# yzang2019/tendermint-fork

Measured on AMD Instinct MI355X. Metric: ed25519 verifies/sec at 1/8 MI355X, higher is better.
Workload: dtype u32 (GF(2^255-19) radix 2^25.5 limbs, int64 accumulate); 1 GPU; C2: raw batch of 1048576 ed25519 signatures per GPU; signatures_per_gpu=1048576, key_cache=False, parallelism=shard-per-gpu x1

## Files before the change

### __graft_entry__.py

```python
from __future__ import annotations

import os
import subprocess
import sys

ROOT = os.path.dirname(os.path.abspath(__file__))
PKG = os.path.join(ROOT, "tendermint-fork_amd")


def _paths():
    for p in (ROOT, PKG):
        if p not in sys.path:
            sys.path.insert(0, p)


def build() -> None:
    env = dict(os.environ, PYTORCH_ROCM_ARCH="gfx950")
    jobs = str(min(8, os.cpu_count() or 1))
    subprocess.check_call(["make", "-j", jobs, "-C", PKG], env=env)
    subprocess.check_call(["make", "-s", "-C", os.path.join(ROOT, "oracle")])
    subprocess.check_call(["make", "-s", "-C", os.path.join(ROOT, "tests", "native")])
    _paths()
    import tmed
    tmed.lib()


def smoke() -> None:
    _paths()
    import numpy as np
    from oracle import port
    from tmed import Engine
    eng = Engine(0)
    rng = np.random.default_rng(0)
    for n in (256, 32768):
        seeds = rng.integers(0, 256, (n, 32), dtype=np.uint8)
        offs = (np.arange(n + 1) * 115).astype(np.uint32)
        msgs = rng.integers(0, 256, int(offs[-1]) + 16, dtype=np.uint8)
        sigs, pubs = eng.sign_arrays(seeds, msgs, offs)
        sigs[1::7, 9] ^= 1
        out = eng.verify_arrays(pubs, sigs, msgs, offs)
        exp = port.verify_batch(pubs, sigs, msgs, offs.astype(np.uint64), 8)
        esig, epub = port.sign_batch(seeds[:8], msgs, offs[:9].astype(np.uint64), 1)
        assert (out == exp).all(), "GPU/oracle decision mismatch (n=%d)" % n
        assert (pubs[:8] == epub).all() and (sigs[:1] == esig[:1]).all(), "GPU signer != oracle signer"
        assert out.sum() == n - len(range(1, n, 7))
    eng.close()
    print("smoke ok: 256 + 32768 signatures verified on cuda:0, decisions == oracle")


if __name__ == "__main__":
    build()
    if len(sys.argv) > 1 and sys.argv[1] == "smoke":
        smoke()
```

### tendermint-fork_amd/csrc/fe25519.h

```cpp
#pragma once
#include <stdint.h>

#if defined(__HIPCC__)
#include <hip/hip_runtime.h>
#define TMED_HD __host__ __device__ __forceinline__
#define TMED_HDM __host__ __device__ __forceinline__
#else
#define TMED_HD static inline
#define TMED_HDM inline
#endif

namespace tmed {

struct fe { int32_t v[10]; };

TMED_HD int32_t mul19(int32_t x) { return (int32_t)(19u * (uint32_t)x); }
TMED_HD int32_t mul38(int32_t x) { return (int32_t)(38u * (uint32_t)x); }
TMED_HD int32_t dbl32(int32_t x) {
#if defined(__HIP_DEVICE_COMPILE__)
  int32_t r;
  asm("v_add_u32 %0, %1, %1" : "=v"(r) : "v"(x));
  return r;
#else
  return (int32_t)(2u * (uint32_t)x);
// ... 163 lines not shown
  int64_t H0[10], H1[10];
  fe_sq2_sq1_fused(H0, H1, a.x, a.x2, a.x4, a.x19, a.x38, b.x, b.x2, b.x4, b.x19, b.x38);
  fe_fused_fin(h0, H0);
  fe_fused_fin(h1, H1);
}

TMED_HD void fe_sqn(fe &h, const fe &f, int n) {
  fe_sqc(h, f);
#pragma unroll 1
  for (int i = 1; i < n; i++) fe_sqc(h, h);
}

TMED_HD void fe_pow250(fe &z250, fe &z11, const fe &z) {
  fe z2, z9, t, a, b, c;
  fe_sqc(z2, z);
  fe_sqn(t, z2, 2); fe_mul(z9, t, z);
  fe_mul(z11, z9, z2);
  fe_sqc(t, z11); fe_mul(a, t, z9);
  fe_sqn(t, a, 5); fe_mul(b, t, a);
  fe_sqn(t, b, 10); fe_mul(c, t, b);
  fe_sqn(t, c, 20); fe_mul(t, t, c);
  fe_sqn(t, t, 10); fe_mul(a, t, b);
  fe_sqn(t, a, 50); fe_mul(b, t, a);
  fe_sqn(t, b, 100); fe_mul(t, t, b);
  fe_sqn(t, t, 50); fe_mul(z250, t, a);
}

TMED_HD void fe_invert(fe &out, const fe &z) {
  fe z250, z11, t;
  fe_pow250(z250, z11, z);
  fe_sqn(t, z250, 5); fe_mul(out, t, z11);
}

TMED_HD void fe_pow22523(fe &out, const fe &z) {
  fe z250, z11, t;
  fe_pow250(z250, z11, z);
  fe_sqn(t, z250, 2); fe_mul(out, t, z);
}

TMED_HD void fe_from_words(fe &h, const uint32_t w[8]) {
  const int off[10] = {0, 26, 51, 77, 102, 128, 153, 179, 204, 230};
  int64_t t[10];
#pragma unroll
  for (int i = 0; i < 10; i++) {
    const int o = off[i], q = o >> 5, r = o & 31;
    const uint64_t lo = w[q];
    const uint64_t hi = (q + 1 < 8) ? (uint64_t)w[q + 1] : 0;
    const uint64_t x = ((hi << 32) | lo) >> r;
    const uint32_t mask = (i & 1) ? 0x1ffffffu : 0x3ffffffu;
    t[i] = (int64_t)(uint32_t)(x & mask) + fe_bias(i);
  }
  fe_carry64(h, t);
}

TMED_HD void fe_to_words(uint32_t w[8], const fe &f) {
  int32_t h[10];
#pragma unroll
  for (int i = 0; i < 10; i++) h[i] = f.v[i];
  int32_t q = (19 * h[9] + (1 << 24)) >> 25;
#pragma unroll
  for (int i = 0; i < 10; i++) q = (h[i] + q) >> ((i & 1) ? 25 : 26);
  h[0] += 19 * q;
#pragma unroll
  for (int i = 0; i < 9; i++) {
    const int s = (i & 1) ? 25 : 26;
    const int32_t c = h[i] >> s;
    h[i + 1] += c;
// ... 211 lines not shown
```

### tendermint-fork_amd/csrc/fe_cols.h

```cpp
#pragma once

TMED_HD void fe_mul_fused(int64_t H[10], const int32_t f[10], const int32_t f2[10], const int32_t g[10], const int32_t g19[10]) {
  const int64_t b0 = (int64_t)1 << 25, b50 = (int64_t)1 << 50;
  int64_t t0, t1;
#if defined(__HIP_DEVICE_COMPILE__)
  asm(
      "v_mad_i64_i32 %0, vcc, %12, %27, %46\n"
      "v_mad_i64_i32 %1, vcc, %12, %28, %47\n"
      "v_mad_i64_i32 %0, vcc, %22, %45, %0\n"
      "v_mad_i64_i32 %1, vcc, %13, %27, %1\n"
      "v_mad_i64_i32 %0, vcc, %14, %44, %0\n"
      "v_mad_i64_i32 %1, vcc, %14, %45, %1\n"
      "v_mad_i64_i32 %0, vcc, %23, %43, %0\n"
      "v_mad_i64_i32 %1, vcc, %15, %44, %1\n"
      "v_mad_i64_i32 %0, vcc, %16, %42, %0\n"
      "v_mad_i64_i32 %1, vcc, %16, %43, %1\n"
      "v_mad_i64_i32 %0, vcc, %24, %41, %0\n"
      "v_mad_i64_i32 %1, vcc, %17, %42, %1\n"
      "v_mad_i64_i32 %0, vcc, %18, %40, %0\n"
      "v_mad_i64_i32 %1, vcc, %18, %41, %1\n"
      "v_mad_i64_i32 %0, vcc, %25, %39, %0\n"
      "v_mad_i64_i32 %1, vcc, %19, %40, %1\n"
      "v_mad_i64_i32 %0, vcc, %20, %38, %0\n"
      "v_mad_i64_i32 %1, vcc, %20, %39, %1\n"
// ... 30 lines not shown
      "v_lshl_add_u64 %3, %10, 0, %3\n"
      "v_mad_i64_i32 %5, vcc, %16, %28, %5\n"
      "v_ashrrev_i64 %11, 25, %3\n"
      "v_mad_i64_i32 %5, vcc, %17, %27, %5\n"
      "v_mad_i64_i32 %4, vcc, %12, %31, %11\n"
      "v_mad_i64_i32 %5, vcc, %18, %45, %5\n"
      "v_mad_i64_i32 %4, vcc, %22, %30, %4\n"
      "v_mad_i64_i32 %5, vcc, %19, %44, %5\n"
      "v_mad_i64_i32 %4, vcc, %14, %29, %4\n"
      "v_mad_i64_i32 %5, vcc, %20, %43, %5\n"
      "v_mad_i64_i32 %4, vcc, %23, %28, %4\n"
      "v_mad_i64_i32 %5, vcc, %21, %42, %5\n"
      "v_mad_i64_i32 %4, vcc, %16, %27, %4\n"
      "v_mad_i64_i32 %7, vcc, %12, %34, %47\n"
      "v_mad_i64_i32 %4, vcc, %24, %45, %4\n"
      "v_mad_i64_i32 %7, vcc, %13, %33, %7\n"
      "v_mad_i64_i32 %4, vcc, %18, %44, %4\n"
      "v_mad_i64_i32 %7, vcc, %14, %32, %7\n"
      "v_mad_i64_i32 %4, vcc, %25, %43, %4\n"
      "v_mad_i64_i32 %7, vcc, %15, %31, %7\n"
      "v_mad_i64_i32 %4, vcc, %20, %42, %4\n"
      "v_mad_i64_i32 %7, vcc, %16, %30, %7\n"
      "v_mad_i64_i32 %4, vcc, %26, %41, %4\n"
      "v_mad_i64_i32 %7, vcc, %17, %29, %7\n"
      "v_ashrrev_i64 %10, 26, %4\n"
      "v_mad_i64_i32 %7, vcc, %18, %28, %7\n"
      "v_lshl_add_u64 %5, %10, 0, %5\n"
      "v_mad_i64_i32 %7, vcc, %19, %27, %7\n"
      "v_ashrrev_i64 %11, 25, %5\n"
      "v_mad_i64_i32 %7, vcc, %20, %45, %7\n"
      "v_mad_i64_i32 %6, vcc, %12, %33, %11\n"
      "v_mad_i64_i32 %7, vcc, %21, %44, %7\n"
      "v_mad_i64_i32 %6, vcc, %22, %32, %6\n"
      "v_mad_i64_i32 %9, vcc, %12, %36, 0\n"
      "v_mad_i64_i32 %6, vcc, %14, %31, %6\n"
      "v_mad_i64_i32 %9, vcc, %13, %35, %9\n"
      "v_mad_i64_i32 %6, vcc, %23, %30, %6\n"
      "v_mad_i64_i32 %9, vcc, %14, %34, %9\n"
      "v_mad_i64_i32 %6, vcc, %16, %29, %6\n"
      "v_mad_i64_i32 %9, vcc, %15, %33, %9\n"
      "v_mad_i64_i32 %6, vcc, %24, %28, %6\n"
      "v_mad_i64_i32 %9, vcc, %16, %32, %9\n"
      "v_mad_i64_i32 %6, vcc, %18, %27, %6\n"
      "v_mad_i64_i32 %9, vcc, %17, %31, %9\n"
      "v_mad_i64_i32 %6, vcc, %25, %45, %6\n"
      "v_mad_i64_i32 %9, vcc, %18, %30, %9\n"
      "v_mad_i64_i32 %6, vcc, %20, %44, %6\n"
      "v_mad_i64_i32 %9, vcc, %19, %29, %9\n"
      "v_mad_i64_i32 %6, vcc, %26, %43, %6\n"
      "v_mad_i64_i32 %9, vcc, %20, %28, %9\n"
      "v_ashrrev_i64 %10, 26, %6\n"
      "v_mad_i64_i32 %9, vcc, %21, %27, %9\n"
      "v_lshl_add_u64 %7, %10, 0, %7\n"
      "v_ashrrev_i64 %11, 25, %7\n"
      "v_mad_i64_i32 %8, vcc, %12, %35, %11\n"
      "v_mad_i64_i32 %8, vcc, %22, %34, %8\n"
      "v_mad_i64_i32 %8, vcc, %14, %33, %8\n"
      "v_mad_i64_i32 %8, vcc, %23, %32, %8\n"
      "v_mad_i64_i32 %8, vcc, %16, %31, %8\n"
      "v_mad_i64_i32 %8, vcc, %24, %30, %8\n"
      "v_mad_i64_i32 %8, vcc, %18, %29, %8\n"
      "v_mad_i64_i32 %8, vcc, %25, %28, %8\n"
      "v_mad_i64_i32 %8, vcc, %20, %27, %8\n"
      "v_mad_i64_i32 %8, vcc, %26, %45, %8\n"
      "v_ashrrev_i64 %10, 26, %8\n"
      "v_lshl_add_u64 %9, %10, 0, %9\n"
      : "=&v"(H[0]), "=&v"(H[1]), "=&v"(H[2]), "=&v"(H[3]), "=&v"(H[4]), "=&v"(H[5]),
        "=&v"(H[6]), "=&v"(H[7]), "=&v"(H[8]), "=&v"(H[9]), "=&v"(t0), "=&v"(t1)
      : "v"(f[0]), "v"(f[1]), "v"(f[2]), "v"(f[3]), "v"(f[4]), "v"(f[5]),
        "v"(f[6]), "v"(f[7]), "v"(f[8]), "v"(f[9]), "v"(f2[1]), "v"(f2[3]),
        "v"(f2[5]), "v"(f2[7]), "v"(f2[9]), "v"(g[0]), "v"(g[1]), "v"(g[2]),
        "v"(g[3]), "v"(g[4]), "v"(g[5]), "v"(g[6]), "v"(g[7]), "v"(g[8]),
        "v"(g[9]), "v"(g19[1]), "v"(g19[2]), "v"(g19[3]), "v"(g19[4]), "v"(g19[5]),
        "v"(g19[6]), "v"(g19[7]), "v"(g19[8]), "v"(g19[9]), "s"(b0), "s"(b50)
      : "vcc");
#else
  H[0] = b0 + (int64_t)f[0] * (int64_t)g[0];
  H[1] = b50 + (int64_t)f[0] * (int64_t)g[1];
  H[0] = H[0] + (int64_t)f2[1] * (int64_t)g19[9];
  H[1] = H[1] + (int64_t)f[1] * (int64_t)g[0];
  H[0] = H[0] + (int64_t)f[2] * (int64_t)g19[8];
  H[1] = H[1] + (int64_t)f[2] * (int64_t)g19[9];
  H[0] = H[0] + (int64_t)f2[3] * (int64_t)g19[7];
  H[1] = H[1] + (int64_t)f[3] * (int64_t)g19[8];
  H[0] = H[0] + (int64_t)f[4] * (int64_t)g19[6];
  H[1] = H[1] + (int64_t)f[4] * (int64_t)g19[7];
  H[0] = H[0] + (int64_t)f2[5] * (int64_t)g19[5];
  H[1] = H[1] + (int64_t)f[5] * (int64_t)g19[6];
  H[0] = H[0] + (int64_t)f[6] * (int64_t)g19[4];
  H[1] = H[1] + (int64_t)f[6] * (int64_t)g19[5];
  H[0] = H[0] + (int64_t)f2[7] * (int64_t)g19[3];
  H[1] = H[1] + (int64_t)f[7] * (int64_t)g19[4];
  H[0] = H[0] + (int64_t)f[8] * (int64_t)g19[2];
  H[1] = H[1] + (int64_t)f[8] * (int64_t)g19[3];
  H[0] = H[0] + (int64_t)f2[9] * (int64_t)g19[1];
  H[1] = H[1] + (int64_t)f[9] * (int64_t)g19[2];
  t0 = H[0] >> 26;
  H[3] = b50 + (int64_t)f[0] * (int64_t)g[3];
  H[1] += t0;
// ... 25 lines not shown
  H[3] += t0;
  H[5] = H[5] + (int64_t)f[4] * (int64_t)g[1];
  t1 = H[3] >> 25;
  H[5] = H[5] + (int64_t)f[5] * (int64_t)g[0];
  H[4] = t1 + (int64_t)f[0] * (int64_t)g[4];
  H[5] = H[5] + (int64_t)f[6] * (int64_t)g19[9];
  H[4] = H[4] + (int64_t)f2[1] * (int64_t)g[3];
  H[5] = H[5] + (int64_t)f[7] * (int64_t)g19[8];
  H[4] = H[4] + (int64_t)f[2] * (int64_t)g[2];
  H[5] = H[5] + (int64_t)f[8] * (int64_t)g19[7];
  H[4] = H[4] + (int64_t)f2[3] * (int64_t)g[1];
  H[5] = H[5] + (int64_t)f[9] * (int64_t)g19[6];
  H[4] = H[4] + (int64_t)f[4] * (int64_t)g[0];
  H[7] = b50 + (int64_t)f[0] * (int64_t)g[7];
  H[4] = H[4] + (int64_t)f2[5] * (int64_t)g19[9];
  H[7] = H[7] + (int64_t)f[1] * (int64_t)g[6];
  H[4] = H[4] + (int64_t)f[6] * (int64_t)g19[8];
  H[7] = H[7] + (int64_t)f[2] * (int64_t)g[5];
  H[4] = H[4] + (int64_t)f2[7] * (int64_t)g19[7];
  H[7] = H[7] + (int64_t)f[3] * (int64_t)g[4];
  H[4] = H[4] + (int64_t)f[8] * (int64_t)g19[6];
  H[7] = H[7] + (int64_t)f[4] * (int64_t)g[3];
  H[4] = H[4] + (int64_t)f2[9] * (int64_t)g19[5];
  H[7] = H[7] + (int64_t)f[5] * (int64_t)g[2];
  t0 = H[4] >> 26;
  H[7] = H[7] + (int64_t)f[6] * (int64_t)g[1];
  H[5] += t0;
  H[7] = H[7] + (int64_t)f[7] * (int64_t)g[0];
  t1 = H[5] >> 25;
  H[7] = H[7] + (int64_t)f[8] * (int64_t)g19[9];
  H[6] = t1 + (int64_t)f[0] * (int64_t)g[6];
  H[7] = H[7] + (int64_t)f[9] * (int64_t)g19[8];
  H[6] = H[6] + (int64_t)f2[1] * (int64_t)g[5];
  H[9] = 0 + (int64_t)f[0] * (int64_t)g[9];
  H[6] = H[6] + (int64_t)f[2] * (int64_t)g[4];
  H[9] = H[9] + (int64_t)f[1] * (int64_t)g[8];
  H[6] = H[6] + (int64_t)f2[3] * (int64_t)g[3];
  H[9] = H[9] + (int64_t)f[2] * (int64_t)g[7];
  H[6] = H[6] + (int64_t)f[4] * (int64_t)g[2];
  H[9] = H[9] + (int64_t)f[3] * (int64_t)g[6];
  H[6] = H[6] + (int64_t)f2[5] * (int64_t)g[1];
  H[9] = H[9] + (int64_t)f[4] * (int64_t)g[5];
  H[6] = H[6] + (int64_t)f[6] * (int64_t)g[0];
  H[9] = H[9] + (int64_t)f[5] * (int64_t)g[4];
  H[6] = H[6] + (int64_t)f2[7] * (int64_t)g19[9];
  H[9] = H[9] + (int64_t)f[6] * (int64_t)g[3];
  H[6] = H[6] + (int64_t)f[8] * (int64_t)g19[8];
  H[9] = H[9] + (int64_t)f[7] * (int64_t)g[2];
  H[6] = H[6] + (int64_t)f2[9] * (int64_t)g19[7];
  H[9] = H[9] + (int64_t)f[8] * (int64_t)g[1];
  t0 = H[6] >> 26;
  H[9] = H[9] + (int64_t)f[9] * (int64_t)g[0];
  H[7] += t0;
  t1 = H[7] >> 25;
  H[8] = t1 + (int64_t)f[0] * (int64_t)g[8];
  H[8] = H[8] + (int64_t)f2[1] * (int64_t)g[7];
  H[8] = H[8] + (int64_t)f[2] * (int64_t)g[6];
  H[8] = H[8] + (int64_t)f2[3] * (int64_t)g[5];
  H[8] = H[8] + (int64_t)f[4] * (int64_t)g[4];
  H[8] = H[8] + (int64_t)f2[5] * (int64_t)g[3];
  H[8] = H[8] + (int64_t)f[6] * (int64_t)g[2];
  H[8] = H[8] + (int64_t)f2[7] * (int64_t)g[1];
  H[8] = H[8] + (int64_t)f[8] * (int64_t)g[0];
  H[8] = H[8] + (int64_t)f2[9] * (int64_t)g19[9];
  t0 = H[8] >> 26;
  H[9] += t0;
#endif
}

TMED_HD void fe_sq1_fused(int64_t H[10], const int32_t x[10], const int32_t x2[10], const int32_t x4[10], const int32_t x19[10], const int32_t x38[10]) {
  const int64_t b0 = (int64_t)1 << 25, b50 = (int64_t)1 << 50;
  int64_t t0, t1;
#if defined(__HIP_DEVICE_COMPILE__)
  asm(
      "v_mad_i64_i32 %0, vcc, %32, %40, %41\n"
      "v_mad_i64_i32 %1, vcc, %24, %40, %42\n"
      "v_mad_i64_i32 %0, vcc, %24, %39, %0\n"
      "v_mad_i64_i32 %1, vcc, %25, %39, %1\n"
      "v_mad_i64_i32 %0, vcc, %33, %38, %0\n"
      "v_mad_i64_i32 %1, vcc, %26, %38, %1\n"
      "v_mad_i64_i32 %0, vcc, %26, %37, %0\n"
      "v_mad_i64_i32 %1, vcc, %27, %37, %1\n"
      "v_mad_i64_i32 %0, vcc, %27, %36, %0\n"
      "v_mad_i64_i32 %1, vcc, %22, %13, %1\n"
      "v_mad_i64_i32 %0, vcc, %12, %12, %0\n"
      "v_mad_i64_i32 %3, vcc, %26, %40, %42\n"
      "v_ashrrev_i64 %10, 26, %0\n"
      "v_mad_i64_i32 %3, vcc, %27, %39, %3\n"
      "v_lshl_add_u64 %1, %10, 0, %1\n"
      "v_mad_i64_i32 %3, vcc, %28, %38, %3\n"
      "v_ashrrev_i64 %11, 25, %1\n"
      "v_mad_i64_i32 %3, vcc, %22, %15, %3\n"
      "v_mad_i64_i32 %2, vcc, %33, %40, %11\n"
      "v_mad_i64_i32 %3, vcc, %23, %14, %3\n"
      "v_mad_i64_i32 %2, vcc, %26, %39, %2\n"
      "v_mad_i64_i32 %5, vcc, %28, %40, %42\n"
      "v_mad_i64_i32 %2, vcc, %34, %38, %2\n"
      "v_mad_i64_i32 %5, vcc, %29, %39, %5\n"
      "v_mad_i64_i32 %2, vcc, %18, %37, %2\n"
      "v_mad_i64_i32 %5, vcc, %22, %17, %5\n"
      "v_mad_i64_i32 %2, vcc, %22, %14, %2\n"
      "v_mad_i64_i32 %5, vcc, %23, %16, %5\n"
      "v_mad_i64_i32 %2, vcc, %23, %13, %2\n"
      "v_mad_i64_i32 %5, vcc, %24, %15, %5\n"
      "v_ashrrev_i64 %10, 26, %2\n"
      "v_mad_i64_i32 %7, vcc, %30, %40, %42\n"
      "v_lshl_add_u64 %3, %10, 0, %3\n"
      "v_mad_i64_i32 %7, vcc, %22, %19, %7\n"
      "v_ashrrev_i64 %11, 25, %3\n"
      "v_mad_i64_i32 %7, vcc, %23, %18, %7\n"
      "v_mad_i64_i32 %4, vcc, %34, %40, %11\n"
      "v_mad_i64_i32 %7, vcc, %24, %17, %7\n"
      "v_mad_i64_i32 %4, vcc, %28, %39, %4\n"
      "v_mad_i64_i32 %7, vcc, %25, %16, %7\n"
      "v_mad_i64_i32 %4, vcc, %29, %38, %4\n"
      "v_mad_i64_i32 %9, vcc, %22, %21, 0\n"
      "v_mad_i64_i32 %4, vcc, %22, %16, %4\n"
      "v_mad_i64_i32 %9, vcc, %23, %20, %9\n"
      "v_mad_i64_i32 %4, vcc, %32, %15, %4\n"
      "v_mad_i64_i32 %9, vcc, %24, %19, %9\n"
      "v_mad_i64_i32 %4, vcc, %14, %14, %4\n"
      "v_mad_i64_i32 %9, vcc, %25, %18, %9\n"
      "v_ashrrev_i64 %10, 26, %4\n"
      "v_mad_i64_i32 %9, vcc, %26, %17, %9\n"
      "v_lshl_add_u64 %5, %10, 0, %5\n"
      "v_ashrrev_i64 %11, 25, %5\n"
      "v_mad_i64_i32 %6, vcc, %35, %40, %11\n"
      "v_mad_i64_i32 %6, vcc, %20, %39, %6\n"
      "v_mad_i64_i32 %6, vcc, %22, %18, %6\n"
      "v_mad_i64_i32 %6, vcc, %32, %17, %6\n"
      "v_mad_i64_i32 %6, vcc, %24, %16, %6\n"
      "v_mad_i64_i32 %6, vcc, %25, %15, %6\n"
      "v_ashrrev_i64 %10, 26, %6\n"
      "v_lshl_add_u64 %7, %10, 0, %7\n"
      "v_ashrrev_i64 %11, 25, %7\n"
      "v_mad_i64_i32 %8, vcc, %31, %40, %11\n"
      "v_mad_i64_i32 %8, vcc, %22, %20, %8\n"
      "v_mad_i64_i32 %8, vcc, %32, %19, %8\n"
      "v_mad_i64_i32 %8, vcc, %24, %18, %8\n"
      "v_mad_i64_i32 %8, vcc, %33, %17, %8\n"
      "v_mad_i64_i32 %8, vcc, %16, %16, %8\n"
      "v_ashrrev_i64 %10, 26, %8\n"
      "v_lshl_add_u64 %9, %10, 0, %9\n"
      : "=&v"(H[0]), "=&v"(H[1]), "=&v"(H[2]), "=&v"(H[3]), "=&v"(H[4]), "=&v"(H[5]),
        "=&v"(H[6]), "=&v"(H[7]), "=&v"(H[8]), "=&v"(H[9]), "=&v"(t0), "=&v"(t1)
      : "v"(x[0]), "v"(x[1]), "v"(x[2]), "v"(x[3]), "v"(x[4]), "v"(x[5]),
        "v"(x[6]), "v"(x[7]), "v"(x[8]), "v"(x[9]), "v"(x2[0]), "v"(x2[1]),
        "v"(x2[2]), "v"(x2[3]), "v"(x2[4]), "v"(x2[5]), "v"(x2[6]), "v"(x2[7]),
        "v"(x2[8]), "v"(x2[9]), "v"(x4[1]), "v"(x4[3]), "v"(x4[5]), "v"(x4[7]),
        "v"(x19[5]), "v"(x19[6]), "v"(x19[7]), "v"(x19[8]), "v"(x19[9]), "s"(b0),
        "s"(b50)
      : "vcc");
#else
  H[0] = b0 + (int64_t)x4[1] * (int64_t)x19[9];
  H[1] = b50 + (int64_t)x2[2] * (int64_t)x19[9];
  H[0] = H[0] + (int64_t)x2[2] * (int64_t)x19[8];
  H[1] = H[1] + (int64_t)x2[3] * (int64_t)x19[8];
  H[0] = H[0] + (int64_t)x4[3] * (int64_t)x19[7];
  H[1] = H[1] + (int64_t)x2[4] * (int64_t)x19[7];
  H[0] = H[0] + (int64_t)x2[4] * (int64_t)x19[6];
  H[1] = H[1] + (int64_t)x2[5] * (int64_t)x19[6];
  H[0] = H[0] + (int64_t)x2[5] * (int64_t)x19[5];
  H[1] = H[1] + (int64_t)x2[0] * (int64_t)x[1];
  H[0] = H[0] + (int64_t)x[0] * (int64_t)x[0];
  H[3] = b50 + (int64_t)x2[4] * (int64_t)x19[9];
  t0 = H[0] >> 26;
  H[3] = H[3] + (int64_t)x2[5] * (int64_t)x19[8];
  H[1] += t0;
  H[3] = H[3] + (int64_t)x2[6] * (int64_t)x19[7];
  t1 = H[1] >> 25;
  H[3] = H[3] + (int64_t)x2[0] * (int64_t)x[3];
  H[2] = t1 + (int64_t)x4[3] * (int64_t)x19[9];
  H[3] = H[3] + (int64_t)x2[1] * (int64_t)x[2];
  H[2] = H[2] + (int64_t)x2[4] * (int64_t)x19[8];
  H[5] = b50 + (int64_t)x2[6] * (int64_t)x19[9];
  H[2] = H[2] + (int64_t)x4[5] * (int64_t)x19[7];
  H[5] = H[5] + (int64_t)x2[7] * (int64_t)x19[8];
  H[2] = H[2] + (int64_t)x[6] * (int64_t)x19[6];
  H[5] = H[5] + (int64_t)x2[0] * (int64_t)x[5];
  H[2] = H[2] + (int64_t)x2[0] * (int64_t)x[2];
  H[5] = H[5] + (int64_t)x2[1] * (int64_t)x[4];
  H[2] = H[2] + (int64_t)x2[1] * (int64_t)x[1];
  H[5] = H[5] + (int64_t)x2[2] * (int64_t)x[3];
  t0 = H[2] >> 26;
  H[7] = b50 + (int64_t)x2[8] * (int64_t)x19[9];
  H[3] += t0;
  H[7] = H[7] + (int64_t)x2[0] * (int64_t)x[7];
  t1 = H[3] >> 25;
  H[7] = H[7] + (int64_t)x2[1] * (int64_t)x[6];
  H[4] = t1 + (int64_t)x4[5] * (int64_t)x19[9];
  H[7] = H[7] + (int64_t)x2[2] * (int64_t)x[5];
  H[4] = H[4] + (int64_t)x2[6] * (int64_t)x19[8];
  H[7] = H[7] + (int64_t)x2[3] * (int64_t)x[4];
  H[4] = H[4] + (int64_t)x2[7] * (int64_t)x19[7];
  H[9] = 0 + (int64_t)x2[0] * (int64_t)x[9];
  H[4] = H[4] + (int64_t)x2[0] * (int64_t)x[4];
  H[9] = H[9] + (int64_t)x2[1] * (int64_t)x[8];
  H[4] = H[4] + (int64_t)x4[1] * (int64_t)x[3];
  H[9] = H[9] + (int64_t)x2[2] * (int64_t)x[7];
  H[4] = H[4] + (int64_t)x[2] * (int64_t)x[2];
  H[9] = H[9] + (int64_t)x2[3] * (int64_t)x[6];
  t0 = H[4] >> 26;
  H[9] = H[9] + (int64_t)x2[4] * (int64_t)x[5];
  H[5] += t0;
  t1 = H[5] >> 25;
  H[6] = t1 + (int64_t)x4[7] * (int64_t)x19[9];
  H[6] = H[6] + (int64_t)x[8] * (int64_t)x19[8];
  H[6] = H[6] + (int64_t)x2[0] * (int64_t)x[6];
  H[6] = H[6] + (int64_t)x4[1] * (int64_t)x[5];
  H[6] = H[6] + (int64_t)x2[2] * (int64_t)x[4];
  H[6] = H[6] + (int64_t)x2[3] * (int64_t)x[3];
  t0 = H[6] >> 26;
  H[7] += t0;
  t1 = H[7] >> 25;
  H[8] = t1 + (int64_t)x2[9] * (int64_t)x19[9];
  H[8] = H[8] + (int64_t)x2[0] * (int64_t)x[8];
  H[8] = H[8] + (int64_t)x4[1] * (int64_t)x[7];
  H[8] = H[8] + (int64_t)x2[2] * (int64_t)x[6];
  H[8] = H[8] + (int64_t)x4[3] * (int64_t)x[5];
  H[8] = H[8] + (int64_t)x[4] * (int64_t)x[4];
  t0 = H[8] >> 26;
  H[9] += t0;
#endif
}

TMED_HD void fe_sq2_fused(int64_t H[10], const int32_t x[10], const int32_t x2[10], const int32_t x4[10], const int32_t x19[10], const int32_t x38[10]) {
  const int64_t b0 = (int64_t)1 << 25, b50 = (int64_t)1 << 50;
  int64_t t0, t1;
#if defined(__HIP_DEVICE_COMPILE__)
  asm(
      "v_mad_i64_i32 %0, vcc, %28, %36, %37\n"
      "v_mad_i64_i32 %1, vcc, %20, %36, %38\n"
      "v_mad_i64_i32 %0, vcc, %20, %35, %0\n"
      "v_mad_i64_i32 %1, vcc, %21, %35, %1\n"
      "v_mad_i64_i32 %0, vcc, %29, %34, %0\n"
      "v_mad_i64_i32 %1, vcc, %22, %34, %1\n"
      "v_mad_i64_i32 %0, vcc, %22, %33, %0\n"
      "v_mad_i64_i32 %1, vcc, %23, %33, %1\n"
      "v_mad_i64_i32 %0, vcc, %23, %32, %0\n"
      "v_mad_i64_i32 %1, vcc, %12, %28, %1\n"
      "v_mad_i64_i32 %0, vcc, %19, %12, %0\n"
      "v_mad_i64_i32 %3, vcc, %22, %36, %38\n"
      "v_ashrrev_i64 %10, 26, %0\n"
      "v_mad_i64_i32 %3, vcc, %23, %35, %3\n"
      "v_lshl_add_u64 %1, %10, 0, %1\n"
      "v_mad_i64_i32 %3, vcc, %24, %34, %3\n"
      "v_ashrrev_i64 %11, 25, %1\n"
      "v_mad_i64_i32 %3, vcc, %19, %21, %3\n"
      "v_mad_i64_i32 %2, vcc, %29, %36, %11\n"
      "v_mad_i64_i32 %3, vcc, %28, %14, %3\n"
      "v_mad_i64_i32 %2, vcc, %22, %35, %2\n"
      "v_mad_i64_i32 %5, vcc, %24, %36, %38\n"
      "v_mad_i64_i32 %2, vcc, %30, %34, %2\n"
      "v_mad_i64_i32 %5, vcc, %25, %35, %5\n"
      "v_mad_i64_i32 %2, vcc, %17, %33, %2\n"
      "v_mad_i64_i32 %5, vcc, %19, %23, %5\n"
      "v_mad_i64_i32 %2, vcc, %19, %20, %2\n"
      "v_mad_i64_i32 %5, vcc, %28, %16, %5\n"
      "v_mad_i64_i32 %2, vcc, %28, %13, %2\n"
      "v_mad_i64_i32 %5, vcc, %20, %21, %5\n"
      "v_ashrrev_i64 %10, 26, %2\n"
      "v_mad_i64_i32 %7, vcc, %26, %36, %38\n"
      "v_lshl_add_u64 %3, %10, 0, %3\n"
      "v_mad_i64_i32 %7, vcc, %19, %25, %7\n"
      "v_ashrrev_i64 %11, 25, %3\n"
      "v_mad_i64_i32 %7, vcc, %28, %17, %7\n"
      "v_mad_i64_i32 %4, vcc, %30, %36, %11\n"
      "v_mad_i64_i32 %7, vcc, %20, %23, %7\n"
      "v_mad_i64_i32 %4, vcc, %24, %35, %4\n"
      "v_mad_i64_i32 %7, vcc, %29, %16, %7\n"
      "v_mad_i64_i32 %4, vcc, %25, %34, %4\n"
      "v_mad_i64_i32 %9, vcc, %19, %27, 0\n"
      "v_mad_i64_i32 %4, vcc, %19, %22, %4\n"
      "v_mad_i64_i32 %9, vcc, %28, %18, %9\n"
      "v_mad_i64_i32 %4, vcc, %28, %21, %4\n"
      "v_mad_i64_i32 %9, vcc, %20, %25, %9\n"
      "v_mad_i64_i32 %4, vcc, %20, %14, %4\n"
      "v_mad_i64_i32 %9, vcc, %29, %17, %9\n"
      "v_ashrrev_i64 %10, 26, %4\n"
      "v_mad_i64_i32 %9, vcc, %22, %23, %9\n"
      "v_lshl_add_u64 %5, %10, 0, %5\n"
      "v_ashrrev_i64 %11, 25, %5\n"
      "v_mad_i64_i32 %6, vcc, %31, %36, %11\n"
      "v_mad_i64_i32 %6, vcc, %18, %35, %6\n"
      "v_mad_i64_i32 %6, vcc, %19, %24, %6\n"
      "v_mad_i64_i32 %6, vcc, %28, %23, %6\n"
      "v_mad_i64_i32 %6, vcc, %20, %22, %6\n"
      "v_mad_i64_i32 %6, vcc, %29, %15, %6\n"
      "v_ashrrev_i64 %10, 26, %6\n"
      "v_lshl_add_u64 %7, %10, 0, %7\n"
      "v_ashrrev_i64 %11, 25, %7\n"
      "v_mad_i64_i32 %8, vcc, %27, %36, %11\n"
      "v_mad_i64_i32 %8, vcc, %19, %26, %8\n"
      "v_mad_i64_i32 %8, vcc, %28, %25, %8\n"
      "v_mad_i64_i32 %8, vcc, %20, %24, %8\n"
      "v_mad_i64_i32 %8, vcc, %29, %23, %8\n"
      "v_mad_i64_i32 %8, vcc, %22, %16, %8\n"
      "v_ashrrev_i64 %10, 26, %8\n"
      "v_lshl_add_u64 %9, %10, 0, %9\n"
      : "=&v"(H[0]), "=&v"(H[1]), "=&v"(H[2]), "=&v"(H[3]), "=&v"(H[4]), "=&v"(H[5]),
        "=&v"(H[6]), "=&v"(H[7]), "=&v"(H[8]), "=&v"(H[9]), "=&v"(t0), "=&v"(t1)
      : "v"(x[0]), "v"(x[1]), "v"(x[2]), "v"(x[3]), "v"(x[4]), "v"(x[6]),
        "v"(x[8]), "v"(x2[0]), "v"(x2[2]), "v"(x2[3]), "v"(x2[4]), "v"(x2[5]),
        "v"(x2[6]), "v"(x2[7]), "v"(x2[8]), "v"(x2[9]), "v"(x4[1]), "v"(x4[3]),
        "v"(x4[5]), "v"(x4[7]), "v"(x38[5]), "v"(x38[6]), "v"(x38[7]), "v"(x38[8]),
        "v"(x38[9]), "s"(b0), "s"(b50)
      : "vcc");
#else
  H[0] = b0 + (int64_t)x4[1] * (int64_t)x38[9];
  H[1] = b50 + (int64_t)x2[2] * (int64_t)x38[9];
  H[0] = H[0] + (int64_t)x2[2] * (int64_t)x38[8];
  H[1] = H[1] + (int64_t)x2[3] * (int64_t)x38[8];
  H[0] = H[0] + (int64_t)x4[3] * (int64_t)x38[7];
  H[1] = H[1] + (int64_t)x2[4] * (int64_t)x38[7];
  H[0] = H[0] + (int64_t)x2[4] * (int64_t)x38[6];
  H[1] = H[1] + (int64_t)x2[5] * (int64_t)x38[6];
  H[0] = H[0] + (int64_t)x2[5] * (int64_t)x38[5];
  H[1] = H[1] + (int64_t)x[0] * (int64_t)x4[1];
  H[0] = H[0] + (int64_t)x2[0] * (int64_t)x[0];
  H[3] = b50 + (int64_t)x2[4] * (int64_t)x38[9];
  t0 = H[0] >> 26;
  H[3] = H[3] + (int64_t)x2[5] * (int64_t)x38[8];
  H[1] += t0;
  H[3] = H[3] + (int64_t)x2[6] * (int64_t)x38[7];
  t1 = H[1] >> 25;
  H[3] = H[3] + (int64_t)x2[0] * (int64_t)x2[3];
  H[2] = t1 + (int64_t)x4[3] * (int64_t)x38[9];
  H[3] = H[3] + (int64_t)x4[1] * (int64_t)x[2];
  H[2] = H[2] + (int64_t)x2[4] * (int64_t)x38[8];
  H[5] = b50 + (int64_t)x2[6] * (int64_t)x38[9];
  H[2] = H[2] + (int64_t)x4[5] * (int64_t)x38[7];
  H[5] = H[5] + (int64_t)x2[7] * (int64_t)x38[8];
  H[2] = H[2] + (int64_t)x[6] * (int64_t)x38[6];
  H[5] = H[5] + (int64_t)x2[0] * (int64_t)x2[5];
  H[2] = H[2] + (int64_t)x2[0] * (int64_t)x2[2];
  H[5] = H[5] + (int64_t)x4[1] * (int64_t)x[4];
  H[2] = H[2] + (int64_t)x4[1] * (int64_t)x[1];
  H[5] = H[5] + (int64_t)x2[2] * (int64_t)x2[3];
  t0 = H[2] >> 26;
  H[7] = b50 + (int64_t)x2[8] * (int64_t)x38[9];
  H[3] += t0;
  H[7] = H[7] + (int64_t)x2[0] * (int64_t)x2[7];
  t1 = H[3] >> 25;
  H[7] = H[7] + (int64_t)x4[1] * (int64_t)x[6];
  H[4] = t1 + (int64_t)x4[5] * (int64_t)x38[9];
  H[7] = H[7] + (int64_t)x2[2] * (int64_t)x2[5];
  H[4] = H[4] + (int64_t)x2[6] * (int64_t)x38[8];
  H[7] = H[7] + (int64_t)x4[3] * (int64_t)x[4];
  H[4] = H[4] + (int64_t)x2[7] * (int64_t)x38[7];
  H[9] = 0 + (int64_t)x2[0] * (int64_t)x2[9];
  H[4] = H[4] + (int64_t)x2[0] * (int64_t)x2[4];
  H[9] = H[9] + (int64_t)x4[1] * (int64_t)x[8];
  H[4] = H[4] + (int64_t)x4[1] * (int64_t)x2[3];
  H[9] = H[9] + (int64_t)x2[2] * (int64_t)x2[7];
  H[4] = H[4] + (int64_t)x2[2] * (int64_t)x[2];
  H[9] = H[9] + (int64_t)x4[3] * (int64_t)x[6];
  t0 = H[4] >> 26;
  H[9] = H[9] + (int64_t)x2[4] * (int64_t)x2[5];
  H[5] += t0;
  t1 = H[5] >> 25;
  H[6] = t1 + (int64_t)x4[7] * (int64_t)x38[9];
  H[6] = H[6] + (int64_t)x[8] * (int64_t)x38[8];
  H[6] = H[6] + (int64_t)x2[0] * (int64_t)x2[6];
  H[6] = H[6] + (int64_t)x4[1] * (int64_t)x2[5];
  H[6] = H[6] + (int64_t)x2[2] * (int64_t)x2[4];
  H[6] = H[6] + (int64_t)x4[3] * (int64_t)x[3];
  t0 = H[6] >> 26;
  H[7] += t0;
  t1 = H[7] >> 25;
  H[8] = t1 + (int64_t)x2[9] * (int64_t)x38[9];
  H[8] = H[8] + (int64_t)x2[0] * (int64_t)x2[8];
  H[8] = H[8] + (int64_t)x4[1] * (int64_t)x2[7];
  H[8] = H[8] + (int64_t)x2[2] * (int64_t)x2[6];
  H[8] = H[8] + (int64_t)x4[3] * (int64_t)x2[5];
  H[8] = H[8] + (int64_t)x2[4] * (int64_t)x[4];
  t0 = H[8] >> 26;
  H[9] += t0;
#endif
}


TMED_HD void fe_mul_fused_x2(int64_t H0[10], int64_t H1[10], const int32_t a_f[10], const int32_t a_f2[10], const int32_t a_g[10], const int32_t a_g19[10], const int32_t b_f[10], const int32_t b_f2[10], const int32_t b_g[10], const int32_t b_g19[10]) {
  const int64_t b0 = (int64_t)1 << 25, b50 = (int64_t)1 << 50;
  int64_t t0_0, t0_1, t1_0, t1_1;
#if defined(__HIP_DEVICE_COMPILE__)
  asm(
      "v_mad_i64_i32 %0, vcc, %24, %39, %92\n"
      "v_mad_i64_i32 %12, vcc, %58, %73, %92\n"
      "v_mad_i64_i32 %1, vcc, %24, %40, %93\n"
      "v_mad_i64_i32 %0, vcc, %34, %57, %0\n"
      "v_mad_i64_i32 %12, vcc, %68, %91, %12\n"
      "v_mad_i64_i32 %13, vcc, %58, %74, %93\n"
      "v_mad_i64_i32 %0, vcc, %26, %56, %0\n"
      "v_mad_i64_i32 %1, vcc, %25, %39, %1\n"
      "v_mad_i64_i32 %12, vcc, %60, %90, %12\n"
      "v_mad_i64_i32 %13, vcc, %59, %73, %13\n"
      "v_mad_i64_i32 %0, vcc, %35, %55, %0\n"
      "v_mad_i64_i32 %1, vcc, %26, %57, %1\n"
      "v_mad_i64_i32 %12, vcc, %69, %89, %12\n"
      "v_mad_i64_i32 %13, vcc, %60, %91, %13\n"
      "v_mad_i64_i32 %0, vcc, %28, %54, %0\n"
      "v_mad_i64_i32 %1, vcc, %27, %56, %1\n"
      "v_mad_i64_i32 %12, vcc, %62, %88, %12\n"
      "v_mad_i64_i32 %13, vcc, %61, %90, %13\n"
      "v_mad_i64_i32 %0, vcc, %36, %53, %0\n"
      "v_mad_i64_i32 %1, vcc, %28, %55, %1\n"
      "v_mad_i64_i32 %12, vcc, %70, %87, %12\n"
      "v_mad_i64_i32 %13, vcc, %62, %89, %13\n"
      "v_mad_i64_i32 %0, vcc, %30, %52, %0\n"
      "v_mad_i64_i32 %1, vcc, %29, %54, %1\n"
// ... 534 lines not shown
      "v_mad_i64_i32 %5, vcc, %36, %27, %5\n"
      "v_ashrrev_i64 %10, 26, %4\n"
      "v_mad_i64_i32 %17, vcc, %65, %56, %17\n"
      "v_ashrrev_i64 %22, 26, %16\n"
      "v_lshl_add_u64 %5, %10, 0, %5\n"
      "v_mad_i64_i32 %7, vcc, %42, %52, %83\n"
      "v_lshl_add_u64 %17, %22, 0, %17\n"
      "v_ashrrev_i64 %11, 25, %5\n"
      "v_mad_i64_i32 %19, vcc, %71, %81, %83\n"
      "v_ashrrev_i64 %23, 25, %17\n"
      "v_mad_i64_i32 %6, vcc, %47, %52, %11\n"
      "v_mad_i64_i32 %7, vcc, %34, %31, %7\n"
      "v_mad_i64_i32 %18, vcc, %76, %81, %23\n"
      "v_mad_i64_i32 %6, vcc, %32, %51, %6\n"
      "v_mad_i64_i32 %19, vcc, %63, %60, %19\n"
      "v_mad_i64_i32 %18, vcc, %61, %80, %18\n"
      "v_mad_i64_i32 %6, vcc, %34, %30, %6\n"
      "v_mad_i64_i32 %7, vcc, %35, %30, %7\n"
      "v_mad_i64_i32 %18, vcc, %63, %59, %18\n"
      "v_mad_i64_i32 %6, vcc, %44, %29, %6\n"
      "v_mad_i64_i32 %19, vcc, %64, %59, %19\n"
      "v_mad_i64_i32 %18, vcc, %73, %58, %18\n"
      "v_mad_i64_i32 %6, vcc, %36, %28, %6\n"
      "v_mad_i64_i32 %7, vcc, %36, %29, %7\n"
      "v_mad_i64_i32 %18, vcc, %65, %57, %18\n"
      "v_mad_i64_i32 %6, vcc, %37, %27, %6\n"
      "v_mad_i64_i32 %19, vcc, %65, %58, %19\n"
      "v_mad_i64_i32 %18, vcc, %66, %56, %18\n"
      "v_mad_i64_i32 %7, vcc, %37, %28, %7\n"
      "v_ashrrev_i64 %10, 26, %6\n"
      "v_mad_i64_i32 %19, vcc, %66, %57, %19\n"
      "v_ashrrev_i64 %22, 26, %18\n"
      "v_lshl_add_u64 %7, %10, 0, %7\n"
      "v_mad_i64_i32 %9, vcc, %34, %33, 0\n"
      "v_lshl_add_u64 %19, %22, 0, %19\n"
      "v_ashrrev_i64 %11, 25, %7\n"
      "v_mad_i64_i32 %21, vcc, %63, %62, 0\n"
      "v_ashrrev_i64 %23, 25, %19\n"
      "v_mad_i64_i32 %8, vcc, %43, %52, %11\n"
      "v_mad_i64_i32 %9, vcc, %35, %32, %9\n"
      "v_mad_i64_i32 %20, vcc, %72, %81, %23\n"
      "v_mad_i64_i32 %8, vcc, %34, %32, %8\n"
      "v_mad_i64_i32 %21, vcc, %64, %61, %21\n"
      "v_mad_i64_i32 %20, vcc, %63, %61, %20\n"
      "v_mad_i64_i32 %8, vcc, %44, %31, %8\n"
      "v_mad_i64_i32 %9, vcc, %36, %31, %9\n"
      "v_mad_i64_i32 %20, vcc, %73, %60, %20\n"
      "v_mad_i64_i32 %8, vcc, %36, %30, %8\n"
      "v_mad_i64_i32 %21, vcc, %65, %60, %21\n"
      "v_mad_i64_i32 %20, vcc, %65, %59, %20\n"
      "v_mad_i64_i32 %8, vcc, %45, %29, %8\n"
      "v_mad_i64_i32 %9, vcc, %37, %30, %9\n"
      "v_mad_i64_i32 %20, vcc, %74, %58, %20\n"
      "v_mad_i64_i32 %8, vcc, %28, %28, %8\n"
      "v_mad_i64_i32 %21, vcc, %66, %59, %21\n"
      "v_mad_i64_i32 %20, vcc, %57, %57, %20\n"
      "v_mad_i64_i32 %9, vcc, %38, %29, %9\n"
      "v_ashrrev_i64 %10, 26, %8\n"
      "v_mad_i64_i32 %21, vcc, %67, %58, %21\n"
      "v_ashrrev_i64 %22, 26, %20\n"
      "v_lshl_add_u64 %9, %10, 0, %9\n"
      "v_lshl_add_u64 %21, %22, 0, %21\n"
      : "=&v"(H0[0]), "=&v"(H0[1]), "=&v"(H0[2]), "=&v"(H0[3]), "=&v"(H0[4]), "=&v"(H0[5]),
        "=&v"(H0[6]), "=&v"(H0[7]), "=&v"(H0[8]), "=&v"(H0[9]), "=&v"(t0_0), "=&v"(t0_1),
        "=&v"(H1[0]), "=&v"(H1[1]), "=&v"(H1[2]), "=&v"(H1[3]), "=&v"(H1[4]), "=&v"(H1[5]),
        "=&v"(H1[6]), "=&v"(H1[7]), "=&v"(H1[8]), "=&v"(H1[9]), "=&v"(t1_0), "=&v"(t1_1)
      : "v"(a_x[0]), "v"(a_x[1]), "v"(a_x[2]), "v"(a_x[3]), "v"(a_x[4]), "v"(a_x[5]),
        "v"(a_x[6]), "v"(a_x[7]), "v"(a_x[8]), "v"(a_x[9]), "v"(a_x2[0]), "v"(a_x2[1]),
        "v"(a_x2[2]), "v"(a_x2[3]), "v"(a_x2[4]), "v"(a_x2[5]), "v"(a_x2[6]), "v"(a_x2[7]),
        "v"(a_x2[8]), "v"(a_x2[9]), "v"(a_x4[1]), "v"(a_x4[3]), "v"(a_x4[5]), "v"(a_x4[7]),
        "v"(a_x19[5]), "v"(a_x19[6]), "v"(a_x19[7]), "v"(a_x19[8]), "v"(a_x19[9]), "v"(b_x[0]),
        "v"(b_x[1]), "v"(b_x[2]), "v"(b_x[3]), "v"(b_x[4]), "v"(b_x[5]), "v"(b_x[6]),
        "v"(b_x[7]), "v"(b_x[8]), "v"(b_x[9]), "v"(b_x2[0]), "v"(b_x2[1]), "v"(b_x2[2]),
        "v"(b_x2[3]), "v"(b_x2[4]), "v"(b_x2[5]), "v"(b_x2[6]), "v"(b_x2[7]), "v"(b_x2[8]),
        "v"(b_x2[9]), "v"(b_x4[1]), "v"(b_x4[3]), "v"(b_x4[5]), "v"(b_x4[7]), "v"(b_x19[5]),
        "v"(b_x19[6]), "v"(b_x19[7]), "v"(b_x19[8]), "v"(b_x19[9]), "s"(b0), "s"(b50)
      : "vcc");
#else
  H0[0] = b0 + (int64_t)a_x4[1] * (int64_t)a_x19[9];
  H1[0] = b0 + (int64_t)b_x4[1] * (int64_t)b_x19[9];
  H0[1] = b50 + (int64_t)a_x2[2] * (int64_t)a_x19[9];
  H0[0] = H0[0] + (int64_t)a_x2[2] * (int64_t)a_x19[8];
  H1[0] = H1[0] + (int64_t)b_x2[2] * (int64_t)b_x19[8];
  H1[1] = b50 + (int64_t)b_x2[2] * (int64_t)b_x19[9];
  H0[0] = H0[0] + (int64_t)a_x4[3] * (int64_t)a_x19[7];
  H1[0] = H1[0] + (int64_t)b_x4[3] * (int64_t)b_x19[7];
  H0[1] = H0[1] + (int64_t)a_x2[3] * (int64_t)a_x19[8];
  H0[0] = H0[0] + (int64_t)a_x2[4] * (int64_t)a_x19[6];
  H1[0] = H1[0] + (int64_t)b_x2[4] * (int64_t)b_x19[6];
  H1[1] = H1[1] + (int64_t)b_x2[3] * (int64_t)b_x19[8];
  H0[0] = H0[0] + (int64_t)a_x2[5] * (int64_t)a_x19[5];
  H0[1] = H0[1] + (int64_t)a_x2[4] * (int64_t)a_x19[7];
  H1[0] = H1[0] + (int64_t)b_x2[5] * (int64_t)b_x19[5];
  H1[1] = H1[1] + (int64_t)b_x2[4] * (int64_t)b_x19[7];
  H0[0] = H0[0] + (int64_t)a_x[0] * (int64_t)a_x[0];
// ... 59 lines not shown
  H0[5] = H0[5] + (int64_t)a_x2[2] * (int64_t)a_x[3];
  t0_0 = H0[4] >> 26;
  H1[5] = H1[5] + (int64_t)b_x2[2] * (int64_t)b_x[3];
  t1_0 = H1[4] >> 26;
  H0[5] += t0_0;
  H0[7] = b50 + (int64_t)a_x2[8] * (int64_t)a_x19[9];
  H1[5] += t1_0;
  t0_1 = H0[5] >> 25;
  H1[7] = b50 + (int64_t)b_x2[8] * (int64_t)b_x19[9];
  t1_1 = H1[5] >> 25;
  H0[6] = t0_1 + (int64_t)a_x4[7] * (int64_t)a_x19[9];
  H0[7] = H0[7] + (int64_t)a_x2[0] * (int64_t)a_x[7];
  H1[6] = t1_1 + (int64_t)b_x4[7] * (int64_t)b_x19[9];
  H0[6] = H0[6] + (int64_t)a_x[8] * (int64_t)a_x19[8];
  H1[7] = H1[7] + (int64_t)b_x2[0] * (int64_t)b_x[7];
  H1[6] = H1[6] + (int64_t)b_x[8] * (int64_t)b_x19[8];
  H0[6] = H0[6] + (int64_t)a_x2[0] * (int64_t)a_x[6];
  H0[7] = H0[7] + (int64_t)a_x2[1] * (int64_t)a_x[6];
  H1[6] = H1[6] + (int64_t)b_x2[0] * (int64_t)b_x[6];
  H0[6] = H0[6] + (int64_t)a_x4[1] * (int64_t)a_x[5];
  H1[7] = H1[7] + (int64_t)b_x2[1] * (int64_t)b_x[6];
  H1[6] = H1[6] + (int64_t)b_x4[1] * (int64_t)b_x[5];
  H0[6] = H0[6] + (int64_t)a_x2[2] * (int64_t)a_x[4];
  H0[7] = H0[7] + (int64_t)a_x2[2] * (int64_t)a_x[5];
  H1[6] = H1[6] + (int64_t)b_x2[2] * (int64_t)b_x[4];
  H0[6] = H0[6] + (int64_t)a_x2[3] * (int64_t)a_x[3];
  H1[7] = H1[7] + (int64_t)b_x2[2] * (int64_t)b_x[5];
  H1[6] = H1[6] + (int64_t)b_x2[3] * (int64_t)b_x[3];
  H0[7] = H0[7] + (int64_t)a_x2[3] * (int64_t)a_x[4];
  t0_0 = H0[6] >> 26;
  H1[7] = H1[7] + (int64_t)b_x2[3] * (int64_t)b_x[4];
  t1_0 = H1[6] >> 26;
  H0[7] += t0_0;
  H0[9] = 0 + (int64_t)a_x2[0] * (int64_t)a_x[9];
  H1[7] += t1_0;
  t0_1 = H0[7] >> 25;
  H1[9] = 0 + (int64_t)b_x2[0] * (int64_t)b_x[9];
  t1_1 = H1[7] >> 25;
  H0[8] = t0_1 + (int64_t)a_x2[9] * (int64_t)a_x19[9];
  H0[9] = H0[9] + (int64_t)a_x2[1] * (int64_t)a_x[8];
  H1[8] = t1_1 + (int64_t)b_x2[9] * (int64_t)b_x19[9];
  H0[8] = H0[8] + (int64_t)a_x2[0] * (int64_t)a_x[8];
  H1[9] = H1[9] + (int64_t)b_x2[1] * (int64_t)b_x[8];
  H1[8] = H1[8] + (int64_t)b_x2[0] * (int64_t)b_x[8];
  H0[8] = H0[8] + (int64_t)a_x4[1] * (int64_t)a_x[7];
  H0[9] = H0[9] + (int64_t)a_x2[2] * (int64_t)a_x[7];
  H1[8] = H1[8] + (int64_t)b_x4[1] * (int64_t)b_x[7];
  H0[8] = H0[8] + (int64_t)a_x2[2] * (int64_t)a_x[6];
  H1[9] = H1[9] + (int64_t)b_x2[2] * (int64_t)b_x[7];
  H1[8] = H1[8] + (int64_t)b_x2[2] * (int64_t)b_x[6];
  H0[8] = H0[8] + (int64_t)a_x4[3] * (int64_t)a_x[5];
  H0[9] = H0[9] + (int64_t)a_x2[3] * (int64_t)a_x[6];
  H1[8] = H1[8] + (int64_t)b_x4[3] * (int64_t)b_x[5];
  H0[8] = H0[8] + (int64_t)a_x[4] * (int64_t)a_x[4];
  H1[9] = H1[9] + (int64_t)b_x2[3] * (int64_t)b_x[6];
  H1[8] = H1[8] + (int64_t)b_x[4] * (int64_t)b_x[4];
  H0[9] = H0[9] + (int64_t)a_x2[4] * (int64_t)a_x[5];
  t0_0 = H0[8] >> 26;
  H1[9] = H1[9] + (int64_t)b_x2[4] * (int64_t)b_x[5];
  t1_0 = H1[8] >> 26;
  H0[9] += t0_0;
  H1[9] += t1_0;
#endif
}

TMED_HD void fe_sq2_sq1_fused(int64_t H0[10], int64_t H1[10], const int32_t a_x[10], const int32_t a_x2[10], const int32_t a_x4[10], const int32_t a_x19[10], const int32_t a_x38[10], const int32_t b_x[10], const int32_t b_x2[10], const int32_t b_x4[10], const int32_t b_x19[10], const int32_t b_x38[10]) {
  const int64_t b0 = (int64_t)1 << 25, b50 = (int64_t)1 << 50;
  int64_t t0_0, t0_1, t1_0, t1_1;
#if defined(__HIP_DEVICE_COMPILE__)
  asm(
      "v_mad_i64_i32 %0, vcc, %40, %48, %78\n"
      "v_mad_i64_i32 %12, vcc, %69, %77, %78\n"
      "v_mad_i64_i32 %1, vcc, %32, %48, %79\n"
      "v_mad_i64_i32 %0, vcc, %32, %47, %0\n"
      "v_mad_i64_i32 %12, vcc, %61, %76, %12\n"
      "v_mad_i64_i32 %13, vcc, %61, %77, %79\n"
      "v_mad_i64_i32 %0, vcc, %41, %46, %0\n"
      "v_mad_i64_i32 %12, vcc, %70, %75, %12\n"
      "v_mad_i64_i32 %1, vcc, %33, %47, %1\n"
      "v_mad_i64_i32 %0, vcc, %34, %45, %0\n"
      "v_mad_i64_i32 %12, vcc, %63, %74, %12\n"
      "v_mad_i64_i32 %13, vcc, %62, %76, %13\n"
      "v_mad_i64_i32 %0, vcc, %35, %44, %0\n"
      "v_mad_i64_i32 %1, vcc, %34, %46, %1\n"
      "v_mad_i64_i32 %12, vcc, %64, %73, %12\n"
      "v_mad_i64_i32 %13, vcc, %63, %75, %13\n"
      "v_mad_i64_i32 %0, vcc, %31, %24, %0\n"
      "v_mad_i64_i32 %1, vcc, %35, %45, %1\n"
      "v_mad_i64_i32 %12, vcc, %49, %49, %12\n"
      "v_mad_i64_i32 %13, vcc, %64, %74, %13\n"
      "v_mad_i64_i32 %1, vcc, %24, %40, %1\n"
      "v_ashrrev_i64 %10, 26, %0\n"
      "v_mad_i64_i32 %13, vcc, %59, %50, %13\n"
      "v_ashrrev_i64 %22, 26, %12\n"
      "v_lshl_add_u64 %1, %10, 0, %1\n"
// ... 51 lines not shown
      "v_mad_i64_i32 %5, vcc, %32, %33, %5\n"
      "v_ashrrev_i64 %10, 26, %4\n"
      "v_mad_i64_i32 %17, vcc, %61, %52, %17\n"
      "v_ashrrev_i64 %22, 26, %16\n"
      "v_lshl_add_u64 %5, %10, 0, %5\n"
      "v_mad_i64_i32 %7, vcc, %38, %48, %79\n"
      "v_lshl_add_u64 %17, %22, 0, %17\n"
      "v_ashrrev_i64 %11, 25, %5\n"
      "v_mad_i64_i32 %19, vcc, %67, %77, %79\n"
      "v_ashrrev_i64 %23, 25, %17\n"
      "v_mad_i64_i32 %6, vcc, %43, %48, %11\n"
      "v_mad_i64_i32 %7, vcc, %31, %37, %7\n"
      "v_mad_i64_i32 %18, vcc, %72, %77, %23\n"
      "v_mad_i64_i32 %6, vcc, %30, %47, %6\n"
      "v_mad_i64_i32 %19, vcc, %59, %56, %19\n"
      "v_mad_i64_i32 %18, vcc, %57, %76, %18\n"
      "v_mad_i64_i32 %6, vcc, %31, %36, %6\n"
      "v_mad_i64_i32 %7, vcc, %40, %29, %7\n"
      "v_mad_i64_i32 %18, vcc, %59, %55, %18\n"
      "v_mad_i64_i32 %6, vcc, %40, %35, %6\n"
      "v_mad_i64_i32 %19, vcc, %60, %55, %19\n"
      "v_mad_i64_i32 %18, vcc, %69, %54, %18\n"
      "v_mad_i64_i32 %6, vcc, %32, %34, %6\n"
      "v_mad_i64_i32 %7, vcc, %32, %35, %7\n"
      "v_mad_i64_i32 %18, vcc, %61, %53, %18\n"
      "v_mad_i64_i32 %6, vcc, %41, %27, %6\n"
      "v_mad_i64_i32 %19, vcc, %61, %54, %19\n"
      "v_mad_i64_i32 %18, vcc, %62, %52, %18\n"
      "v_mad_i64_i32 %7, vcc, %41, %28, %7\n"
      "v_ashrrev_i64 %10, 26, %6\n"
      "v_mad_i64_i32 %19, vcc, %62, %53, %19\n"
      "v_ashrrev_i64 %22, 26, %18\n"
      "v_lshl_add_u64 %7, %10, 0, %7\n"
      "v_mad_i64_i32 %9, vcc, %31, %39, 0\n"
      "v_lshl_add_u64 %19, %22, 0, %19\n"
      "v_ashrrev_i64 %11, 25, %7\n"
      "v_mad_i64_i32 %21, vcc, %59, %58, 0\n"
      "v_ashrrev_i64 %23, 25, %19\n"
      "v_mad_i64_i32 %8, vcc, %39, %48, %11\n"
      "v_mad_i64_i32 %9, vcc, %40, %30, %9\n"
      "v_mad_i64_i32 %20, vcc, %68, %77, %23\n"
      "v_mad_i64_i32 %8, vcc, %31, %38, %8\n"
      "v_mad_i64_i32 %21, vcc, %60, %57, %21\n"
      "v_mad_i64_i32 %20, vcc, %59, %57, %20\n"
      "v_mad_i64_i32 %8, vcc, %40, %37, %8\n"
      "v_mad_i64_i32 %9, vcc, %32, %37, %9\n"
      "v_mad_i64_i32 %20, vcc, %69, %56, %20\n"
      "v_mad_i64_i32 %8, vcc, %32, %36, %8\n"
      "v_mad_i64_i32 %21, vcc, %61, %56, %21\n"
      "v_mad_i64_i32 %20, vcc, %61, %55, %20\n"
      "v_mad_i64_i32 %8, vcc, %41, %35, %8\n"
      "v_mad_i64_i32 %9, vcc, %41, %29, %9\n"
      "v_mad_i64_i32 %20, vcc, %70, %54, %20\n"
      "v_mad_i64_i32 %8, vcc, %34, %28, %8\n"
      "v_mad_i64_i32 %21, vcc, %62, %55, %21\n"
      "v_mad_i64_i32 %20, vcc, %53, %53, %20\n"
      "v_mad_i64_i32 %9, vcc, %34, %35, %9\n"
      "v_ashrrev_i64 %10, 26, %8\n"
      "v_mad_i64_i32 %21, vcc, %63, %54, %21\n"
      "v_ashrrev_i64 %22, 26, %20\n"
      "v_lshl_add_u64 %9, %10, 0, %9\n"
      "v_lshl_add_u64 %21, %22, 0, %21\n"
      : "=&v"(H0[0]), "=&v"(H0[1]), "=&v"(H0[2]), "=&v"(H0[3]), "=&v"(H0[4]), "=&v"(H0[5]),
        "=&v"(H0[6]), "=&v"(H0[7]), "=&v"(H0[8]), "=&v"(H0[9]), "=&v"(t0_0), "=&v"(t0_1),
        "=&v"(H1[0]), "=&v"(H1[1]), "=&v"(H1[2]), "=&v"(H1[3]), "=&v"(H1[4]), "=&v"(H1[5]),
        "=&v"(H1[6]), "=&v"(H1[7]), "=&v"(H1[8]), "=&v"(H1[9]), "=&v"(t1_0), "=&v"(t1_1)
      : "v"(a_x[0]), "v"(a_x[1]), "v"(a_x[2]), "v"(a_x[3]), "v"(a_x[4]), "v"(a_x[6]),
        "v"(a_x[8]), "v"(a_x2[0]), "v"(a_x2[2]), "v"(a_x2[3]), "v"(a_x2[4]), "v"(a_x2[5]),
        "v"(a_x2[6]), "v"(a_x2[7]), "v"(a_x2[8]), "v"(a_x2[9]), "v"(a_x4[1]), "v"(a_x4[3]),
        "v"(a_x4[5]), "v"(a_x4[7]), "v"(a_x38[5]), "v"(a_x38[6]), "v"(a_x38[7]), "v"(a_x38[8]),
        "v"(a_x38[9]), "v"(b_x[0]), "v"(b_x[1]), "v"(b_x[2]), "v"(b_x[3]), "v"(b_x[4]),
        "v"(b_x[5]), "v"(b_x[6]), "v"(b_x[7]), "v"(b_x[8]), "v"(b_x[9]), "v"(b_x2[0]),
        "v"(b_x2[1]), "v"(b_x2[2]), "v"(b_x2[3]), "v"(b_x2[4]), "v"(b_x2[5]), "v"(b_x2[6]),
        "v"(b_x2[7]), "v"(b_x2[8]), "v"(b_x2[9]), "v"(b_x4[1]), "v"(b_x4[3]), "v"(b_x4[5]),
        "v"(b_x4[7]), "v"(b_x19[5]), "v"(b_x19[6]), "v"(b_x19[7]), "v"(b_x19[8]), "v"(b_x19[9]),
        "s"(b0), "s"(b50)
      : "vcc");
#else
  H0[0] = b0 + (int64_t)a_x4[1] * (int64_t)a_x38[9];
  H1[0] = b0 + (int64_t)b_x4[1] * (int64_t)b_x19[9];
  H0[1] = b50 + (int64_t)a_x2[2] * (int64_t)a_x38[9];
  H0[0] = H0[0] + (int64_t)a_x2[2] * (int64_t)a_x38[8];
  H1[0] = H1[0] + (int64_t)b_x2[2] * (int64_t)b_x19[8];
  H1[1] = b50 + (int64_t)b_x2[2] * (int64_t)b_x19[9];
  H0[0] = H0[0] + (int64_t)a_x4[3] * (int64_t)a_x38[7];
  H1[0] = H1[0] + (int64_t)b_x4[3] * (int64_t)b_x19[7];
  H0[1] = H0[1] + (int64_t)a_x2[3] * (int64_t)a_x38[8];
  H0[0] = H0[0] + (int64_t)a_x2[4] * (int64_t)a_x38[6];
  H1[0] = H1[0] + (int64_t)b_x2[4] * (int64_t)b_x19[6];
  H1[1] = H1[1] + (int64_t)b_x2[3] * (int64_t)b_x19[8];
  H0[0] = H0[0] + (int64_t)a_x2[5] * (int64_t)a_x38[5];
  H0[1] = H0[1] + (int64_t)a_x2[4] * (int64_t)a_x38[7];
  H1[0] = H1[0] + (int64_t)b_x2[5] * (int64_t)b_x19[5];
  H1[1] = H1[1] + (int64_t)b_x2[4] * (int64_t)b_x19[7];
  H0[0] = H0[0] + (int64_t)a_x2[0] * (int64_t)a_x[0];
// ... 59 lines not shown
  H0[5] = H0[5] + (int64_t)a_x2[2] * (int64_t)a_x2[3];
  t0_0 = H0[4] >> 26;
  H1[5] = H1[5] + (int64_t)b_x2[2] * (int64_t)b_x[3];
  t1_0 = H1[4] >> 26;
  H0[5] += t0_0;
  H0[7] = b50 + (int64_t)a_x2[8] * (int64_t)a_x38[9];
  H1[5] += t1_0;
  t0_1 = H0[5] >> 25;
  H1[7] = b50 + (int64_t)b_x2[8] * (int64_t)b_x19[9];
  t1_1 = H1[5] >> 25;
  H0[6] = t0_1 + (int64_t)a_x4[7] * (int64_t)a_x38[9];
  H0[7] = H0[7] + (int64_t)a_x2[0] * (int64_t)a_x2[7];
  H1[6] = t1_1 + (int64_t)b_x4[7] * (int64_t)b_x19[9];
  H0[6] = H0[6] + (int64_t)a_x[8] * (int64_t)a_x38[8];
  H1[7] = H1[7] + (int64_t)b_x2[0] * (int64_t)b_x[7];
  H1[6] = H1[6] + (int64_t)b_x[8] * (int64_t)b_x19[8];
  H0[6] = H0[6] + (int64_t)a_x2[0] * (int64_t)a_x2[6];
  H0[7] = H0[7] + (int64_t)a_x4[1] * (int64_t)a_x[6];
  H1[6] = H1[6] + (int64_t)b_x2[0] * (int64_t)b_x[6];
  H0[6] = H0[6] + (int64_t)a_x4[1] * (int64_t)a_x2[5];
  H1[7] = H1[7] + (int64_t)b_x2[1] * (int64_t)b_x[6];
  H1[6] = H1[6] + (int64_t)b_x4[1] * (int64_t)b_x[5];
  H0[6] = H0[6] + (int64_t)a_x2[2] * (int64_t)a_x2[4];
  H0[7] = H0[7] + (int64_t)a_x2[2] * (int64_t)a_x2[5];
  H1[6] = H1[6] + (int64_t)b_x2[2] * (int64_t)b_x[4];
  H0[6] = H0[6] + (int64_t)a_x4[3] * (int64_t)a_x[3];
  H1[7] = H1[7] + (int64_t)b_x2[2] * (int64_t)b_x[5];
  H1[6] = H1[6] + (int64_t)b_x2[3] * (int64_t)b_x[3];
  H0[7] = H0[7] + (int64_t)a_x4[3] * (int64_t)a_x[4];
  t0_0 = H0[6] >> 26;
  H1[7] = H1[7] + (int64_t)b_x2[3] * (int64_t)b_x[4];
  t1_0 = H1[6] >> 26;
  H0[7] += t0_0;
  H0[9] = 0 + (int64_t)a_x2[0] * (int64_t)a_x2[9];
  H1[7] += t1_0;
  t0_1 = H0[7] >> 25;
  H1[9] = 0 + (int64_t)b_x2[0] * (int64_t)b_x[9];
  t1_1 = H1[7] >> 25;
  H0[8] = t0_1 + (int64_t)a_x2[9] * (int64_t)a_x38[9];
  H0[9] = H0[9] + (int64_t)a_x4[1] * (int64_t)a_x[8];
  H1[8] = t1_1 + (int64_t)b_x2[9] * (int64_t)b_x19[9];
  H0[8] = H0[8] + (int64_t)a_x2[0] * (int64_t)a_x2[8];
  H1[9] = H1[9] + (int64_t)b_x2[1] * (int64_t)b_x[8];
  H1[8] = H1[8] + (int64_t)b_x2[0] * (int64_t)b_x[8];
  H0[8] = H0[8] + (int64_t)a_x4[1] * (int64_t)a_x2[7];
  H0[9] = H0[9] + (int64_t)a_x2[2] * (int64_t)a_x2[7];
  H1[8] = H1[8] + (int64_t)b_x4[1] * (int64_t)b_x[7];
  H0[8] = H0[8] + (int64_t)a_x2[2] * (int64_t)a_x2[6];
  H1[9] = H1[9] + (int64_t)b_x2[2] * (int64_t)b_x[7];
  H1[8] = H1[8] + (int64_t)b_x2[2] * (int64_t)b_x[6];
  H0[8] = H0[8] + (int64_t)a_x4[3] * (int64_t)a_x2[5];
  H0[9] = H0[9] + (int64_t)a_x4[3] * (int64_t)a_x[6];
  H1[8] = H1[8] + (int64_t)b_x4[3] * (int64_t)b_x[5];
  H0[8] = H0[8] + (int64_t)a_x2[4] * (int64_t)a_x[4];
  H1[9] = H1[9] + (int64_t)b_x2[3] * (int64_t)b_x[6];
  H1[8] = H1[8] + (int64_t)b_x[4] * (int64_t)b_x[4];
  H0[9] = H0[9] + (int64_t)a_x2[4] * (int64_t)a_x2[5];
  t0_0 = H0[8] >> 26;
  H1[9] = H1[9] + (int64_t)b_x2[4] * (int64_t)b_x[5];
  t1_0 = H1[8] >> 26;
  H0[9] += t0_0;
  H1[9] += t1_0;
#endif
}


TMED_HD void fe_sq1c_fused(int64_t H[10], const int32_t x[10], const int32_t x2[10], const int32_t x19[10], const int32_t x38[10]) {
  const int64_t b0 = (int64_t)1 << 25, b50 = (int64_t)1 << 50;
  int64_t t0, t1;
#if defined(__HIP_DEVICE_COMPILE__)
  asm(
      "v_mad_i64_i32 %0, vcc, %23, %34, %35\n"
      "v_mad_i64_i32 %1, vcc, %14, %34, %36\n"
      "v_mad_i64_i32 %0, vcc, %14, %33, %0\n"
      "v_mad_i64_i32 %1, vcc, %15, %33, %1\n"
      "v_mad_i64_i32 %0, vcc, %25, %32, %0\n"
      "v_mad_i64_i32 %1, vcc, %16, %32, %1\n"
      "v_mad_i64_i32 %0, vcc, %16, %31, %0\n"
      "v_mad_i64_i32 %1, vcc, %17, %31, %1\n"
      "v_mad_i64_i32 %0, vcc, %17, %30, %0\n"
      "v_mad_i64_i32 %1, vcc, %12, %23, %1\n"
      "v_mad_i64_i32 %0, vcc, %12, %12, %0\n"
      "v_mad_i64_i32 %3, vcc, %16, %34, %36\n"
      "v_ashrrev_i64 %10, 26, %0\n"
      "v_mad_i64_i32 %3, vcc, %17, %33, %3\n"
      "v_lshl_add_u64 %1, %10, 0, %1\n"
      "v_mad_i64_i32 %3, vcc, %18, %32, %3\n"
      "v_ashrrev_i64 %11, 25, %1\n"
      "v_mad_i64_i32 %3, vcc, %22, %15, %3\n"
      "v_mad_i64_i32 %2, vcc, %25, %34, %11\n"
      "v_mad_i64_i32 %3, vcc, %23, %14, %3\n"
      "v_mad_i64_i32 %2, vcc, %16, %33, %2\n"
      "v_mad_i64_i32 %5, vcc, %18, %34, %36\n"
      "v_mad_i64_i32 %2, vcc, %26, %32, %2\n"
      "v_mad_i64_i32 %5, vcc, %19, %33, %5\n"
      "v_mad_i64_i32 %2, vcc, %18, %28, %2\n"
      "v_mad_i64_i32 %5, vcc, %22, %17, %5\n"
      "v_mad_i64_i32 %2, vcc, %22, %14, %2\n"
      "v_mad_i64_i32 %5, vcc, %23, %16, %5\n"
      "v_mad_i64_i32 %2, vcc, %23, %13, %2\n"
      "v_mad_i64_i32 %5, vcc, %14, %25, %5\n"
      "v_ashrrev_i64 %10, 26, %2\n"
      "v_mad_i64_i32 %7, vcc, %20, %34, %36\n"
      "v_lshl_add_u64 %3, %10, 0, %3\n"
      "v_mad_i64_i32 %7, vcc, %22, %19, %7\n"
      "v_ashrrev_i64 %11, 25, %3\n"
      "v_mad_i64_i32 %7, vcc, %23, %18, %7\n"
      "v_mad_i64_i32 %4, vcc, %26, %34, %11\n"
      "v_mad_i64_i32 %7, vcc, %24, %17, %7\n"
      "v_mad_i64_i32 %4, vcc, %18, %33, %4\n"
      "v_mad_i64_i32 %7, vcc, %25, %16, %7\n"
      "v_mad_i64_i32 %4, vcc, %19, %32, %4\n"
      "v_mad_i64_i32 %9, vcc, %22, %21, 0\n"
      "v_mad_i64_i32 %4, vcc, %22, %16, %4\n"
      "v_mad_i64_i32 %9, vcc, %23, %20, %9\n"
      "v_mad_i64_i32 %4, vcc, %23, %25, %4\n"
      "v_mad_i64_i32 %9, vcc, %24, %19, %9\n"
      "v_mad_i64_i32 %4, vcc, %14, %14, %4\n"
      "v_mad_i64_i32 %9, vcc, %25, %18, %9\n"
      "v_ashrrev_i64 %10, 26, %4\n"
      "v_mad_i64_i32 %9, vcc, %16, %26, %9\n"
      "v_lshl_add_u64 %5, %10, 0, %5\n"
      "v_ashrrev_i64 %11, 25, %5\n"
      "v_mad_i64_i32 %6, vcc, %27, %34, %11\n"
      "v_mad_i64_i32 %6, vcc, %20, %29, %6\n"
      "v_mad_i64_i32 %6, vcc, %22, %18, %6\n"
      "v_mad_i64_i32 %6, vcc, %23, %26, %6\n"
      "v_mad_i64_i32 %6, vcc, %24, %16, %6\n"
      "v_mad_i64_i32 %6, vcc, %25, %15, %6\n"
      "v_ashrrev_i64 %10, 26, %6\n"
      "v_lshl_add_u64 %7, %10, 0, %7\n"
      "v_ashrrev_i64 %11, 25, %7\n"
      "v_mad_i64_i32 %8, vcc, %21, %34, %11\n"
      "v_mad_i64_i32 %8, vcc, %22, %20, %8\n"
      "v_mad_i64_i32 %8, vcc, %23, %27, %8\n"
      "v_mad_i64_i32 %8, vcc, %24, %18, %8\n"
      "v_mad_i64_i32 %8, vcc, %25, %26, %8\n"
      "v_mad_i64_i32 %8, vcc, %16, %16, %8\n"
      "v_ashrrev_i64 %10, 26, %8\n"
      "v_lshl_add_u64 %9, %10, 0, %9\n"
      : "=&v"(H[0]), "=&v"(H[1]), "=&v"(H[2]), "=&v"(H[3]), "=&v"(H[4]), "=&v"(H[5]),
        "=&v"(H[6]), "=&v"(H[7]), "=&v"(H[8]), "=&v"(H[9]), "=&v"(t0), "=&v"(t1)
      : "v"(x[0]), "v"(x[1]), "v"(x[2]), "v"(x[3]), "v"(x[4]), "v"(x[5]),
        "v"(x[6]), "v"(x[7]), "v"(x[8]), "v"(x[9]), "v"(x2[0]), "v"(x2[1]),
        "v"(x2[2]), "v"(x2[3]), "v"(x2[5]), "v"(x2[7]), "v"(x19[6]), "v"(x19[8]),
        "v"(x38[5]), "v"(x38[6]), "v"(x38[7]), "v"(x38[8]), "v"(x38[9]), "s"(b0),
        "s"(b50)
      : "vcc");
#else
  H[0] = b0 + (int64_t)x2[1] * (int64_t)x38[9];
  H[1] = b50 + (int64_t)x[2] * (int64_t)x38[9];
  H[0] = H[0] + (int64_t)x[2] * (int64_t)x38[8];
  H[1] = H[1] + (int64_t)x[3] * (int64_t)x38[8];
  H[0] = H[0] + (int64_t)x2[3] * (int64_t)x38[7];
  H[1] = H[1] + (int64_t)x[4] * (int64_t)x38[7];
  H[0] = H[0] + (int64_t)x[4] * (int64_t)x38[6];
  H[1] = H[1] + (int64_t)x[5] * (int64_t)x38[6];
  H[0] = H[0] + (int64_t)x[5] * (int64_t)x38[5];
  H[1] = H[1] + (int64_t)x[0] * (int64_t)x2[1];
  H[0] = H[0] + (int64_t)x[0] * (int64_t)x[0];
  H[3] = b50 + (int64_t)x[4] * (int64_t)x38[9];
  t0 = H[0] >> 26;
  H[3] = H[3] + (int64_t)x[5] * (int64_t)x38[8];
  H[1] += t0;
  H[3] = H[3] + (int64_t)x[6] * (int64_t)x38[7];
  t1 = H[1] >> 25;
  H[3] = H[3] + (int64_t)x2[0] * (int64_t)x[3];
  H[2] = t1 + (int64_t)x2[3] * (int64_t)x38[9];
  H[3] = H[3] + (int64_t)x2[1] * (int64_t)x[2];
  H[2] = H[2] + (int64_t)x[4] * (int64_t)x38[8];
  H[5] = b50 + (int64_t)x[6] * (int64_t)x38[9];
  H[2] = H[2] + (int64_t)x2[5] * (int64_t)x38[7];
  H[5] = H[5] + (int64_t)x[7] * (int64_t)x38[8];
  H[2] = H[2] + (int64_t)x[6] * (int64_t)x19[6];
  H[5] = H[5] + (int64_t)x2[0] * (int64_t)x[5];
  H[2] = H[2] + (int64_t)x2[0] * (int64_t)x[2];
  H[5] = H[5] + (int64_t)x2[1] * (int64_t)x[4];
  H[2] = H[2] + (int64_t)x2[1] * (int64_t)x[1];
  H[5] = H[5] + (int64_t)x[2] * (int64_t)x2[3];
  t0 = H[2] >> 26;
  H[7] = b50 + (int64_t)x[8] * (int64_t)x38[9];
  H[3] += t0;
  H[7] = H[7] + (int64_t)x2[0] * (int64_t)x[7];
  t1 = H[3] >> 25;
  H[7] = H[7] + (int64_t)x2[1] * (int64_t)x[6];
  H[4] = t1 + (int64_t)x2[5] * (int64_t)x38[9];
  H[7] = H[7] + (int64_t)x2[2] * (int64_t)x[5];
  H[4] = H[4] + (int64_t)x[6] * (int64_t)x38[8];
  H[7] = H[7] + (int64_t)x2[3] * (int64_t)x[4];
  H[4] = H[4] + (int64_t)x[7] * (int64_t)x38[7];
  H[9] = 0 + (int64_t)x2[0] * (int64_t)x[9];
  H[4] = H[4] + (int64_t)x2[0] * (int64_t)x[4];
  H[9] = H[9] + (int64_t)x2[1] * (int64_t)x[8];
  H[4] = H[4] + (int64_t)x2[1] * (int64_t)x2[3];
  H[9] = H[9] + (int64_t)x2[2] * (int64_t)x[7];
  H[4] = H[4] + (int64_t)x[2] * (int64_t)x[2];
  H[9] = H[9] + (int64_t)x2[3] * (int64_t)x[6];
  t0 = H[4] >> 26;
  H[9] = H[9] + (int64_t)x[4] * (int64_t)x2[5];
  H[5] += t0;
  t1 = H[5] >> 25;
  H[6] = t1 + (int64_t)x2[7] * (int64_t)x38[9];
  H[6] = H[6] + (int64_t)x[8] * (int64_t)x19[8];
  H[6] = H[6] + (int64_t)x2[0] * (int64_t)x[6];
  H[6] = H[6] + (int64_t)x2[1] * (int64_t)x2[5];
  H[6] = H[6] + (int64_t)x2[2] * (int64_t)x[4];
  H[6] = H[6] + (int64_t)x2[3] * (int64_t)x[3];
  t0 = H[6] >> 26;
  H[7] += t0;
  t1 = H[7] >> 25;
  H[8] = t1 + (int64_t)x[9] * (int64_t)x38[9];
  H[8] = H[8] + (int64_t)x2[0] * (int64_t)x[8];
  H[8] = H[8] + (int64_t)x2[1] * (int64_t)x2[7];
  H[8] = H[8] + (int64_t)x2[2] * (int64_t)x[6];
  H[8] = H[8] + (int64_t)x2[3] * (int64_t)x2[5];
  H[8] = H[8] + (int64_t)x[4] * (int64_t)x[4];
  t0 = H[8] >> 26;
  H[9] += t0;
#endif
}

TMED_HD void fe_sq1c_fused_x2(int64_t H0[10], int64_t H1[10], const int32_t a_x[10], const int32_t a_x2[10], const int32_t a_x19[10], const int32_t a_x38[10], const int32_t b_x[10], const int32_t b_x2[10], const int32_t b_x19[10], const int32_t b_x38[10]) {
  const int64_t b0 = (int64_t)1 << 25, b50 = (int64_t)1 << 50;
  int64_t t0_0, t0_1, t1_0, t1_1;
#if defined(__HIP_DEVICE_COMPILE__)
  asm(
      "v_mad_i64_i32 %0, vcc, %35, %46, %70\n"
      "v_mad_i64_i32 %12, vcc, %58, %69, %70\n"
      "v_mad_i64_i32 %1, vcc, %26, %46, %71\n"
      "v_mad_i64_i32 %0, vcc, %26, %45, %0\n"
      "v_mad_i64_i32 %12, vcc, %49, %68, %12\n"
      "v_mad_i64_i32 %13, vcc, %49, %69, %71\n"
      "v_mad_i64_i32 %0, vcc, %37, %44, %0\n"
      "v_mad_i64_i32 %12, vcc, %60, %67, %12\n"
      "v_mad_i64_i32 %1, vcc, %27, %45, %1\n"
      "v_mad_i64_i32 %0, vcc, %28, %43, %0\n"
      "v_mad_i64_i32 %12, vcc, %51, %66, %12\n"
      "v_mad_i64_i32 %13, vcc, %50, %68, %13\n"
      "v_mad_i64_i32 %0, vcc, %29, %42, %0\n"
      "v_mad_i64_i32 %1, vcc, %28, %44, %1\n"
      "v_mad_i64_i32 %12, vcc, %52, %65, %12\n"
      "v_mad_i64_i32 %13, vcc, %51, %67, %13\n"
      "v_mad_i64_i32 %0, vcc, %24, %24, %0\n"
      "v_mad_i64_i32 %1, vcc, %29, %43, %1\n"
      "v_mad_i64_i32 %12, vcc, %47, %47, %12\n"
      "v_mad_i64_i32 %13, vcc, %52, %66, %13\n"
      "v_mad_i64_i32 %1, vcc, %24, %35, %1\n"
      "v_ashrrev_i64 %10, 26, %0\n"
      "v_mad_i64_i32 %13, vcc, %47, %58, %13\n"
      "v_ashrrev_i64 %22, 26, %12\n"
      "v_lshl_add_u64 %1, %10, 0, %1\n"
// ... 51 lines not shown
      "v_mad_i64_i32 %5, vcc, %26, %37, %5\n"
      "v_ashrrev_i64 %10, 26, %4\n"
      "v_mad_i64_i32 %17, vcc, %49, %60, %17\n"
      "v_ashrrev_i64 %22, 26, %16\n"
      "v_lshl_add_u64 %5, %10, 0, %5\n"
      "v_mad_i64_i32 %7, vcc, %32, %46, %71\n"
      "v_lshl_add_u64 %17, %22, 0, %17\n"
      "v_ashrrev_i64 %11, 25, %5\n"
      "v_mad_i64_i32 %19, vcc, %55, %69, %71\n"
      "v_ashrrev_i64 %23, 25, %17\n"
      "v_mad_i64_i32 %6, vcc, %39, %46, %11\n"
      "v_mad_i64_i32 %7, vcc, %34, %31, %7\n"
      "v_mad_i64_i32 %18, vcc, %62, %69, %23\n"
      "v_mad_i64_i32 %6, vcc, %32, %41, %6\n"
      "v_mad_i64_i32 %19, vcc, %57, %54, %19\n"
      "v_mad_i64_i32 %18, vcc, %55, %64, %18\n"
      "v_mad_i64_i32 %6, vcc, %34, %30, %6\n"
      "v_mad_i64_i32 %7, vcc, %35, %30, %7\n"
      "v_mad_i64_i32 %18, vcc, %57, %53, %18\n"
      "v_mad_i64_i32 %6, vcc, %35, %38, %6\n"
      "v_mad_i64_i32 %19, vcc, %58, %53, %19\n"
      "v_mad_i64_i32 %18, vcc, %58, %61, %18\n"
      "v_mad_i64_i32 %6, vcc, %36, %28, %6\n"
      "v_mad_i64_i32 %7, vcc, %36, %29, %7\n"
      "v_mad_i64_i32 %18, vcc, %59, %51, %18\n"
      "v_mad_i64_i32 %6, vcc, %37, %27, %6\n"
      "v_mad_i64_i32 %19, vcc, %59, %52, %19\n"
      "v_mad_i64_i32 %18, vcc, %60, %50, %18\n"
      "v_mad_i64_i32 %7, vcc, %37, %28, %7\n"
      "v_ashrrev_i64 %10, 26, %6\n"
      "v_mad_i64_i32 %19, vcc, %60, %51, %19\n"
      "v_ashrrev_i64 %22, 26, %18\n"
      "v_lshl_add_u64 %7, %10, 0, %7\n"
      "v_mad_i64_i32 %9, vcc, %34, %33, 0\n"
      "v_lshl_add_u64 %19, %22, 0, %19\n"
      "v_ashrrev_i64 %11, 25, %7\n"
      "v_mad_i64_i32 %21, vcc, %57, %56, 0\n"
      "v_ashrrev_i64 %23, 25, %19\n"
      "v_mad_i64_i32 %8, vcc, %33, %46, %11\n"
      "v_mad_i64_i32 %9, vcc, %35, %32, %9\n"
      "v_mad_i64_i32 %20, vcc, %56, %69, %23\n"
      "v_mad_i64_i32 %8, vcc, %34, %32, %8\n"
      "v_mad_i64_i32 %21, vcc, %58, %55, %21\n"
      "v_mad_i64_i32 %20, vcc, %57, %55, %20\n"
      "v_mad_i64_i32 %8, vcc, %35, %39, %8\n"
      "v_mad_i64_i32 %9, vcc, %36, %31, %9\n"
      "v_mad_i64_i32 %20, vcc, %58, %62, %20\n"
      "v_mad_i64_i32 %8, vcc, %36, %30, %8\n"
      "v_mad_i64_i32 %21, vcc, %59, %54, %21\n"
      "v_mad_i64_i32 %20, vcc, %59, %53, %20\n"
      "v_mad_i64_i32 %8, vcc, %37, %38, %8\n"
      "v_mad_i64_i32 %9, vcc, %37, %30, %9\n"
      "v_mad_i64_i32 %20, vcc, %60, %61, %20\n"
      "v_mad_i64_i32 %8, vcc, %28, %28, %8\n"
      "v_mad_i64_i32 %21, vcc, %60, %53, %21\n"
      "v_mad_i64_i32 %20, vcc, %51, %51, %20\n"
      "v_mad_i64_i32 %9, vcc, %28, %38, %9\n"
      "v_ashrrev_i64 %10, 26, %8\n"
      "v_mad_i64_i32 %21, vcc, %51, %61, %21\n"
      "v_ashrrev_i64 %22, 26, %20\n"
      "v_lshl_add_u64 %9, %10, 0, %9\n"
      "v_lshl_add_u64 %21, %22, 0, %21\n"
      : "=&v"(H0[0]), "=&v"(H0[1]), "=&v"(H0[2]), "=&v"(H0[3]), "=&v"(H0[4]), "=&v"(H0[5]),
        "=&v"(H0[6]), "=&v"(H0[7]), "=&v"(H0[8]), "=&v"(H0[9]), "=&v"(t0_0), "=&v"(t0_1),
        "=&v"(H1[0]), "=&v"(H1[1]), "=&v"(H1[2]), "=&v"(H1[3]), "=&v"(H1[4]), "=&v"(H1[5]),
        "=&v"(H1[6]), "=&v"(H1[7]), "=&v"(H1[8]), "=&v"(H1[9]), "=&v"(t1_0), "=&v"(t1_1)
      : "v"(a_x[0]), "v"(a_x[1]), "v"(a_x[2]), "v"(a_x[3]), "v"(a_x[4]), "v"(a_x[5]),
        "v"(a_x[6]), "v"(a_x[7]), "v"(a_x[8]), "v"(a_x[9]), "v"(a_x2[0]), "v"(a_x2[1]),
        "v"(a_x2[2]), "v"(a_x2[3]), "v"(a_x2[5]), "v"(a_x2[7]), "v"(a_x19[6]), "v"(a_x19[8]),
        "v"(a_x38[5]), "v"(a_x38[6]), "v"(a_x38[7]), "v"(a_x38[8]), "v"(a_x38[9]), "v"(b_x[0]),
        "v"(b_x[1]), "v"(b_x[2]), "v"(b_x[3]), "v"(b_x[4]), "v"(b_x[5]), "v"(b_x[6]),
        "v"(b_x[7]), "v"(b_x[8]), "v"(b_x[9]), "v"(b_x2[0]), "v"(b_x2[1]), "v"(b_x2[2]),
        "v"(b_x2[3]), "v"(b_x2[5]), "v"(b_x2[7]), "v"(b_x19[6]), "v"(b_x19[8]), "v"(b_x38[5]),
        "v"(b_x38[6]), "v"(b_x38[7]), "v"(b_x38[8]), "v"(b_x38[9]), "s"(b0), "s"(b50)
      : "vcc");
#else
  H0[0] = b0 + (int64_t)a_x2[1] * (int64_t)a_x38[9];
  H1[0] = b0 + (int64_t)b_x2[1] * (int64_t)b_x38[9];
  H0[1] = b50 + (int64_t)a_x[2] * (int64_t)a_x38[9];
  H0[0] = H0[0] + (int64_t)a_x[2] * (int64_t)a_x38[8];
  H1[0] = H1[0] + (int64_t)b_x[2] * (int64_t)b_x38[8];
  H1[1] = b50 + (int64_t)b_x[2] * (int64_t)b_x38[9];
  H0[0] = H0[0] + (int64_t)a_x2[3] * (int64_t)a_x38[7];
  H1[0] = H1[0] + (int64_t)b_x2[3] * (int64_t)b_x38[7];
  H0[1] = H0[1] + (int64_t)a_x[3] * (int64_t)a_x38[8];
  H0[0] = H0[0] + (int64_t)a_x[4] * (int64_t)a_x38[6];
  H1[0] = H1[0] + (int64_t)b_x[4] * (int64_t)b_x38[6];
  H1[1] = H1[1] + (int64_t)b_x[3] * (int64_t)b_x38[8];
  H0[0] = H0[0] + (int64_t)a_x[5] * (int64_t)a_x38[5];
  H0[1] = H0[1] + (int64_t)a_x[4] * (int64_t)a_x38[7];
  H1[0] = H1[0] + (int64_t)b_x[5] * (int64_t)b_x38[5];
  H1[1] = H1[1] + (int64_t)b_x[4] * (int64_t)b_x38[7];
  H0[0] = H0[0] + (int64_t)a_x[0] * (int64_t)a_x[0];
  H0[1] = H0[1] + (int64_t)a_x[5] * (int64_t)a_x38[6];
  H1[0] = H1[0] + (int64_t)b_x[0] * (int64_t)b_x[0];
// ... 57 lines not shown
  H0[5] = H0[5] + (int64_t)a_x[2] * (int64_t)a_x2[3];
  t0_0 = H0[4] >> 26;
  H1[5] = H1[5] + (int64_t)b_x[2] * (int64_t)b_x2[3];
  t1_0 = H1[4] >> 26;
  H0[5] += t0_0;
  H0[7] = b50 + (int64_t)a_x[8] * (int64_t)a_x38[9];
  H1[5] += t1_0;
  t0_1 = H0[5] >> 25;
  H1[7] = b50 + (int64_t)b_x[8] * (int64_t)b_x38[9];
  t1_1 = H1[5] >> 25;
  H0[6] = t0_1 + (int64_t)a_x2[7] * (int64_t)a_x38[9];
  H0[7] = H0[7] + (int64_t)a_x2[0] * (int64_t)a_x[7];
  H1[6] = t1_1 + (int64_t)b_x2[7] * (int64_t)b_x38[9];
  H0[6] = H0[6] + (int64_t)a_x[8] * (int64_t)a_x19[8];
  H1[7] = H1[7] + (int64_t)b_x2[0] * (int64_t)b_x[7];
  H1[6] = H1[6] + (int64_t)b_x[8] * (int64_t)b_x19[8];
  H0[6] = H0[6] + (int64_t)a_x2[0] * (int64_t)a_x[6];
  H0[7] = H0[7] + (int64_t)a_x2[1] * (int64_t)a_x[6];
  H1[6] = H1[6] + (int64_t)b_x2[0] * (int64_t)b_x[6];
  H0[6] = H0[6] + (int64_t)a_x2[1] * (int64_t)a_x2[5];
  H1[7] = H1[7] + (int64_t)b_x2[1] * (int64_t)b_x[6];
  H1[6] = H1[6] + (int64_t)b_x2[1] * (int64_t)b_x2[5];
  H0[6] = H0[6] + (int64_t)a_x2[2] * (int64_t)a_x[4];
  H0[7] = H0[7] + (int64_t)a_x2[2] * (int64_t)a_x[5];
  H1[6] = H1[6] + (int64_t)b_x2[2] * (int64_t)b_x[4];
  H0[6] = H0[6] + (int64_t)a_x2[3] * (int64_t)a_x[3];
  H1[7] = H1[7] + (int64_t)b_x2[2] * (int64_t)b_x[5];
  H1[6] = H1[6] + (int64_t)b_x2[3] * (int64_t)b_x[3];
  H0[7] = H0[7] + (int64_t)a_x2[3] * (int64_t)a_x[4];
  t0_0 = H0[6] >> 26;
  H1[7] = H1[7] + (int64_t)b_x2[3] * (int64_t)b_x[4];
  t1_0 = H1[6] >> 26;
  H0[7] += t0_0;
  H0[9] = 0 + (int64_t)a_x2[0] * (int64_t)a_x[9];
  H1[7] += t1_0;
  t0_1 = H0[7] >> 25;
  H1[9] = 0 + (int64_t)b_x2[0] * (int64_t)b_x[9];
  t1_1 = H1[7] >> 25;
  H0[8] = t0_1 + (int64_t)a_x[9] * (int64_t)a_x38[9];
  H0[9] = H0[9] + (int64_t)a_x2[1] * (int64_t)a_x[8];
  H1[8] = t1_1 + (int64_t)b_x[9] * (int64_t)b_x38[9];
  H0[8] = H0[8] + (int64_t)a_x2[0] * (int64_t)a_x[8];
  H1[9] = H1[9] + (int64_t)b_x2[1] * (int64_t)b_x[8];
  H1[8] = H1[8] + (int64_t)b_x2[0] * (int64_t)b_x[8];
  H0[8] = H0[8] + (int64_t)a_x2[1] * (int64_t)a_x2[7];
  H0[9] = H0[9] + (int64_t)a_x2[2] * (int64_t)a_x[7];
  H1[8] = H1[8] + (int64_t)b_x2[1] * (int64_t)b_x2[7];
  H0[8] = H0[8] + (int64_t)a_x2[2] * (int64_t)a_x[6];
  H1[9] = H1[9] + (int64_t)b_x2[2] * (int64_t)b_x[7];
  H1[8] = H1[8] + (int64_t)b_x2[2] * (int64_t)b_x[6];
  H0[8] = H0[8] + (int64_t)a_x2[3] * (int64_t)a_x2[5];
  H0[9] = H0[9] + (int64_t)a_x2[3] * (int64_t)a_x[6];
  H1[8] = H1[8] + (int64_t)b_x2[3] * (int64_t)b_x2[5];
  H0[8] = H0[8] + (int64_t)a_x[4] * (int64_t)a_x[4];
  H1[9] = H1[9] + (int64_t)b_x2[3] * (int64_t)b_x[6];
  H1[8] = H1[8] + (int64_t)b_x[4] * (int64_t)b_x[4];
  H0[9] = H0[9] + (int64_t)a_x[4] * (int64_t)a_x2[5];
  t0_0 = H0[8] >> 26;
  H1[9] = H1[9] + (int64_t)b_x[4] * (int64_t)b_x2[5];
  t1_0 = H1[8] >> 26;
  H0[9] += t0_0;
  H1[9] += t1_0;
#endif
}
```

### tendermint-fork_amd/csrc/ge25519.h

```cpp
#pragma once
#include "fe25519.h"

namespace tmed {

struct ge_p2 { fe X, Y, Z; };
struct ge_p3 { fe X, Y, Z, T; };
struct ge_p1p1 { fe X, Y, Z, T; };
struct ge_cached { fe YpX, YmX, Z, T2d; };
struct ge_niels { fe YpX, YmX, XY2d; };

TMED_HD void ge_p2_0(ge_p2 &h) { fe_0(h.X); fe_1(h.Y); fe_1(h.Z); }
TMED_HD void ge_p3_0(ge_p3 &h) { fe_0(h.X); fe_1(h.Y); fe_1(h.Z); fe_0(h.T); }
TMED_HD void ge_cached_0(ge_cached &h) { fe_1(h.YpX); fe_1(h.YmX); fe_1(h.Z); fe_0(h.T2d); }
TMED_HD void ge_niels_0(ge_niels &h) { fe_1(h.YpX); fe_1(h.YmX); fe_0(h.XY2d); }

TMED_HD void ge_p1p1_to_p2(ge_p2 &r, const ge_p1p1 &p) {
  fe_mul_x2(r.X, p.X, p.T, r.Y, p.Z, p.Y);
  fe_mul(r.Z, p.Z, p.T);
}
TMED_HD void ge_p1p1_to_p3(ge_p3 &r, const ge_p1p1 &p) {
  fe_mul_x2(r.X, p.X, p.T, r.Y, p.Z, p.Y);
  fe_mul(r.Z, p.Z, p.T);
  fe_mul(r.T, p.X, p.Y);
}
// ... 64 lines not shown
  fe a, b, c, d, t, t2, qp, qm;
  fe_select(qp, q.YpX, q.YmX, neg);
  fe_select(qm, q.YmX, q.YpX, neg);
  fe_add(t, p.Y, p.X);
  fe_sub(t2, p.Y, p.X);
  fe_mul_x2(a, t, qp, b, t2, qm);
  fe_mul(c, q.XY2d, p.T);
  fe_neg(t, c); fe_select(c, c, t, neg);
  fe_add(d, p.Z, p.Z);
  fe_sub(r.X, a, b);
  fe_add(r.Y, a, b);
  fe_add(r.Z, d, c);
  fe_sub(r.T, d, c);
}

TMED_HD bool ge_frombytes_go(ge_p3 &h, const uint32_t w[8]) {
  fe y, u, v, v3, uv7, r, chk, t, one, d, sqrtm1;
  fe_const_d(d); fe_const_sqrtm1(sqrtm1); fe_1(one);
  fe_from_words(y, w);
  fe_sqc(u, y);
  fe_mul(v, u, d);
  fe_sub(u, u, one); fe_carry(u, u);
  fe_add(v, v, one); fe_carry(v, v);
  fe_sqc(t, v); fe_mul(v3, t, v);
  fe_sqc(t, v3); fe_mul(uv7, t, v);
  fe_mul(uv7, uv7, u);
  fe_pow22523(t, uv7);
  fe_mul(r, u, v3);
  fe_mul(r, r, t);
  fe_sqc(t, r); fe_mul(chk, v, t);
  fe uneg; fe_neg(uneg, u);
  const bool correct = fe_equal(chk, u);
  const bool flipped = fe_equal(chk, uneg);
  fe_mul(t, uneg, sqrtm1);
  const bool flipped_i = fe_equal(chk, t);
  fe_mul(t, r, sqrtm1);
  fe_select(r, r, t, flipped || flipped_i);
  fe_neg(t, r);
  fe_select(r, r, t, fe_isnegative(r));
  const bool ok = correct || flipped;
  fe_neg(t, r);
  fe_select(r, r, t, (w[7] >> 31) != 0);
  fe_copy(h.X, r); fe_copy(h.Y, y); fe_1(h.Z); fe_mul(h.T, r, y);
  if (!ok) ge_p3_0(h);
  return ok;
}

TMED_HD void ge_tobytes(uint32_t w[8], const fe &X, const fe &Y, const fe &Z) {
  fe zi, x, y;
  fe_invert(zi, Z);
  fe_mul(x, X, zi);
  fe_mul(y, Y, zi);
  fe_to_words(w, y);
  w[7] |= (uint32_t)fe_isnegative(x) << 31;
}

}
```

### tendermint-fork_amd/csrc/kernels.hip

```cpp
#include "kernels.h"
#include "verify_core.h"
#include "verify_hs.h"
#include "kernel_util.h"
#include "rows.h"
#include "votes_dev.h"

namespace tmed {

__device__ int4 kIdentityRow[8] = {{1, 0, 0, 0}, {0, 0, 0, 0}, {1, 0, 0, 0}, {0, 0, 0, 0},
                                          {1, 0, 0, 0}, {0, 0, 0, 0}, {0, 0, 0, 0}, {0, 0, 0, 0}};

__device__ __forceinline__ void slab_st(int4 *p, int4 v) { *p = v; }
__device__ __forceinline__ int4 slab_ld(const int4 *p) { return *p; }

template <int ROWS>
struct SlabTabN {
  int4 *base;
  uint32_t slot;

  __device__ __forceinline__ const int4 *row(int j) const {
    return j == 0 ? kIdentityRow : base + ((size_t)slot * ROWS + (j - 1)) * 8;
  }

  __device__ __forceinline__ void store(int j, const ge_cached &c) const {
// ... 337 lines not shown
  for (int j = 0; j < 10; j++) { A.X.v[j] = w[44 + j]; A.Y.v[j] = w[54 + j]; }
  if (!active) { fe_1(A.Y); fe_1(Ry); }
  fe_1(A.Z);
  fe_mul(A.T, A.X, A.Y);
  const int flags = w[41];
  int W = active ? (flags >> 8) : 29;
#pragma unroll
  for (int o = 32; o > 0; o >>= 1) {
    const int x = __shfl_xor(W, o);
    W = x > W ? x : W;
  }
  W = __builtin_amdgcn_readfirstlane(W);
  if (W < 29) W = 29;
  if (W > 64) W = 64;
  const uint32_t lane = threadIdx.x & 63u, wv = threadIdx.x >> 6;
  const uint32_t slot0 = blockIdx.x * blockDim.x + ((uint32_t)__builtin_amdgcn_readfirstlane((int)threadIdx.x) & ~63u);
  const HsDigitsDev ds{prep2, stride, slot0, active};
  const size_t hi = BB == 26 ? (size_t)kB26Entries * kCombEntryInt4 : (size_t)8 * kB16Entries * kCombEntryInt4;
  BPf<BB> bl{btab, sm.bl[wv], lane};
  BPf<BB> bh{btab + hi, sm.bh(wv), lane};
  bool id;
  if constexpr (BB == 26) {
    SlabLdsTabJ tj{slab + (size_t)blockIdx.x * blockDim.x * (kJointRows * 8), threadIdx.x, sm.pq + threadIdx.x};
    ge_p3 P, Q;
    hs_points(P, Q, (flags & 2) != 0, A, Rx, Ry);
    build_table_joint(tj, P, Q);
#pragma unroll
    for (int q = 3; q < 6; q++) {
      const int4 v = active ? prep2[(size_t)q * stride + slot0 + lane_fresh()] : make_int4(0, 0, 0, 0);
      w[4 * q] = v.x; w[4 * q + 1] = v.y; w[4 * q + 2] = v.z; w[4 * q + 3] = v.w;
    }
#pragma unroll
    for (int j = 0; j < 8; j++) er[j] = (uint32_t)w[13 + j];
    ge_p2 q;
    hs_straus_joint(q, ds, er, W, tj, bl, bh);
    if (zip215) p2_mul8(q);
    id = p2_is_identity(q);
  } else {
    SlabTabJ tj{slab, slot};
    id = verify_main_hsj(ds, (flags & 2) != 0, er, W, A, Rx, Ry, tj, bl, bh, zip215 != 0);
  }
  if (active) {
    const int4 v = prep2[(size_t)10 * stride + slot0 + lane_fresh()];
    out[base + (uint32_t)v.z] = ((v.y & 1) && id) ? 1 : 0;
  }
}

__global__ __launch_bounds__(kThreadsPerBlock) void window_stats_kernel(const int4 *__restrict__ prep2, uint32_t stride,
                                                                       uint32_t count, uint32_t *__restrict__ lane_hist,
                                                                       uint32_t *__restrict__ wave_hist) {
  __shared__ uint32_t lh[65], wh[65];
  for (uint32_t b = threadIdx.x; b < 65; b += blockDim.x) lh[b] = wh[b] = 0;
  __syncthreads();
  const uint32_t slot = blockIdx.x * blockDim.x + threadIdx.x;
  const bool active = slot < count;
  int W = active ? (prep2[(size_t)10 * stride + slot].y >> 8) : 0;
  if (W < 0 || W > 64) W = 64;
  if (active) atomicAdd(&lh[W], 1u);
  int m = W;
#pragma unroll
  for (int o = 32; o > 0; o >>= 1) {
    const int x = __shfl_xor(m, o);
    m = x > m ? x : m;
  }
  if ((threadIdx.x & 63u) == 0 && slot < count) atomicAdd(&wh[m], 1u);
  __syncthreads();
  for (uint32_t b = threadIdx.x; b < 65; b += blockDim.x) {
    if (lh[b]) atomicAdd(&lane_hist[b], lh[b]);
    if (wh[b]) atomicAdd(&wave_hist[b], wh[b]);
  }
// ... 823 lines not shown
```

### tendermint-fork_amd/csrc/verify_hs.h

```cpp
#pragma once
#include <math.h>

#include "verify_core.h"

namespace tmed {

TMED_HD void sc_const_8L(uint32_t n[8]) {
  const uint32_t c[8] = {0xe7ae9f68u, 0xc09318d2u, 0x17bce6b2u, 0xa6f7cef5u, 0u, 0u, 0u, 0x80000000u};
#pragma unroll
  for (int i = 0; i < 8; i++) n[i] = c[i];
}

TMED_HD int bitlen_words(const uint32_t *x, int n) {
  int b = 0;
#pragma unroll
  for (int i = 0; i < n; i++)
    if (x[i]) b = 32 * i + 32 - __builtin_clz(x[i]);
  return b;
}

TMED_HD double words_to_double(const uint32_t *x, int n) {
  double r = 0.0;
#pragma unroll
  for (int i = n - 1; i >= 0; i--) r = r * 4294967296.0 + (double)x[i];
// ... 342 lines not shown
      ge_p1p1_to_p3(r, t);
      tr.take(ca);
      ge_add_cached_pre(t, r, ca, dd < 0);
    }
    if (b26) {
      if (n == 0 || n == 13 || n == 26) hs_b26_add(t, r, n / 13 * 2, d26l, d26h, bl, bh);
    } else if ((n & 3) == 0 && n <= 28) {
      const int dl = (int)(el[3] >> 16) - 32768, dh = (int)(eh[3] >> 16) - 32768;
      words4_shl16(el);
      words4_shl16(eh);
      ge_p1p1_to_p3(r, t);
      bl.take(nb);
      const int nl = (int)(el[3] >> 16) - 32768;
      bl.prefetch(nl < 0 ? -nl : nl);
      niels_apply_sign(nb, dl < 0);
      ge_madd_niels(t, r, nb, false);
      ge_p1p1_to_p3(r, t);
      bh.take(nb);
      const int nh = (int)(eh[3] >> 16) - 32768;
      bh.prefetch(nh < 0 ? -nh : nh);
      niels_apply_sign(nb, dh < 0);
      ge_madd_niels(t, r, nb, false);
    }
    ge_p1p1_to_p2(q, t);
  }
  out = q;
}

TMED_HD void hs_split4(int D, int &h, int &l) {
  l = ((D + 2) & 3) - 2;
  h = (D - l) >> 2;
}

template <class DS, class TJ, class BL, class BH>
TMED_HD void hs_straus_joint(ge_p2 &out, const DS &ds, const uint32_t er[8], int W, TJ &tj, BL &bl, BH &bh) {
  constexpr bool b26 = BL::kBits == 26;
  static_assert(BL::kBits == 16 || BL::kBits == 26, "B windows of radix 2^16 or 2^26");
  uint32_t el[4] = {er[0], er[1], er[2], er[3]}, eh[4] = {er[4], er[5], er[6], er[7]};
  int d26l[5] = {0, 0, 0, 0, 0}, d26h[5] = {0, 0, 0, 0, 0};
  if (b26) {
    hs_b26_digits(d26l, d26h, er);
    bl.prefetch(d26l[4] < 0 ? -d26l[4] : d26l[4]);
  } else {
    const int dl = (int)(el[3] >> 16) - 32768, dh = (int)(eh[3] >> 16) - 32768;
    bl.prefetch(dl < 0 ? -dl : dl);
    bh.prefetch(dh < 0 ? -dh : dh);
  }
  ge_p2 q;
  ge_p1p1 t;
  ge_p3 r;
  ge_cached ca;
  ge_niels nb;
  uint32_t cw = ds.cword((W - 1) >> 3), dw = ds.dword((W - 1) >> 3), cwn = cw, dwn = dw;
  int ih = 0, il;
  {
    const int dc = hs_top_digit(cw, W < 64 ? ((W & 7) ? cw : ds.cword(W >> 3)) : 0u, W);
    const int dd = hs_top_digit(dw, W < 64 ? ((W & 7) ? dw : ds.dword(W >> 3)) : 0u, W);
    int hc, lc, hd, ld;
    hs_split4(dc, hc, lc);
    hs_split4(dd, hd, ld);
    const int c1 = hc < 2 ? hc : 2, d1 = hd < 2 ? hd : 2;
    tj.prefetch(joint_index(c1, d1), false);
    tj.take(ca);
    tj.prefetch(joint_index(hc - c1, hd - d1), false);
    ge_cached_to_p3(r, ca);
    tj.take(ca);
    il = joint_index(lc, ld);
    tj.prefetch(il < 0 ? -il : il, il < 0);
// ... 24 lines not shown
    tj.take(ca);
    const bool lneg = il < 0;
    if (n > 0) {
      cw = cwn;
      dw = dwn;
      const int sh = 4 * ((n - 1) & 7);
      int hc, lc, hd, ld;
      hs_split4((int)((cw >> sh) & 15u) - 8, hc, lc);
      hs_split4((int)((dw >> sh) & 15u) - 8, hd, ld);
      ih = joint_index(hc, hd);
      il = joint_index(lc, ld);
      tj.prefetch(ih < 0 ? -ih : ih, ih < 0);
    }
    ge_add_cached_pre(t, r, ca, lneg);
    if (b26) {
      if (n == 0 || n == 13 || n == 26) hs_b26_add(t, r, n / 13 * 2, d26l, d26h, bl, bh);
    } else if ((n & 3) == 0 && n <= 28) {
      const int dl = (int)(el[3] >> 16) - 32768, dh = (int)(eh[3] >> 16) - 32768;
      words4_shl16(el);
      words4_shl16(eh);
      ge_p1p1_to_p3(r, t);
      bl.take(nb);
      const int nl = (int)(el[3] >> 16) - 32768;
      bl.prefetch(nl < 0 ? -nl : nl);
      niels_apply_sign(nb, dl < 0);
      ge_madd_niels(t, r, nb, false);
      ge_p1p1_to_p3(r, t);
      bh.take(nb);
      const int nh = (int)(eh[3] >> 16) - 32768;
      bh.prefetch(nh < 0 ? -nh : nh);
      niels_apply_sign(nb, dh < 0);
      ge_madd_niels(t, r, nb, false);
    }
    ge_p1p1_to_p2(q, t);
  }
  out = q;
}

TMED_HD bool p2_is_identity(const ge_p2 &q) { return fe_iszero(q.X) && fe_equal(q.Y, q.Z) && !fe_iszero(q.Z); }

TMED_HD void p2_mul8(ge_p2 &q) {
  ge_p1p1 t;
#pragma unroll 1
  for (int i = 0; i < 3; i++) {
    ge_p2_dbl(t, q);
    ge_p1p1_to_p2(q, t);
  }
}

TMED_HD void hs_points(ge_p3 &P, ge_p3 &Q, bool dneg, const ge_p3 &A, const fe &Rx, const fe &Ry) {
  fe_neg(P.X, A.X);
  fe_copy(P.Y, A.Y);
  fe_1(P.Z);
  fe_neg(P.T, A.T);
  if (dneg) fe_copy(Q.X, Rx); else fe_neg(Q.X, Rx);
  fe_copy(Q.Y, Ry);
  fe_1(Q.Z);
  fe_mul(Q.T, Q.X, Q.Y);
}

template <class DS, class TJ, class BL, class BH>
TMED_HD bool verify_main_hsj(const DS &ds, bool dneg, const uint32_t er[8], int W, const ge_p3 &A, const fe &Rx,
                             const fe &Ry, TJ &tj, BL &bl, BH &bh, bool cofactor8 = false) {
  ge_p3 P, Q;
  hs_points(P, Q, dneg, A, Rx, Ry);
  build_table_joint(tj, P, Q);
  ge_p2 q;
  hs_straus_joint(q, ds, er, W, tj, bl, bh);
  if (cofactor8) p2_mul8(q);
  return p2_is_identity(q);
}

// ... 21 lines not shown
```

Baseline: 113.7 million verifies/s.

## Use unsigned-limb field ops in pow22523, reorder H9 accumulation, skip final p1p1 conversion

Adds an unsigned canonical-limb multiply and square path (fe_mul_uc/fe_sq_uc with a cheaper finalisation) and uses it for the whole fe_pow22523 chain in point decompression. Moves the H[9] accumulation in every fused mul/square so the carry from H[8] seeds it directly, which removes one add per multiply. Drops the extra sqrt(-1) check in decompression, and for the non-ZIP215 path tests identity directly on the completed point, skipping the last p1p1-to-p2 conversion. Together these reduce ALU work per verify, but they change the correctness logic of decompression and identity checks, and the unsigned limbs carry overflow-bound risk.

```diff
diff --git a/__graft_entry__.py b/__graft_entry__.py
--- a/__graft_entry__.py
+++ b/__graft_entry__.py
@@ -20,6 +20,7 @@
     subprocess.check_call(["make", "-j", jobs, "-C", PKG], env=env)
     subprocess.check_call(["make", "-s", "-C", os.path.join(ROOT, "oracle")])
     subprocess.check_call(["make", "-s", "-C", os.path.join(ROOT, "tests", "native")])
+    subprocess.check_call(["make", "-s", "-C", os.path.join(ROOT, "tests", "native"), "-f", "fe_uc.mk"])
     _paths()
     import tmed
     tmed.lib()
diff --git a/tendermint-fork_amd/csrc/fe25519.h b/tendermint-fork_amd/csrc/fe25519.h
--- a/tendermint-fork_amd/csrc/fe25519.h
+++ b/tendermint-fork_amd/csrc/fe25519.h
@@ -219,7 +219,76 @@
   fe_sqn(t, z250, 5); fe_mul(out, t, z11);
 }
 
+TMED_HD void fe_fused_fin_u(fe &h, const uint64_t H[10]) {
+  const uint64_t c9 = H[9] >> 25;
+  const uint64_t h0 = (uint64_t)((uint32_t)H[0] & 0x3ffffffu) + c9 * 19;
+  h.v[0] = (int32_t)((uint32_t)h0 & 0x3ffffffu);
+  h.v[1] = (int32_t)(((uint32_t)H[1] & 0x1ffffffu) + (uint32_t)(h0 >> 26));
+#pragma unroll
+  for (int k = 2; k < 10; k++) h.v[k] = (int32_t)((uint32_t)H[k] & ((k & 1) ? 0x1ffffffu : 0x3ffffffu));
+}
+
+TMED_HD void fe_to_uc(fe &h, const fe &f) {
+  uint32_t t[10];
+#pragma unroll
+  for (int i = 0; i < 10; i++)
+    t[i] = (uint32_t)f.v[i] + (i == 0 ? 0x7ffffdau : (i & 1) ? 0x3fffffeu : 0x7fffffeu);
+#pragma unroll
+  for (int i = 0; i < 9; i++) {
+    const int s = (i & 1) ? 25 : 26;
+    t[i + 1] += t[i] >> s;
+    t[i] &= (1u << s) - 1u;
+  }
+  t[0] += 19u * (t[9] >> 25);
+  t[9] &= 0x1ffffffu;
+  t[1] += t[0] >> 26;
+  t[0] &= 0x3ffffffu;
+#pragma unroll
+  for (int i = 0; i < 10; i++) h.v[i] = (int32_t)t[i];
+}
+
+TMED_HD void fe_mul_uc(fe &h, const fe &f, const fe &g) {
+  int32_t g19[10], f2[10];
+#pragma unroll
+  for (int j = 0; j < 10; j++) g19[j] = mul19(g.v[j]);
+#pragma unroll
+  for (int i = 0; i < 10; i++) f2[i] = dbl32(f.v[i]);
+  uint64_t acc[10];
+  fe_mul_uc_fused(acc, f.v, f2, g.v, g19);
+  fe_fused_fin_u(h, acc);
+}
+
+TMED_HD void fe_sq_uc(fe &h, const fe &f) {
+  const fe_premul_c p(f);
+  uint64_t acc[10];
+  fe_sq_uc_fused(acc, p.x, p.x2, p.x19, p.x38);
+  fe_fused_fin_u(h, acc);
+}
+
+TMED_HD void fe_sqn_uc(fe &h, const fe &f, int n) {
+  fe_sq_uc(h, f);
+#pragma unroll 1
+  for (int i = 1; i < n; i++) fe_sq_uc(h, h);
+}
+
 TMED_HD void fe_pow22523(fe &out, const fe &z) {
+  fe zu, z2, z9, z11, t, a, b, c;
+  fe_to_uc(zu, z);
+  fe_sq_uc(z2, zu);
+  fe_sqn_uc(t, z2, 2); fe_mul_uc(z9, t, zu);
+  fe_mul_uc(z11, z9, z2);
+  fe_sq_uc(t, z11); fe_mul_uc(a, t, z9);
+  fe_sqn_uc(t, a, 5); fe_mul_uc(b, t, a);
+  fe_sqn_uc(t, b, 10); fe_mul_uc(c, t, b);
+  fe_sqn_uc(t, c, 20); fe_mul_uc(t, t, c);
+  fe_sqn_uc(t, t, 10); fe_mul_uc(a, t, b);
+  fe_sqn_uc(t, a, 50); fe_mul_uc(b, t, a);
+  fe_sqn_uc(t, b, 100); fe_mul_uc(t, t, b);
+  fe_sqn_uc(t, t, 50); fe_mul_uc(t, t, a);
+  fe_sqn_uc(t, t, 2); fe_mul_uc(out, t, zu);
+}
+
+TMED_HD void fe_pow22523_signed(fe &out, const fe &z) {
   fe z250, z11, t;
   fe_pow250(z250, z11, z);
   fe_sqn(t, z250, 2); fe_mul(out, t, z);
diff --git a/tendermint-fork_amd/csrc/fe_cols.h b/tendermint-fork_amd/csrc/fe_cols.h
--- a/tendermint-fork_amd/csrc/fe_cols.h
+++ b/tendermint-fork_amd/csrc/fe_cols.h
@@ -86,25 +86,15 @@
       "v_mad_i64_i32 %6, vcc, %12, %33, %11\n"
       "v_mad_i64_i32 %7, vcc, %21, %44, %7\n"
       "v_mad_i64_i32 %6, vcc, %22, %32, %6\n"
-      "v_mad_i64_i32 %9, vcc, %12, %36, 0\n"
       "v_mad_i64_i32 %6, vcc, %14, %31, %6\n"
-      "v_mad_i64_i32 %9, vcc, %13, %35, %9\n"
       "v_mad_i64_i32 %6, vcc, %23, %30, %6\n"
-      "v_mad_i64_i32 %9, vcc, %14, %34, %9\n"
       "v_mad_i64_i32 %6, vcc, %16, %29, %6\n"
-      "v_mad_i64_i32 %9, vcc, %15, %33, %9\n"
       "v_mad_i64_i32 %6, vcc, %24, %28, %6\n"
-      "v_mad_i64_i32 %9, vcc, %16, %32, %9\n"
       "v_mad_i64_i32 %6, vcc, %18, %27, %6\n"
-      "v_mad_i64_i32 %9, vcc, %17, %31, %9\n"
       "v_mad_i64_i32 %6, vcc, %25, %45, %6\n"
-      "v_mad_i64_i32 %9, vcc, %18, %30, %9\n"
       "v_mad_i64_i32 %6, vcc, %20, %44, %6\n"
-      "v_mad_i64_i32 %9, vcc, %19, %29, %9\n"
       "v_mad_i64_i32 %6, vcc, %26, %43, %6\n"
-      "v_mad_i64_i32 %9, vcc, %20, %28, %9\n"
       "v_ashrrev_i64 %10, 26, %6\n"
-      "v_mad_i64_i32 %9, vcc, %21, %27, %9\n"
       "v_lshl_add_u64 %7, %10, 0, %7\n"
       "v_ashrrev_i64 %11, 25, %7\n"
       "v_mad_i64_i32 %8, vcc, %12, %35, %11\n"
@@ -118,7 +108,16 @@
       "v_mad_i64_i32 %8, vcc, %20, %27, %8\n"
       "v_mad_i64_i32 %8, vcc, %26, %45, %8\n"
       "v_ashrrev_i64 %10, 26, %8\n"
-      "v_lshl_add_u64 %9, %10, 0, %9\n"
+      "v_mad_i64_i32 %9, vcc, %12, %36, %10\n"
+      "v_mad_i64_i32 %9, vcc, %13, %35, %9\n"
+      "v_mad_i64_i32 %9, vcc, %14, %34, %9\n"
+      "v_mad_i64_i32 %9, vcc, %15, %33, %9\n"
+      "v_mad_i64_i32 %9, vcc, %16, %32, %9\n"
+      "v_mad_i64_i32 %9, vcc, %17, %31, %9\n"
+      "v_mad_i64_i32 %9, vcc, %18, %30, %9\n"
+      "v_mad_i64_i32 %9, vcc, %19, %29, %9\n"
+      "v_mad_i64_i32 %9, vcc, %20, %28, %9\n"
+      "v_mad_i64_i32 %9, vcc, %21, %27, %9\n"
       : "=&v"(H[0]), "=&v"(H[1]), "=&v"(H[2]), "=&v"(H[3]), "=&v"(H[4]), "=&v"(H[5]),
         "=&v"(H[6]), "=&v"(H[7]), "=&v"(H[8]), "=&v"(H[9]), "=&v"(t0), "=&v"(t1)
       : "v"(f[0]), "v"(f[1]), "v"(f[2]), "v"(f[3]), "v"(f[4]), "v"(f[5]),
@@ -210,25 +209,15 @@
   H[6] = t1 + (int64_t)f[0] * (int64_t)g[6];
   H[7] = H[7] + (int64_t)f[9] * (int64_t)g19[8];
   H[6] = H[6] + (int64_t)f2[1] * (int64_t)g[5];
-  H[9] = 0 + (int64_t)f[0] * (int64_t)g[9];
   H[6] = H[6] + (int64_t)f[2] * (int64_t)g[4];
-  H[9] = H[9] + (int64_t)f[1] * (int64_t)g[8];
   H[6] = H[6] + (int64_t)f2[3] * (int64_t)g[3];
-  H[9] = H[9] + (int64_t)f[2] * (int64_t)g[7];
   H[6] = H[6] + (int64_t)f[4] * (int64_t)g[2];
-  H[9] = H[9] + (int64_t)f[3] * (int64_t)g[6];
   H[6] = H[6] + (int64_t)f2[5] * (int64_t)g[1];
-  H[9] = H[9] + (int64_t)f[4] * (int64_t)g[5];
   H[6] = H[6] + (int64_t)f[6] * (int64_t)g[0];
-  H[9] = H[9] + (int64_t)f[5] * (int64_t)g[4];
   H[6] = H[6] + (int64_t)f2[7] * (int64_t)g19[9];
-  H[9] = H[9] + (int64_t)f[6] * (int64_t)g[3];
   H[6] = H[6] + (int64_t)f[8] * (int64_t)g19[8];
-  H[9] = H[9] + (int64_t)f[7] * (int64_t)g[2];
   H[6] = H[6] + (int64_t)f2[9] * (int64_t)g19[7];
-  H[9] = H[9] + (int64_t)f[8] * (int64_t)g[1];
   t0 = H[6] >> 26;
-  H[9] = H[9] + (int64_t)f[9] * (int64_t)g[0];
   H[7] += t0;
   t1 = H[7] >> 25;
   H[8] = t1 + (int64_t)f[0] * (int64_t)g[8];
@@ -242,7 +231,16 @@
   H[8] = H[8] + (int64_t)f[8] * (int64_t)g[0];
   H[8] = H[8] + (int64_t)f2[9] * (int64_t)g19[9];
   t0 = H[8] >> 26;
-  H[9] += t0;
+  H[9] = t0 + (int64_t)f[0] * (int64_t)g[9];
+  H[9] = H[9] + (int64_t)f[1] * (int64_t)g[8];
+  H[9] = H[9] + (int64_t)f[2] * (int64_t)g[7];
+  H[9] = H[9] + (int64_t)f[3] * (int64_t)g[6];
+  H[9] = H[9] + (int64_t)f[4] * (int64_t)g[5];
+  H[9] = H[9] + (int64_t)f[5] * (int64_t)g[4];
+  H[9] = H[9] + (int64_t)f[6] * (int64_t)g[3];
+  H[9] = H[9] + (int64_t)f[7] * (int64_t)g[2];
+  H[9] = H[9] + (int64_t)f[8] * (int64_t)g[1];
+  H[9] = H[9] + (int64_t)f[9] * (int64_t)g[0];
 #endif
 }
 
@@ -292,15 +290,10 @@
       "v_mad_i64_i32 %4, vcc, %28, %39, %4\n"
       "v_mad_i64_i32 %7, vcc, %25, %16, %7\n"
       "v_mad_i64_i32 %4, vcc, %29, %38, %4\n"
-      "v_mad_i64_i32 %9, vcc, %22, %21, 0\n"
       "v_mad_i64_i32 %4, vcc, %22, %16, %4\n"
-      "v_mad_i64_i32 %9, vcc, %23, %20, %9\n"
       "v_mad_i64_i32 %4, vcc, %32, %15, %4\n"
-      "v_mad_i64_i32 %9, vcc, %24, %19, %9\n"
       "v_mad_i64_i32 %4, vcc, %14, %14, %4\n"
-      "v_mad_i64_i32 %9, vcc, %25, %18, %9\n"
       "v_ashrrev_i64 %10, 26, %4\n"
-      "v_mad_i64_i32 %9, vcc, %26, %17, %9\n"
       "v_lshl_add_u64 %5, %10, 0, %5\n"
       "v_ashrrev_i64 %11, 25, %5\n"
       "v_mad_i64_i32 %6, vcc, %35, %40, %11\n"
@@ -319,7 +312,11 @@
       "v_mad_i64_i32 %8, vcc, %33, %17, %8\n"
       "v_mad_i64_i32 %8, vcc, %16, %16, %8\n"
       "v_ashrrev_i64 %10, 26, %8\n"
-      "v_lshl_add_u64 %9, %10, 0, %9\n"
+      "v_mad_i64_i32 %9, vcc, %22, %21, %10\n"
+      "v_mad_i64_i32 %9, vcc, %23, %20, %9\n"
+      "v_mad_i64_i32 %9, vcc, %24, %19, %9\n"
+      "v_mad_i64_i32 %9, vcc, %25, %18, %9\n"
+      "v_mad_i64_i32 %9, vcc, %26, %17, %9\n"
       : "=&v"(H[0]), "=&v"(H[1]), "=&v"(H[2]), "=&v"(H[3]), "=&v"(H[4]), "=&v"(H[5]),
         "=&v"(H[6]), "=&v"(H[7]), "=&v"(H[8]), "=&v"(H[9]), "=&v"(t0), "=&v"(t1)
       : "v"(x[0]), "v"(x[1]), "v"(x[2]), "v"(x[3]), "v"(x[4]), "v"(x[5]),
@@ -371,15 +368,10 @@
   H[4] = H[4] + (int64_t)x2[6] * (int64_t)x19[8];
   H[7] = H[7] + (int64_t)x2[3] * (int64_t)x[4];
   H[4] = H[4] + (int64_t)x2[7] * (int64_t)x19[7];
-  H[9] = 0 + (int64_t)x2[0] * (int64_t)x[9];
   H[4] = H[4] + (int64_t)x2[0] * (int64_t)x[4];
-  H[9] = H[9] + (int64_t)x2[1] * (int64_t)x[8];
   H[4] = H[4] + (int64_t)x4[1] * (int64_t)x[3];
-  H[9] = H[9] + (int64_t)x2[2] * (int64_t)x[7];
   H[4] = H[4] + (int64_t)x[2] * (int64_t)x[2];
-  H[9] = H[9] + (int64_t)x2[3] * (int64_t)x[6];
   t0 = H[4] >> 26;
-  H[9] = H[9] + (int64_t)x2[4] * (int64_t)x[5];
   H[5] += t0;
   t1 = H[5] >> 25;
   H[6] = t1 + (int64_t)x4[7] * (int64_t)x19[9];
@@ -398,7 +390,11 @@
   H[8] = H[8] + (int64_t)x4[3] * (int64_t)x[5];
   H[8] = H[8] + (int64_t)x[4] * (int64_t)x[4];
   t0 = H[8] >> 26;
-  H[9] += t0;
+  H[9] = t0 + (int64_t)x2[0] * (int64_t)x[9];
+  H[9] = H[9] + (int64_t)x2[1] * (int64_t)x[8];
+  H[9] = H[9] + (int64_t)x2[2] * (int64_t)x[7];
+  H[9] = H[9] + (int64_t)x2[3] * (int64_t)x[6];
+  H[9] = H[9] + (int64_t)x2[4] * (int64_t)x[5];
 #endif
 }
 
@@ -448,15 +444,10 @@
       "v_mad_i64_i32 %4, vcc, %24, %35, %4\n"
       "v_mad_i64_i32 %7, vcc, %29, %16, %7\n"
       "v_mad_i64_i32 %4, vcc, %25, %34, %4\n"
-      "v_mad_i64_i32 %9, vcc, %19, %27, 0\n"
       "v_mad_i64_i32 %4, vcc, %19, %22, %4\n"
-      "v_mad_i64_i32 %9, vcc, %28, %18, %9\n"
       "v_mad_i64_i32 %4, vcc, %28, %21, %4\n"
-      "v_mad_i64_i32 %9, vcc, %20, %25, %9\n"
       "v_mad_i64_i32 %4, vcc, %20, %14, %4\n"
-      "v_mad_i64_i32 %9, vcc, %29, %17, %9\n"
       "v_ashrrev_i64 %10, 26, %4\n"
-      "v_mad_i64_i32 %9, vcc, %22, %23, %9\n"
       "v_lshl_add_u64 %5, %10, 0, %5\n"
       "v_ashrrev_i64 %11, 25, %5\n"
       "v_mad_i64_i32 %6, vcc, %31, %36, %11\n"
@@ -475,7 +466,11 @@
       "v_mad_i64_i32 %8, vcc, %29, %23, %8\n"
       "v_mad_i64_i32 %8, vcc, %22, %16, %8\n"
       "v_ashrrev_i64 %10, 26, %8\n"
-      "v_lshl_add_u64 %9, %10, 0, %9\n"
+      "v_mad_i64_i32 %9, vcc, %19, %27, %10\n"
+      "v_mad_i64_i32 %9, vcc, %28, %18, %9\n"
+      "v_mad_i64_i32 %9, vcc, %20, %25, %9\n"
+      "v_mad_i64_i32 %9, vcc, %29, %17, %9\n"
+      "v_mad_i64_i32 %9, vcc, %22, %23, %9\n"
       : "=&v"(H[0]), "=&v"(H[1]), "=&v"(H[2]), "=&v"(H[3]), "=&v"(H[4]), "=&v"(H[5]),
         "=&v"(H[6]), "=&v"(H[7]), "=&v"(H[8]), "=&v"(H[9]), "=&v"(t0), "=&v"(t1)
       : "v"(x[0]), "v"(x[1]), "v"(x[2]), "v"(x[3]), "v"(x[4]), "v"(x[6]),
@@ -526,15 +521,10 @@
   H[4] = H[4] + (int64_t)x2[6] * (int64_t)x38[8];
   H[7] = H[7] + (int64_t)x4[3] * (int64_t)x[4];
   H[4] = H[4] + (int64_t)x2[7] * (int64_t)x38[7];
-  H[9] = 0 + (int64_t)x2[0] * (int64_t)x2[9];
   H[4] = H[4] + (int64_t)x2[0] * (int64_t)x2[4];
-  H[9] = H[9] + (int64_t)x4[1] * (int64_t)x[8];
   H[4] = H[4] + (int64_t)x4[1] * (int64_t)x2[3];
-  H[9] = H[9] + (int64_t)x2[2] * (int64_t)x2[7];
   H[4] = H[4] + (int64_t)x2[2] * (int64_t)x[2];
-  H[9] = H[9] + (int64_t)x4[3] * (int64_t)x[6];
   t0 = H[4] >> 26;
-  H[9] = H[9] + (int64_t)x2[4] * (int64_t)x2[5];
   H[5] += t0;
   t1 = H[5] >> 25;
   H[6] = t1 + (int64_t)x4[7] * (int64_t)x38[9];
@@ -553,7 +543,11 @@
   H[8] = H[8] + (int64_t)x4[3] * (int64_t)x2[5];
   H[8] = H[8] + (int64_t)x2[4] * (int64_t)x[4];
   t0 = H[8] >> 26;
-  H[9] += t0;
+  H[9] = t0 + (int64_t)x2[0] * (int64_t)x2[9];
+  H[9] = H[9] + (int64_t)x4[1] * (int64_t)x[8];
+  H[9] = H[9] + (int64_t)x2[2] * (int64_t)x2[7];
+  H[9] = H[9] + (int64_t)x4[3] * (int64_t)x[6];
+  H[9] = H[9] + (int64_t)x2[4] * (int64_t)x2[5];
 #endif
 }
 
@@ -1154,35 +1148,33 @@
       "v_mad_i64_i32 %19, vcc, %66, %57, %19\n"
       "v_ashrrev_i64 %22, 26, %18\n"
       "v_lshl_add_u64 %7, %10, 0, %7\n"
-      "v_mad_i64_i32 %9, vcc, %34, %33, 0\n"
       "v_lshl_add_u64 %19, %22, 0, %19\n"
       "v_ashrrev_i64 %11, 25, %7\n"
-      "v_mad_i64_i32 %21, vcc, %63, %62, 0\n"
       "v_ashrrev_i64 %23, 25, %19\n"
       "v_mad_i64_i32 %8, vcc, %43, %52, %11\n"
-      "v_mad_i64_i32 %9, vcc, %35, %32, %9\n"
       "v_mad_i64_i32 %20, vcc, %72, %81, %23\n"
       "v_mad_i64_i32 %8, vcc, %34, %32, %8\n"
-      "v_mad_i64_i32 %21, vcc, %64, %61, %21\n"
       "v_mad_i64_i32 %20, vcc, %63, %61, %20\n"
       "v_mad_i64_i32 %8, vcc, %44, %31, %8\n"
-      "v_mad_i64_i32 %9, vcc, %36, %31, %9\n"
       "v_mad_i64_i32 %20, vcc, %73, %60, %20\n"
       "v_mad_i64_i32 %8, vcc, %36, %30, %8\n"
-      "v_mad_i64_i32 %21, vcc, %65, %60, %21\n"
       "v_mad_i64_i32 %20, vcc, %65, %59, %20\n"
       "v_mad_i64_i32 %8, vcc, %45, %29, %8\n"
-      "v_mad_i64_i32 %9, vcc, %37, %30, %9\n"
       "v_mad_i64_i32 %20, vcc, %74, %58, %20\n"
       "v_mad_i64_i32 %8, vcc, %28, %28, %8\n"
+      "v_mad_i64_i32 %20, vcc, %57, %57, %20\n"
+      "v_ashrrev_i64 %10, 26, %8\n"
+      "v_ashrrev_i64 %22, 26, %20\n"
+      "v_mad_i64_i32 %9, vcc, %34, %33, %10\n"
+      "v_mad_i64_i32 %21, vcc, %63, %62, %22\n"
+      "v_mad_i64_i32 %9, vcc, %35, %32, %9\n"
+      "v_mad_i64_i32 %21, vcc, %64, %61, %21\n"
+      "v_mad_i64_i32 %9, vcc, %36, %31, %9\n"
+      "v_mad_i64_i32 %21, vcc, %65, %60, %21\n"
+      "v_mad_i64_i32 %9, vcc, %37, %30, %9\n"
       "v_mad_i64_i32 %21, vcc, %66, %59, %21\n"
-      "v_mad_i64_i32 %20, vcc, %57, %57, %20\n"
       "v_mad_i64_i32 %9, vcc, %38, %29, %9\n"
-      "v_ashrrev_i64 %10, 26, %8\n"
       "v_mad_i64_i32 %21, vcc, %67, %58, %21\n"
-      "v_ashrrev_i64 %22, 26, %20\n"
-      "v_lshl_add_u64 %9, %10, 0, %9\n"
-      "v_lshl_add_u64 %21, %22, 0, %21\n"
       : "=&v"(H0[0]), "=&v"(H0[1]), "=&v"(H0[2]), "=&v"(H0[3]), "=&v"(H0[4]), "=&v"(H0[5]),
         "=&v"(H0[6]), "=&v"(H0[7]), "=&v"(H0[8]), "=&v"(H0[9]), "=&v"(t0_0), "=&v"(t0_1),
         "=&v"(H1[0]), "=&v"(H1[1]), "=&v"(H1[2]), "=&v"(H1[3]), "=&v"(H1[4]), "=&v"(H1[5]),
@@ -1308,35 +1300,33 @@
   H1[7] = H1[7] + (int64_t)b_x2[3] * (int64_t)b_x[4];
   t1_0 = H1[6] >> 26;
   H0[7] += t0_0;
-  H0[9] = 0 + (int64_t)a_x2[0] * (int64_t)a_x[9];
   H1[7] += t1_0;
   t0_1 = H0[7] >> 25;
-  H1[9] = 0 + (int64_t)b_x2[0] * (int64_t)b_x[9];
   t1_1 = H1[7] >> 25;
   H0[8] = t0_1 + (int64_t)a_x2[9] * (int64_t)a_x19[9];
-  H0[9] = H0[9] + (int64_t)a_x2[1] * (int64_t)a_x[8];
   H1[8] = t1_1 + (int64_t)b_x2[9] * (int64_t)b_x19[9];
   H0[8] = H0[8] + (int64_t)a_x2[0] * (int64_t)a_x[8];
-  H1[9] = H1[9] + (int64_t)b_x2[1] * (int64_t)b_x[8];
   H1[8] = H1[8] + (int64_t)b_x2[0] * (int64_t)b_x[8];
   H0[8] = H0[8] + (int64_t)a_x4[1] * (int64_t)a_x[7];
-  H0[9] = H0[9] + (int64_t)a_x2[2] * (int64_t)a_x[7];
   H1[8] = H1[8] + (int64_t)b_x4[1] * (int64_t)b_x[7];
   H0[8] = H0[8] + (int64_t)a_x2[2] * (int64_t)a_x[6];
-  H1[9] = H1[9] + (int64_t)b_x2[2] * (int64_t)b_x[7];
   H1[8] = H1[8] + (int64_t)b_x2[2] * (int64_t)b_x[6];
   H0[8] = H0[8] + (int64_t)a_x4[3] * (int64_t)a_x[5];
-  H0[9] = H0[9] + (int64_t)a_x2[3] * (int64_t)a_x[6];
   H1[8] = H1[8] + (int64_t)b_x4[3] * (int64_t)b_x[5];
   H0[8] = H0[8] + (int64_t)a_x[4] * (int64_t)a_x[4];
+  H1[8] = H1[8] + (int64_t)b_x[4] * (int64_t)b_x[4];
+  t0_0 = H0[8] >> 26;
+  t1_0 = H1[8] >> 26;
+  H0[9] = t0_0 + (int64_t)a_x2[0] * (int64_t)a_x[9];
+  H1[9] = t1_0 + (int64_t)b_x2[0] * (int64_t)b_x[9];
+  H0[9] = H0[9] + (int64_t)a_x2[1] * (int64_t)a_x[8];
+  H1[9] = H1[9] + (int64_t)b_x2[1] * (int64_t)b_x[8];
+  H0[9] = H0[9] + (int64_t)a_x2[2] * (int64_t)a_x[7];
+  H1[9] = H1[9] + (int64_t)b_x2[2] * (int64_t)b_x[7];
+  H0[9] = H0[9] + (int64_t)a_x2[3] * (int64_t)a_x[6];
   H1[9] = H1[9] + (int64_t)b_x2[3] * (int64_t)b_x[6];
-  H1[8] = H1[8] + (int64_t)b_x[4] * (int64_t)b_x[4];
   H0[9] = H0[9] + (int64_t)a_x2[4] * (int64_t)a_x[5];
-  t0_0 = H0[8] >> 26;
   H1[9] = H1[9] + (int64_t)b_x2[4] * (int64_t)b_x[5];
-  t1_0 = H1[8] >> 26;
-  H0[9] += t0_0;
-  H1[9] += t1_0;
 #endif
 }
 
@@ -1454,35 +1444,33 @@
       "v_mad_i64_i32 %19, vcc, %62, %53, %19\n"
       "v_ashrrev_i64 %22, 26, %18\n"
       "v_lshl_add_u64 %7, %10, 0, %7\n"
-      "v_mad_i64_i32 %9, vcc, %31, %39, 0\n"
       "v_lshl_add_u64 %19, %22, 0, %19\n"
       "v_ashrrev_i64 %11, 25, %7\n"
-      "v_mad_i64_i32 %21, vcc, %59, %58, 0\n"
       "v_ashrrev_i64 %23, 25, %19\n"
       "v_mad_i64_i32 %8, vcc, %39, %48, %11\n"
-      "v_mad_i64_i32 %9, vcc, %40, %30, %9\n"
       "v_mad_i64_i32 %20, vcc, %68, %77, %23\n"
       "v_mad_i64_i32 %8, vcc, %31, %38, %8\n"
-      "v_mad_i64_i32 %21, vcc, %60, %57, %21\n"
       "v_mad_i64_i32 %20, vcc, %59, %57, %20\n"
       "v_mad_i64_i32 %8, vcc, %40, %37, %8\n"
-      "v_mad_i64_i32 %9, vcc, %32, %37, %9\n"
       "v_mad_i64_i32 %20, vcc, %69, %56, %20\n"
       "v_mad_i64_i32 %8, vcc, %32, %36, %8\n"
-      "v_mad_i64_i32 %21, vcc, %61, %56, %21\n"
       "v_mad_i64_i32 %20, vcc, %61, %55, %20\n"
       "v_mad_i64_i32 %8, vcc, %41, %35, %8\n"
-      "v_mad_i64_i32 %9, vcc, %41, %29, %9\n"
       "v_mad_i64_i32 %20, vcc, %70, %54, %20\n"
       "v_mad_i64_i32 %8, vcc, %34, %28, %8\n"
+      "v_mad_i64_i32 %20, vcc, %53, %53, %20\n"
+      "v_ashrrev_i64 %10, 26, %8\n"
+      "v_ashrrev_i64 %22, 26, %20\n"
+      "v_mad_i64_i32 %9, vcc, %31, %39, %10\n"
+      "v_mad_i64_i32 %21, vcc, %59, %58, %22\n"
+      "v_mad_i64_i32 %9, vcc, %40, %30, %9\n"
+      "v_mad_i64_i32 %21, vcc, %60, %57, %21\n"
+      "v_mad_i64_i32 %9, vcc, %32, %37, %9\n"
+      "v_mad_i64_i32 %21, vcc, %61, %56, %21\n"
+      "v_mad_i64_i32 %9, vcc, %41, %29, %9\n"
       "v_mad_i64_i32 %21, vcc, %62, %55, %21\n"
-      "v_mad_i64_i32 %20, vcc, %53, %53, %20\n"
       "v_mad_i64_i32 %9, vcc, %34, %35, %9\n"
-      "v_ashrrev_i64 %10, 26, %8\n"
       "v_mad_i64_i32 %21, vcc, %63, %54, %21\n"
-      "v_ashrrev_i64 %22, 26, %20\n"
-      "v_lshl_add_u64 %9, %10, 0, %9\n"
-      "v_lshl_add_u64 %21, %22, 0, %21\n"
       : "=&v"(H0[0]), "=&v"(H0[1]), "=&v"(H0[2]), "=&v"(H0[3]), "=&v"(H0[4]), "=&v"(H0[5]),
         "=&v"(H0[6]), "=&v"(H0[7]), "=&v"(H0[8]), "=&v"(H0[9]), "=&v"(t0_0), "=&v"(t0_1),
         "=&v"(H1[0]), "=&v"(H1[1]), "=&v"(H1[2]), "=&v"(H1[3]), "=&v"(H1[4]), "=&v"(H1[5]),
@@ -1608,35 +1596,33 @@
   H1[7] = H1[7] + (int64_t)b_x2[3] * (int64_t)b_x[4];
   t1_0 = H1[6] >> 26;
   H0[7] += t0_0;
-  H0[9] = 0 + (int64_t)a_x2[0] * (int64_t)a_x2[9];
   H1[7] += t1_0;
   t0_1 = H0[7] >> 25;
-  H1[9] = 0 + (int64_t)b_x2[0] * (int64_t)b_x[9];
   t1_1 = H1[7] >> 25;
   H0[8] = t0_1 + (int64_t)a_x2[9] * (int64_t)a_x38[9];
-  H0[9] = H0[9] + (int64_t)a_x4[1] * (int64_t)a_x[8];
   H1[8] = t1_1 + (int64_t)b_x2[9] * (int64_t)b_x19[9];
   H0[8] = H0[8] + (int64_t)a_x2[0] * (int64_t)a_x2[8];
-  H1[9] = H1[9] + (int64_t)b_x2[1] * (int64_t)b_x[8];
   H1[8] = H1[8] + (int64_t)b_x2[0] * (int64_t)b_x[8];
   H0[8] = H0[8] + (int64_t)a_x4[1] * (int64_t)a_x2[7];
-  H0[9] = H0[9] + (int64_t)a_x2[2] * (int64_t)a_x2[7];
   H1[8] = H1[8] + (int64_t)b_x4[1] * (int64_t)b_x[7];
   H0[8] = H0[8] + (int64_t)a_x2[2] * (int64_t)a_x2[6];
-  H1[9] = H1[9] + (int64_t)b_x2[2] * (int64_t)b_x[7];
   H1[8] = H1[8] + (int64_t)b_x2[2] * (int64_t)b_x[6];
   H0[8] = H0[8] + (int64_t)a_x4[3] * (int64_t)a_x2[5];
-  H0[9] = H0[9] + (int64_t)a_x4[3] * (int64_t)a_x[6];
   H1[8] = H1[8] + (int64_t)b_x4[3] * (int64_t)b_x[5];
   H0[8] = H0[8] + (int64_t)a_x2[4] * (int64_t)a_x[4];
+  H1[8] = H1[8] + (int64_t)b_x[4] * (int64_t)b_x[4];
+  t0_0 = H0[8] >> 26;
+  t1_0 = H1[8] >> 26;
+  H0[9] = t0_0 + (int64_t)a_x2[0] * (int64_t)a_x2[9];
+  H1[9] = t1_0 + (int64_t)b_x2[0] * (int64_t)b_x[9];
+  H0[9] = H0[9] + (int64_t)a_x4[1] * (int64_t)a_x[8];
+  H1[9] = H1[9] + (int64_t)b_x2[1] * (int64_t)b_x[8];
+  H0[9] = H0[9] + (int64_t)a_x2[2] * (int64_t)a_x2[7];
+  H1[9] = H1[9] + (int64_t)b_x2[2] * (int64_t)b_x[7];
+  H0[9] = H0[9] + (int64_t)a_x4[3] * (int64_t)a_x[6];
   H1[9] = H1[9] + (int64_t)b_x2[3] * (int64_t)b_x[6];
-  H1[8] = H1[8] + (int64_t)b_x[4] * (int64_t)b_x[4];
   H0[9] = H0[9] + (int64_t)a_x2[4] * (int64_t)a_x2[5];
-  t0_0 = H0[8] >> 26;
   H1[9] = H1[9] + (int64_t)b_x2[4] * (int64_t)b_x[5];
-  t1_0 = H1[8] >> 26;
-  H0[9] += t0_0;
-  H1[9] += t1_0;
 #endif
 }
 
@@ -1687,15 +1673,10 @@
       "v_mad_i64_i32 %4, vcc, %18, %33, %4\n"
       "v_mad_i64_i32 %7, vcc, %25, %16, %7\n"
       "v_mad_i64_i32 %4, vcc, %19, %32, %4\n"
-      "v_mad_i64_i32 %9, vcc, %22, %21, 0\n"
       "v_mad_i64_i32 %4, vcc, %22, %16, %4\n"
-      "v_mad_i64_i32 %9, vcc, %23, %20, %9\n"
       "v_mad_i64_i32 %4, vcc, %23, %25, %4\n"
-      "v_mad_i64_i32 %9, vcc, %24, %19, %9\n"
       "v_mad_i64_i32 %4, vcc, %14, %14, %4\n"
-      "v_mad_i64_i32 %9, vcc, %25, %18, %9\n"
       "v_ashrrev_i64 %10, 26, %4\n"
-      "v_mad_i64_i32 %9, vcc, %16, %26, %9\n"
       "v_lshl_add_u64 %5, %10, 0, %5\n"
       "v_ashrrev_i64 %11, 25, %5\n"
       "v_mad_i64_i32 %6, vcc, %27, %34, %11\n"
@@ -1714,7 +1695,11 @@
       "v_mad_i64_i32 %8, vcc, %25, %26, %8\n"
       "v_mad_i64_i32 %8, vcc, %16, %16, %8\n"
       "v_ashrrev_i64 %10, 26, %8\n"
-      "v_lshl_add_u64 %9, %10, 0, %9\n"
+      "v_mad_i64_i32 %9, vcc, %22, %21, %10\n"
+      "v_mad_i64_i32 %9, vcc, %23, %20, %9\n"
+      "v_mad_i64_i32 %9, vcc, %24, %19, %9\n"
+      "v_mad_i64_i32 %9, vcc, %25, %18, %9\n"
+      "v_mad_i64_i32 %9, vcc, %16, %26, %9\n"
       : "=&v"(H[0]), "=&v"(H[1]), "=&v"(H[2]), "=&v"(H[3]), "=&v"(H[4]), "=&v"(H[5]),
         "=&v"(H[6]), "=&v"(H[7]), "=&v"(H[8]), "=&v"(H[9]), "=&v"(t0), "=&v"(t1)
       : "v"(x[0]), "v"(x[1]), "v"(x[2]), "v"(x[3]), "v"(x[4]), "v"(x[5]),
@@ -1765,15 +1750,10 @@
   H[4] = H[4] + (int64_t)x[6] * (int64_t)x38[8];
   H[7] = H[7] + (int64_t)x2[3] * (int64_t)x[4];
   H[4] = H[4] + (int64_t)x[7] * (int64_t)x38[7];
-  H[9] = 0 + (int64_t)x2[0] * (int64_t)x[9];
   H[4] = H[4] + (int64_t)x2[0] * (int64_t)x[4];
-  H[9] = H[9] + (int64_t)x2[1] * (int64_t)x[8];
   H[4] = H[4] + (int64_t)x2[1] * (int64_t)x2[3];
-  H[9] = H[9] + (int64_t)x2[2] * (int64_t)x[7];
   H[4] = H[4] + (int64_t)x[2] * (int64_t)x[2];
-  H[9] = H[9] + (int64_t)x2[3] * (int64_t)x[6];
   t0 = H[4] >> 26;
-  H[9] = H[9] + (int64_t)x[4] * (int64_t)x2[5];
   H[5] += t0;
   t1 = H[5] >> 25;
   H[6] = t1 + (int64_t)x2[7] * (int64_t)x38[9];
@@ -1792,7 +1772,11 @@
   H[8] = H[8] + (int64_t)x2[3] * (int64_t)x2[5];
   H[8] = H[8] + (int64_t)x[4] * (int64_t)x[4];
   t0 = H[8] >> 26;
-  H[9] += t0;
+  H[9] = t0 + (int64_t)x2[0] * (int64_t)x[9];
+  H[9] = H[9] + (int64_t)x2[1] * (int64_t)x[8];
+  H[9] = H[9] + (int64_t)x2[2] * (int64_t)x[7];
+  H[9] = H[9] + (int64_t)x2[3] * (int64_t)x[6];
+  H[9] = H[9] + (int64_t)x[4] * (int64_t)x2[5];
 #endif
 }
 
@@ -1910,35 +1894,33 @@
       "v_mad_i64_i32 %19, vcc, %60, %51, %19\n"
       "v_ashrrev_i64 %22, 26, %18\n"
       "v_lshl_add_u64 %7, %10, 0, %7\n"
-      "v_mad_i64_i32 %9, vcc, %34, %33, 0\n"
       "v_lshl_add_u64 %19, %22, 0, %19\n"
       "v_ashrrev_i64 %11, 25, %7\n"
-      "v_mad_i64_i32 %21, vcc, %57, %56, 0\n"
       "v_ashrrev_i64 %23, 25, %19\n"
       "v_mad_i64_i32 %8, vcc, %33, %46, %11\n"
-      "v_mad_i64_i32 %9, vcc, %35, %32, %9\n"
       "v_mad_i64_i32 %20, vcc, %56, %69, %23\n"
       "v_mad_i64_i32 %8, vcc, %34, %32, %8\n"
-      "v_mad_i64_i32 %21, vcc, %58, %55, %21\n"
       "v_mad_i64_i32 %20, vcc, %57, %55, %20\n"
       "v_mad_i64_i32 %8, vcc, %35, %39, %8\n"
-      "v_mad_i64_i32 %9, vcc, %36, %31, %9\n"
       "v_mad_i64_i32 %20, vcc, %58, %62, %20\n"
       "v_mad_i64_i32 %8, vcc, %36, %30, %8\n"
-      "v_mad_i64_i32 %21, vcc, %59, %54, %21\n"
       "v_mad_i64_i32 %20, vcc, %59, %53, %20\n"
       "v_mad_i64_i32 %8, vcc, %37, %38, %8\n"
-      "v_mad_i64_i32 %9, vcc, %37, %30, %9\n"
       "v_mad_i64_i32 %20, vcc, %60, %61, %20\n"
       "v_mad_i64_i32 %8, vcc, %28, %28, %8\n"
+      "v_mad_i64_i32 %20, vcc, %51, %51, %20\n"
+      "v_ashrrev_i64 %10, 26, %8\n"
+      "v_ashrrev_i64 %22, 26, %20\n"
+      "v_mad_i64_i32 %9, vcc, %34, %33, %10\n"
+      "v_mad_i64_i32 %21, vcc, %57, %56, %22\n"
+      "v_mad_i64_i32 %9, vcc, %35, %32, %9\n"
+      "v_mad_i64_i32 %21, vcc, %58, %55, %21\n"
+      "v_mad_i64_i32 %9, vcc, %36, %31, %9\n"
+      "v_mad_i64_i32 %21, vcc, %59, %54, %21\n"
+      "v_mad_i64_i32 %9, vcc, %37, %30, %9\n"
       "v_mad_i64_i32 %21, vcc, %60, %53, %21\n"
-      "v_mad_i64_i32 %20, vcc, %51, %51, %20\n"
       "v_mad_i64_i32 %9, vcc, %28, %38, %9\n"
-      "v_ashrrev_i64 %10, 26, %8\n"
       "v_mad_i64_i32 %21, vcc, %51, %61, %21\n"
-      "v_ashrrev_i64 %22, 26, %20\n"
-      "v_lshl_add_u64 %9, %10, 0, %9\n"
-      "v_lshl_add_u64 %21, %22, 0, %21\n"
       : "=&v"(H0[0]), "=&v"(H0[1]), "=&v"(H0[2]), "=&v"(H0[3]), "=&v"(H0[4]), "=&v"(H0[5]),
         "=&v"(H0[6]), "=&v"(H0[7]), "=&v"(H0[8]), "=&v"(H0[9]), "=&v"(t0_0), "=&v"(t0_1),
         "=&v"(H1[0]), "=&v"(H1[1]), "=&v"(H1[2]), "=&v"(H1[3]), "=&v"(H1[4]), "=&v"(H1[5]),
@@ -2062,34 +2044,427 @@
   H1[7] = H1[7] + (int64_t)b_x2[3] * (int64_t)b_x[4];
   t1_0 = H1[6] >> 26;
   H0[7] += t0_0;
-  H0[9] = 0 + (int64_t)a_x2[0] * (int64_t)a_x[9];
   H1[7] += t1_0;
   t0_1 = H0[7] >> 25;
-  H1[9] = 0 + (int64_t)b_x2[0] * (int64_t)b_x[9];
   t1_1 = H1[7] >> 25;
   H0[8] = t0_1 + (int64_t)a_x[9] * (int64_t)a_x38[9];
-  H0[9] = H0[9] + (int64_t)a_x2[1] * (int64_t)a_x[8];
   H1[8] = t1_1 + (int64_t)b_x[9] * (int64_t)b_x38[9];
   H0[8] = H0[8] + (int64_t)a_x2[0] * (int64_t)a_x[8];
-  H1[9] = H1[9] + (int64_t)b_x2[1] * (int64_t)b_x[8];
   H1[8] = H1[8] + (int64_t)b_x2[0] * (int64_t)b_x[8];
   H0[8] = H0[8] + (int64_t)a_x2[1] * (int64_t)a_x2[7];
-  H0[9] = H0[9] + (int64_t)a_x2[2] * (int64_t)a_x[7];
   H1[8] = H1[8] + (int64_t)b_x2[1] * (int64_t)b_x2[7];
   H0[8] = H0[8] + (int64_t)a_x2[2] * (int64_t)a_x[6];
-  H1[9] = H1[9] + (int64_t)b_x2[2] * (int64_t)b_x[7];
   H1[8] = H1[8] + (int64_t)b_x2[2] * (int64_t)b_x[6];
   H0[8] = H0[8] + (int64_t)a_x2[3] * (int64_t)a_x2[5];
-  H0[9] = H0[9] + (int64_t)a_x2[3] * (int64_t)a_x[6];
   H1[8] = H1[8] + (int64_t)b_x2[3] * (int64_t)b_x2[5];
   H0[8] = H0[8] + (int64_t)a_x[4] * (int64_t)a_x[4];
+  H1[8] = H1[8] + (int64_t)b_x[4] * (int64_t)b_x[4];
+  t0_0 = H0[8] >> 26;
+  t1_0 = H1[8] >> 26;
+  H0[9] = t0_0 + (int64_t)a_x2[0] * (int64_t)a_x[9];
+  H1[9] = t1_0 + (int64_t)b_x2[0] * (int64_t)b_x[9];
+  H0[9] = H0[9] + (int64_t)a_x2[1] * (int64_t)a_x[8];
+  H1[9] = H1[9] + (int64_t)b_x2[1] * (int64_t)b_x[8];
+  H0[9] = H0[9] + (int64_t)a_x2[2] * (int64_t)a_x[7];
+  H1[9] = H1[9] + (int64_t)b_x2[2] * (int64_t)b_x[7];
+  H0[9] = H0[9] + (int64_t)a_x2[3] * (int64_t)a_x[6];
   H1[9] = H1[9] + (int64_t)b_x2[3] * (int64_t)b_x[6];
-  H1[8] = H1[8] + (int64_t)b_x[4] * (int64_t)b_x[4];
   H0[9] = H0[9] + (int64_t)a_x[4] * (int64_t)a_x2[5];
-  t0_0 = H0[8] >> 26;
   H1[9] = H1[9] + (int64_t)b_x[4] * (int64_t)b_x2[5];
-  t1_0 = H1[8] >> 26;
-  H0[9] += t0_0;
-  H1[9] += t1_0;
 #endif
 }
+
+
+TMED_HD void fe_sq_uc_fused(uint64_t H[10], const int32_t x[10], const int32_t x2[10], const int32_t x19[10], const int32_t x38[10]) {
+  uint64_t t0, t1;
+#if defined(__HIP_DEVICE_COMPILE__)
+  asm(
+      "v_mad_u64_u32 %0, vcc, %23, %34, 0\n"
+      "v_mad_u64_u32 %1, vcc, %14, %34, 0\n"
+      "v_mad_u64_u32 %0, vcc, %14, %33, %0\n"
+      "v_mad_u64_u32 %1, vcc, %15, %33, %1\n"
+      "v_mad_u64_u32 %0, vcc, %25, %32, %0\n"
+      "v_mad_u64_u32 %1, vcc, %16, %32, %1\n"
+      "v_mad_u64_u32 %0, vcc, %16, %31, %0\n"
+      "v_mad_u64_u32 %1, vcc, %17, %31, %1\n"
+      "v_mad_u64_u32 %0, vcc, %17, %30, %0\n"
+      "v_mad_u64_u32 %1, vcc, %12, %23, %1\n"
+      "v_mad_u64_u32 %0, vcc, %12, %12, %0\n"
+      "v_mad_u64_u32 %3, vcc, %16, %34, 0\n"
+      "v_lshrrev_b64 %10, 26, %0\n"
+      "v_mad_u64_u32 %3, vcc, %17, %33, %3\n"
+      "v_lshl_add_u64 %1, %10, 0, %1\n"
+      "v_mad_u64_u32 %3, vcc, %18, %32, %3\n"
+      "v_lshrrev_b64 %11, 25, %1\n"
+      "v_mad_u64_u32 %3, vcc, %22, %15, %3\n"
+      "v_mad_u64_u32 %2, vcc, %25, %34, %11\n"
+      "v_mad_u64_u32 %3, vcc, %23, %14, %3\n"
+      "v_mad_u64_u32 %2, vcc, %16, %33, %2\n"
+      "v_mad_u64_u32 %5, vcc, %18, %34, 0\n"
+      "v_mad_u64_u32 %2, vcc, %26, %32, %2\n"
+      "v_mad_u64_u32 %5, vcc, %19, %33, %5\n"
+      "v_mad_u64_u32 %2, vcc, %18, %28, %2\n"
+      "v_mad_u64_u32 %5, vcc, %22, %17, %5\n"
+      "v_mad_u64_u32 %2, vcc, %22, %14, %2\n"
+      "v_mad_u64_u32 %5, vcc, %23, %16, %5\n"
+      "v_mad_u64_u32 %2, vcc, %23, %13, %2\n"
+      "v_mad_u64_u32 %5, vcc, %14, %25, %5\n"
+      "v_lshrrev_b64 %10, 26, %2\n"
+      "v_mad_u64_u32 %7, vcc, %20, %34, 0\n"
+      "v_lshl_add_u64 %3, %10, 0, %3\n"
+      "v_mad_u64_u32 %7, vcc, %22, %19, %7\n"
+      "v_lshrrev_b64 %11, 25, %3\n"
+      "v_mad_u64_u32 %7, vcc, %23, %18, %7\n"
+      "v_mad_u64_u32 %4, vcc, %26, %34, %11\n"
+      "v_mad_u64_u32 %7, vcc, %24, %17, %7\n"
+      "v_mad_u64_u32 %4, vcc, %18, %33, %4\n"
+      "v_mad_u64_u32 %7, vcc, %25, %16, %7\n"
+      "v_mad_u64_u32 %4, vcc, %19, %32, %4\n"
+      "v_mad_u64_u32 %4, vcc, %22, %16, %4\n"
+      "v_mad_u64_u32 %4, vcc, %23, %25, %4\n"
+      "v_mad_u64_u32 %4, vcc, %14, %14, %4\n"
+      "v_lshrrev_b64 %10, 26, %4\n"
+      "v_lshl_add_u64 %5, %10, 0, %5\n"
+      "v_lshrrev_b64 %11, 25, %5\n"
+      "v_mad_u64_u32 %6, vcc, %27, %34, %11\n"
+      "v_mad_u64_u32 %6, vcc, %20, %29, %6\n"
+      "v_mad_u64_u32 %6, vcc, %22, %18, %6\n"
+      "v_mad_u64_u32 %6, vcc, %23, %26, %6\n"
+      "v_mad_u64_u32 %6, vcc, %24, %16, %6\n"
+      "v_mad_u64_u32 %6, vcc, %25, %15, %6\n"
+      "v_lshrrev_b64 %10, 26, %6\n"
+      "v_lshl_add_u64 %7, %10, 0, %7\n"
+      "v_lshrrev_b64 %11, 25, %7\n"
+      "v_mad_u64_u32 %8, vcc, %21, %34, %11\n"
+      "v_mad_u64_u32 %8, vcc, %22, %20, %8\n"
+      "v_mad_u64_u32 %8, vcc, %23, %27, %8\n"
+      "v_mad_u64_u32 %8, vcc, %24, %18, %8\n"
+      "v_mad_u64_u32 %8, vcc, %25, %26, %8\n"
+      "v_mad_u64_u32 %8, vcc, %16, %16, %8\n"
+      "v_lshrrev_b64 %10, 26, %8\n"
+      "v_mad_u64_u32 %9, vcc, %22, %21, %10\n"
+      "v_mad_u64_u32 %9, vcc, %23, %20, %9\n"
+      "v_mad_u64_u32 %9, vcc, %24, %19, %9\n"
+      "v_mad_u64_u32 %9, vcc, %25, %18, %9\n"
+      "v_mad_u64_u32 %9, vcc, %16, %26, %9\n"
+      : "=&v"(H[0]), "=&v"(H[1]), "=&v"(H[2]), "=&v"(H[3]), "=&v"(H[4]), "=&v"(H[5]),
+        "=&v"(H[6]), "=&v"(H[7]), "=&v"(H[8]), "=&v"(H[9]), "=&v"(t0), "=&v"(t1)
+      : "v"(x[0]), "v"(x[1]), "v"(x[2]), "v"(x[3]), "v"(x[4]), "v"(x[5]),
+        "v"(x[6]), "v"(x[7]), "v"(x[8]), "v"(x[9]), "v"(x2[0]), "v"(x2[1]),
+        "v"(x2[2]), "v"(x2[3]), "v"(x2[5]), "v"(x2[7]), "v"(x19[6]), "v"(x19[8]),
+        "v"(x38[5]), "v"(x38[6]), "v"(x38[7]), "v"(x38[8]), "v"(x38[9])
+      : "vcc");
+#else
+  H[0] = 0 + (uint64_t)(uint32_t)x2[1] * (uint64_t)(uint32_t)x38[9];
+  H[1] = 0 + (uint64_t)(uint32_t)x[2] * (uint64_t)(uint32_t)x38[9];
+  H[0] = H[0] + (uint64_t)(uint32_t)x[2] * (uint64_t)(uint32_t)x38[8];
+  H[1] = H[1] + (uint64_t)(uint32_t)x[3] * (uint64_t)(uint32_t)x38[8];
+  H[0] = H[0] + (uint64_t)(uint32_t)x2[3] * (uint64_t)(uint32_t)x38[7];
+  H[1] = H[1] + (uint64_t)(uint32_t)x[4] * (uint64_t)(uint32_t)x38[7];
+  H[0] = H[0] + (uint64_t)(uint32_t)x[4] * (uint64_t)(uint32_t)x38[6];
+  H[1] = H[1] + (uint64_t)(uint32_t)x[5] * (uint64_t)(uint32_t)x38[6];
+  H[0] = H[0] + (uint64_t)(uint32_t)x[5] * (uint64_t)(uint32_t)x38[5];
+  H[1] = H[1] + (uint64_t)(uint32_t)x[0] * (uint64_t)(uint32_t)x2[1];
+  H[0] = H[0] + (uint64_t)(uint32_t)x[0] * (uint64_t)(uint32_t)x[0];
+  H[3] = 0 + (uint64_t)(uint32_t)x[4] * (uint64_t)(uint32_t)x38[9];
+  t0 = H[0] >> 26;
+  H[3] = H[3] + (uint64_t)(uint32_t)x[5] * (uint64_t)(uint32_t)x38[8];
+  H[1] += t0;
+  H[3] = H[3] + (uint64_t)(uint32_t)x[6] * (uint64_t)(uint32_t)x38[7];
+  t1 = H[1] >> 25;
+  H[3] = H[3] + (uint64_t)(uint32_t)x2[0] * (uint64_t)(uint32_t)x[3];
+  H[2] = t1 + (uint64_t)(uint32_t)x2[3] * (uint64_t)(uint32_t)x38[9];
+  H[3] = H[3] + (uint64_t)(uint32_t)x2[1] * (uint64_t)(uint32_t)x[2];
+  H[2] = H[2] + (uint64_t)(uint32_t)x[4] * (uint64_t)(uint32_t)x38[8];
+  H[5] = 0 + (uint64_t)(uint32_t)x[6] * (uint64_t)(uint32_t)x38[9];
+  H[2] = H[2] + (uint64_t)(uint32_t)x2[5] * (uint64_t)(uint32_t)x38[7];
+  H[5] = H[5] + (uint64_t)(uint32_t)x[7] * (uint64_t)(uint32_t)x38[8];
+  H[2] = H[2] + (uint64_t)(uint32_t)x[6] * (uint64_t)(uint32_t)x19[6];
+  H[5] = H[5] + (uint64_t)(uint32_t)x2[0] * (uint64_t)(uint32_t)x[5];
+  H[2] = H[2] + (uint64_t)(uint32_t)x2[0] * (uint64_t)(uint32_t)x[2];
+  H[5] = H[5] + (uint64_t)(uint32_t)x2[1] * (uint64_t)(uint32_t)x[4];
+  H[2] = H[2] + (uint64_t)(uint32_t)x2[1] * (uint64_t)(uint32_t)x[1];
+  H[5] = H[5] + (uint64_t)(uint32_t)x[2] * (uint64_t)(uint32_t)x2[3];
+  t0 = H[2] >> 26;
+  H[7] = 0 + (uint64_t)(uint32_t)x[8] * (uint64_t)(uint32_t)x38[9];
+  H[3] += t0;
+  H[7] = H[7] + (uint64_t)(uint32_t)x2[0] * (uint64_t)(uint32_t)x[7];
+  t1 = H[3] >> 25;
+  H[7] = H[7] + (uint64_t)(uint32_t)x2[1] * (uint64_t)(uint32_t)x[6];
+  H[4] = t1 + (uint64_t)(uint32_t)x2[5] * (uint64_t)(uint32_t)x38[9];
+  H[7] = H[7] + (uint64_t)(uint32_t)x2[2] * (uint64_t)(uint32_t)x[5];
+  H[4] = H[4] + (uint64_t)(uint32_t)x[6] * (uint64_t)(uint32_t)x38[8];
+  H[7] = H[7] + (uint64_t)(uint32_t)x2[3] * (uint64_t)(uint32_t)x[4];
+  H[4] = H[4] + (uint64_t)(uint32_t)x[7] * (uint64_t)(uint32_t)x38[7];
+  H[4] = H[4] + (uint64_t)(uint32_t)x2[0] * (uint64_t)(uint32_t)x[4];
+  H[4] = H[4] + (uint64_t)(uint32_t)x2[1] * (uint64_t)(uint32_t)x2[3];
+  H[4] = H[4] + (uint64_t)(uint32_t)x[2] * (uint64_t)(uint32_t)x[2];
+  t0 = H[4] >> 26;
+  H[5] += t0;
+  t1 = H[5] >> 25;
+  H[6] = t1 + (uint64_t)(uint32_t)x2[7] * (uint64_t)(uint32_t)x38[9];
+  H[6] = H[6] + (uint64_t)(uint32_t)x[8] * (uint64_t)(uint32_t)x19[8];
+  H[6] = H[6] + (uint64_t)(uint32_t)x2[0] * (uint64_t)(uint32_t)x[6];
+  H[6] = H[6] + (uint64_t)(uint32_t)x2[1] * (uint64_t)(uint32_t)x2[5];
+  H[6] = H[6] + (uint64_t)(uint32_t)x2[2] * (uint64_t)(uint32_t)x[4];
+  H[6] = H[6] + (uint64_t)(uint32_t)x2[3] * (uint64_t)(uint32_t)x[3];
+  t0 = H[6] >> 26;
+  H[7] += t0;
+  t1 = H[7] >> 25;
+  H[8] = t1 + (uint64_t)(uint32_t)x[9] * (uint64_t)(uint32_t)x38[9];
+  H[8] = H[8] + (uint64_t)(uint32_t)x2[0] * (uint64_t)(uint32_t)x[8];
+  H[8] = H[8] + (uint64_t)(uint32_t)x2[1] * (uint64_t)(uint32_t)x2[7];
+  H[8] = H[8] + (uint64_t)(uint32_t)x2[2] * (uint64_t)(uint32_t)x[6];
+  H[8] = H[8] + (uint64_t)(uint32_t)x2[3] * (uint64_t)(uint32_t)x2[5];
+  H[8] = H[8] + (uint64_t)(uint32_t)x[4] * (uint64_t)(uint32_t)x[4];
+  t0 = H[8] >> 26;
+  H[9] = t0 + (uint64_t)(uint32_t)x2[0] * (uint64_t)(uint32_t)x[9];
+  H[9] = H[9] + (uint64_t)(uint32_t)x2[1] * (uint64_t)(uint32_t)x[8];
+  H[9] = H[9] + (uint64_t)(uint32_t)x2[2] * (uint64_t)(uint32_t)x[7];
+  H[9] = H[9] + (uint64_t)(uint32_t)x2[3] * (uint64_t)(uint32_t)x[6];
+  H[9] = H[9] + (uint64_t)(uint32_t)x[4] * (uint64_t)(uint32_t)x2[5];
+#endif
+}
+
+TMED_HD void fe_mul_uc_fused(uint64_t H[10], const int32_t f[10], const int32_t f2[10], const int32_t g[10], const int32_t g19[10]) {
+  uint64_t t0, t1;
+#if defined(__HIP_DEVICE_COMPILE__)
+  asm(
+      "v_mad_u64_u32 %0, vcc, %12, %27, 0\n"
+      "v_mad_u64_u32 %1, vcc, %12, %28, 0\n"
+      "v_mad_u64_u32 %0, vcc, %22, %45, %0\n"
+      "v_mad_u64_u32 %1, vcc, %13, %27, %1\n"
+      "v_mad_u64_u32 %0, vcc, %14, %44, %0\n"
+      "v_mad_u64_u32 %1, vcc, %14, %45, %1\n"
+      "v_mad_u64_u32 %0, vcc, %23, %43, %0\n"
+      "v_mad_u64_u32 %1, vcc, %15, %44, %1\n"
+      "v_mad_u64_u32 %0, vcc, %16, %42, %0\n"
+      "v_mad_u64_u32 %1, vcc, %16, %43, %1\n"
+      "v_mad_u64_u32 %0, vcc, %24, %41, %0\n"
+      "v_mad_u64_u32 %1, vcc, %17, %42, %1\n"
+      "v_mad_u64_u32 %0, vcc, %18, %40, %0\n"
+      "v_mad_u64_u32 %1, vcc, %18, %41, %1\n"
+      "v_mad_u64_u32 %0, vcc, %25, %39, %0\n"
+      "v_mad_u64_u32 %1, vcc, %19, %40, %1\n"
+      "v_mad_u64_u32 %0, vcc, %20, %38, %0\n"
+      "v_mad_u64_u32 %1, vcc, %20, %39, %1\n"
+      "v_mad_u64_u32 %0, vcc, %26, %37, %0\n"
+      "v_mad_u64_u32 %1, vcc, %21, %38, %1\n"
+      "v_lshrrev_b64 %10, 26, %0\n"
+      "v_mad_u64_u32 %3, vcc, %12, %30, 0\n"
+      "v_lshl_add_u64 %1, %10, 0, %1\n"
+      "v_mad_u64_u32 %3, vcc, %13, %29, %3\n"
+      "v_lshrrev_b64 %11, 25, %1\n"
+      "v_mad_u64_u32 %3, vcc, %14, %28, %3\n"
+      "v_mad_u64_u32 %2, vcc, %12, %29, %11\n"
+      "v_mad_u64_u32 %3, vcc, %15, %27, %3\n"
+      "v_mad_u64_u32 %2, vcc, %22, %28, %2\n"
+      "v_mad_u64_u32 %3, vcc, %16, %45, %3\n"
+      "v_mad_u64_u32 %2, vcc, %14, %27, %2\n"
+      "v_mad_u64_u32 %3, vcc, %17, %44, %3\n"
+      "v_mad_u64_u32 %2, vcc, %23, %45, %2\n"
+      "v_mad_u64_u32 %3, vcc, %18, %43, %3\n"
+      "v_mad_u64_u32 %2, vcc, %16, %44, %2\n"
+      "v_mad_u64_u32 %3, vcc, %19, %42, %3\n"
+      "v_mad_u64_u32 %2, vcc, %24, %43, %2\n"
+      "v_mad_u64_u32 %3, vcc, %20, %41, %3\n"
+      "v_mad_u64_u32 %2, vcc, %18, %42, %2\n"
+      "v_mad_u64_u32 %3, vcc, %21, %40, %3\n"
+      "v_mad_u64_u32 %2, vcc, %25, %41, %2\n"
+      "v_mad_u64_u32 %5, vcc, %12, %32, 0\n"
+      "v_mad_u64_u32 %2, vcc, %20, %40, %2\n"
+      "v_mad_u64_u32 %5, vcc, %13, %31, %5\n"
+      "v_mad_u64_u32 %2, vcc, %26, %39, %2\n"
+      "v_mad_u64_u32 %5, vcc, %14, %30, %5\n"
+      "v_lshrrev_b64 %10, 26, %2\n"
+      "v_mad_u64_u32 %5, vcc, %15, %29, %5\n"
+      "v_lshl_add_u64 %3, %10, 0, %3\n"
+      "v_mad_u64_u32 %5, vcc, %16, %28, %5\n"
+      "v_lshrrev_b64 %11, 25, %3\n"
+      "v_mad_u64_u32 %5, vcc, %17, %27, %5\n"
+      "v_mad_u64_u32 %4, vcc, %12, %31, %11\n"
+      "v_mad_u64_u32 %5, vcc, %18, %45, %5\n"
+      "v_mad_u64_u32 %4, vcc, %22, %30, %4\n"
+      "v_mad_u64_u32 %5, vcc, %19, %44, %5\n"
+      "v_mad_u64_u32 %4, vcc, %14, %29, %4\n"
+      "v_mad_u64_u32 %5, vcc, %20, %43, %5\n"
+      "v_mad_u64_u32 %4, vcc, %23, %28, %4\n"
+      "v_mad_u64_u32 %5, vcc, %21, %42, %5\n"
+      "v_mad_u64_u32 %4, vcc, %16, %27, %4\n"
+      "v_mad_u64_u32 %7, vcc, %12, %34, 0\n"
+      "v_mad_u64_u32 %4, vcc, %24, %45, %4\n"
+      "v_mad_u64_u32 %7, vcc, %13, %33, %7\n"
+      "v_mad_u64_u32 %4, vcc, %18, %44, %4\n"
+      "v_mad_u64_u32 %7, vcc, %14, %32, %7\n"
+      "v_mad_u64_u32 %4, vcc, %25, %43, %4\n"
+      "v_mad_u64_u32 %7, vcc, %15, %31, %7\n"
+      "v_mad_u64_u32 %4, vcc, %20, %42, %4\n"
+      "v_mad_u64_u32 %7, vcc, %16, %30, %7\n"
+      "v_mad_u64_u32 %4, vcc, %26, %41, %4\n"
+      "v_mad_u64_u32 %7, vcc, %17, %29, %7\n"
+      "v_lshrrev_b64 %10, 26, %4\n"
+      "v_mad_u64_u32 %7, vcc, %18, %28, %7\n"
+      "v_lshl_add_u64 %5, %10, 0, %5\n"
+      "v_mad_u64_u32 %7, vcc, %19, %27, %7\n"
+      "v_lshrrev_b64 %11, 25, %5\n"
+      "v_mad_u64_u32 %7, vcc, %20, %45, %7\n"
+      "v_mad_u64_u32 %6, vcc, %12, %33, %11\n"
+      "v_mad_u64_u32 %7, vcc, %21, %44, %7\n"
+      "v_mad_u64_u32 %6, vcc, %22, %32, %6\n"
+      "v_mad_u64_u32 %6, vcc, %14, %31, %6\n"
+      "v_mad_u64_u32 %6, vcc, %23, %30, %6\n"
+      "v_mad_u64_u32 %6, vcc, %16, %29, %6\n"
+      "v_mad_u64_u32 %6, vcc, %24, %28, %6\n"
+      "v_mad_u64_u32 %6, vcc, %18, %27, %6\n"
+      "v_mad_u64_u32 %6, vcc, %25, %45, %6\n"
+      "v_mad_u64_u32 %6, vcc, %20, %44, %6\n"
+      "v_mad_u64_u32 %6, vcc, %26, %43, %6\n"
+      "v_lshrrev_b64 %10, 26, %6\n"
+      "v_lshl_add_u64 %7, %10, 0, %7\n"
+      "v_lshrrev_b64 %11, 25, %7\n"
+      "v_mad_u64_u32 %8, vcc, %12, %35, %11\n"
+      "v_mad_u64_u32 %8, vcc, %22, %34, %8\n"
+      "v_mad_u64_u32 %8, vcc, %14, %33, %8\n"
+      "v_mad_u64_u32 %8, vcc, %23, %32, %8\n"
+      "v_mad_u64_u32 %8, vcc, %16, %31, %8\n"
+      "v_mad_u64_u32 %8, vcc, %24, %30, %8\n"
+      "v_mad_u64_u32 %8, vcc, %18, %29, %8\n"
+      "v_mad_u64_u32 %8, vcc, %25, %28, %8\n"
+      "v_mad_u64_u32 %8, vcc, %20, %27, %8\n"
+      "v_mad_u64_u32 %8, vcc, %26, %45, %8\n"
+      "v_lshrrev_b64 %10, 26, %8\n"
+      "v_mad_u64_u32 %9, vcc, %12, %36, %10\n"
+      "v_mad_u64_u32 %9, vcc, %13, %35, %9\n"
+      "v_mad_u64_u32 %9, vcc, %14, %34, %9\n"
+      "v_mad_u64_u32 %9, vcc, %15, %33, %9\n"
+      "v_mad_u64_u32 %9, vcc, %16, %32, %9\n"
+      "v_mad_u64_u32 %9, vcc, %17, %31, %9\n"
+      "v_mad_u64_u32 %9, vcc, %18, %30, %9\n"
+      "v_mad_u64_u32 %9, vcc, %19, %29, %9\n"
+      "v_mad_u64_u32 %9, vcc, %20, %28, %9\n"
+      "v_mad_u64_u32 %9, vcc, %21, %27, %9\n"
+      : "=&v"(H[0]), "=&v"(H[1]), "=&v"(H[2]), "=&v"(H[3]), "=&v"(H[4]), "=&v"(H[5]),
+        "=&v"(H[6]), "=&v"(H[7]), "=&v"(H[8]), "=&v"(H[9]), "=&v"(t0), "=&v"(t1)
+      : "v"(f[0]), "v"(f[1]), "v"(f[2]), "v"(f[3]), "v"(f[4]), "v"(f[5]),
+        "v"(f[6]), "v"(f[7]), "v"(f[8]), "v"(f[9]), "v"(f2[1]), "v"(f2[3]),
+        "v"(f2[5]), "v"(f2[7]), "v"(f2[9]), "v"(g[0]), "v"(g[1]), "v"(g[2]),
+        "v"(g[3]), "v"(g[4]), "v"(g[5]), "v"(g[6]), "v"(g[7]), "v"(g[8]),
+        "v"(g[9]), "v"(g19[1]), "v"(g19[2]), "v"(g19[3]), "v"(g19[4]), "v"(g19[5]),
+        "v"(g19[6]), "v"(g19[7]), "v"(g19[8]), "v"(g19[9])
+      : "vcc");
+#else
+  H[0] = 0 + (uint64_t)(uint32_t)f[0] * (uint64_t)(uint32_t)g[0];
+  H[1] = 0 + (uint64_t)(uint32_t)f[0] * (uint64_t)(uint32_t)g[1];
+  H[0] = H[0] + (uint64_t)(uint32_t)f2[1] * (uint64_t)(uint32_t)g19[9];
+  H[1] = H[1] + (uint64_t)(uint32_t)f[1] * (uint64_t)(uint32_t)g[0];
+  H[0] = H[0] + (uint64_t)(uint32_t)f[2] * (uint64_t)(uint32_t)g19[8];
+  H[1] = H[1] + (uint64_t)(uint32_t)f[2] * (uint64_t)(uint32_t)g19[9];
+  H[0] = H[0] + (uint64_t)(uint32_t)f2[3] * (uint64_t)(uint32_t)g19[7];
+  H[1] = H[1] + (uint64_t)(uint32_t)f[3] * (uint64_t)(uint32_t)g19[8];
+  H[0] = H[0] + (uint64_t)(uint32_t)f[4] * (uint64_t)(uint32_t)g19[6];
+  H[1] = H[1] + (uint64_t)(uint32_t)f[4] * (uint64_t)(uint32_t)g19[7];
+  H[0] = H[0] + (uint64_t)(uint32_t)f2[5] * (uint64_t)(uint32_t)g19[5];
+  H[1] = H[1] + (uint64_t)(uint32_t)f[5] * (uint64_t)(uint32_t)g19[6];
+  H[0] = H[0] + (uint64_t)(uint32_t)f[6] * (uint64_t)(uint32_t)g19[4];
+  H[1] = H[1] + (uint64_t)(uint32_t)f[6] * (uint64_t)(uint32_t)g19[5];
+  H[0] = H[0] + (uint64_t)(uint32_t)f2[7] * (uint64_t)(uint32_t)g19[3];
+  H[1] = H[1] + (uint64_t)(uint32_t)f[7] * (uint64_t)(uint32_t)g19[4];
+  H[0] = H[0] + (uint64_t)(uint32_t)f[8] * (uint64_t)(uint32_t)g19[2];
+  H[1] = H[1] + (uint64_t)(uint32_t)f[8] * (uint64_t)(uint32_t)g19[3];
+  H[0] = H[0] + (uint64_t)(uint32_t)f2[9] * (uint64_t)(uint32_t)g19[1];
+  H[1] = H[1] + (uint64_t)(uint32_t)f[9] * (uint64_t)(uint32_t)g19[2];
+  t0 = H[0] >> 26;
+  H[3] = 0 + (uint64_t)(uint32_t)f[0] * (uint64_t)(uint32_t)g[3];
+  H[1] += t0;
+  H[3] = H[3] + (uint64_t)(uint32_t)f[1] * (uint64_t)(uint32_t)g[2];
+  t1 = H[1] >> 25;
+  H[3] = H[3] + (uint64_t)(uint32_t)f[2] * (uint64_t)(uint32_t)g[1];
+  H[2] = t1 + (uint64_t)(uint32_t)f[0] * (uint64_t)(uint32_t)g[2];
+  H[3] = H[3] + (uint64_t)(uint32_t)f[3] * (uint64_t)(uint32_t)g[0];
+  H[2] = H[2] + (uint64_t)(uint32_t)f2[1] * (uint64_t)(uint32_t)g[1];
+  H[3] = H[3] + (uint64_t)(uint32_t)f[4] * (uint64_t)(uint32_t)g19[9];
+  H[2] = H[2] + (uint64_t)(uint32_t)f[2] * (uint64_t)(uint32_t)g[0];
+  H[3] = H[3] + (uint64_t)(uint32_t)f[5] * (uint64_t)(uint32_t)g19[8];
+  H[2] = H[2] + (uint64_t)(uint32_t)f2[3] * (uint64_t)(uint32_t)g19[9];
+  H[3] = H[3] + (uint64_t)(uint32_t)f[6] * (uint64_t)(uint32_t)g19[7];
+  H[2] = H[2] + (uint64_t)(uint32_t)f[4] * (uint64_t)(uint32_t)g19[8];
+  H[3] = H[3] + (uint64_t)(uint32_t)f[7] * (uint64_t)(uint32_t)g19[6];
+  H[2] = H[2] + (uint64_t)(uint32_t)f2[5] * (uint64_t)(uint32_t)g19[7];
+  H[3] = H[3] + (uint64_t)(uint32_t)f[8] * (uint64_t)(uint32_t)g19[5];
+  H[2] = H[2] + (uint64_t)(uint32_t)f[6] * (uint64_t)(uint32_t)g19[6];
+  H[3] = H[3] + (uint64_t)(uint32_t)f[9] * (uint64_t)(uint32_t)g19[4];
+  H[2] = H[2] + (uint64_t)(uint32_t)f2[7] * (uint64_t)(uint32_t)g19[5];
+  H[5] = 0 + (uint64_t)(uint32_t)f[0] * (uint64_t)(uint32_t)g[5];
+  H[2] = H[2] + (uint64_t)(uint32_t)f[8] * (uint64_t)(uint32_t)g19[4];
+  H[5] = H[5] + (uint64_t)(uint32_t)f[1] * (uint64_t)(uint32_t)g[4];
+  H[2] = H[2] + (uint64_t)(uint32_t)f2[9] * (uint64_t)(uint32_t)g19[3];
+  H[5] = H[5] + (uint64_t)(uint32_t)f[2] * (uint64_t)(uint32_t)g[3];
+  t0 = H[2] >> 26;
+  H[5] = H[5] + (uint64_t)(uint32_t)f[3] * (uint64_t)(uint32_t)g[2];
+  H[3] += t0;
+  H[5] = H[5] + (uint64_t)(uint32_t)f[4] * (uint64_t)(uint32_t)g[1];
+  t1 = H[3] >> 25;
+  H[5] = H[5] + (uint64_t)(uint32_t)f[5] * (uint64_t)(uint32_t)g[0];
+  H[4] = t1 + (uint64_t)(uint32_t)f[0] * (uint64_t)(uint32_t)g[4];
+  H[5] = H[5] + (uint64_t)(uint32_t)f[6] * (uint64_t)(uint32_t)g19[9];
+  H[4] = H[4] + (uint64_t)(uint32_t)f2[1] * (uint64_t)(uint32_t)g[3];
+  H[5] = H[5] + (uint64_t)(uint32_t)f[7] * (uint64_t)(uint32_t)g19[8];
+  H[4] = H[4] + (uint64_t)(uint32_t)f[2] * (uint64_t)(uint32_t)g[2];
+  H[5] = H[5] + (uint64_t)(uint32_t)f[8] * (uint64_t)(uint32_t)g19[7];
+  H[4] = H[4] + (uint64_t)(uint32_t)f2[3] * (uint64_t)(uint32_t)g[1];
+  H[5] = H[5] + (uint64_t)(uint32_t)f[9] * (uint64_t)(uint32_t)g19[6];
+  H[4] = H[4] + (uint64_t)(uint32_t)f[4] * (uint64_t)(uint32_t)g[0];
+  H[7] = 0 + (uint64_t)(uint32_t)f[0] * (uint64_t)(uint32_t)g[7];
+  H[4] = H[4] + (uint64_t)(uint32_t)f2[5] * (uint64_t)(uint32_t)g19[9];
+  H[7] = H[7] + (uint64_t)(uint32_t)f[1] * (uint64_t)(uint32_t)g[6];
+  H[4] = H[4] + (uint64_t)(uint32_t)f[6] * (uint64_t)(uint32_t)g19[8];
+  H[7] = H[7] + (uint64_t)(uint32_t)f[2] * (uint64_t)(uint32_t)g[5];
+  H[4] = H[4] + (uint64_t)(uint32_t)f2[7] * (uint64_t)(uint32_t)g19[7];
+  H[7] = H[7] + (uint64_t)(uint32_t)f[3] * (uint64_t)(uint32_t)g[4];
+  H[4] = H[4] + (uint64_t)(uint32_t)f[8] * (uint64_t)(uint32_t)g19[6];
+  H[7] = H[7] + (uint64_t)(uint32_t)f[4] * (uint64_t)(uint32_t)g[3];
+  H[4] = H[4] + (uint64_t)(uint32_t)f2[9] * (uint64_t)(uint32_t)g19[5];
+  H[7] = H[7] + (uint64_t)(uint32_t)f[5] * (uint64_t)(uint32_t)g[2];
+  t0 = H[4] >> 26;
+  H[7] = H[7] + (uint64_t)(uint32_t)f[6] * (uint64_t)(uint32_t)g[1];
+  H[5] += t0;
+  H[7] = H[7] + (uint64_t)(uint32_t)f[7] * (uint64_t)(uint32_t)g[0];
+  t1 = H[5] >> 25;
+  H[7] = H[7] + (uint64_t)(uint32_t)f[8] * (uint64_t)(uint32_t)g19[9];
+  H[6] = t1 + (uint64_t)(uint32_t)f[0] * (uint64_t)(uint32_t)g[6];
+  H[7] = H[7] + (uint64_t)(uint32_t)f[9] * (uint64_t)(uint32_t)g19[8];
+  H[6] = H[6] + (uint64_t)(uint32_t)f2[1] * (uint64_t)(uint32_t)g[5];
+  H[6] = H[6] + (uint64_t)(uint32_t)f[2] * (uint64_t)(uint32_t)g[4];
+  H[6] = H[6] + (uint64_t)(uint32_t)f2[3] * (uint64_t)(uint32_t)g[3];
+  H[6] = H[6] + (uint64_t)(uint32_t)f[4] * (uint64_t)(uint32_t)g[2];
+  H[6] = H[6] + (uint64_t)(uint32_t)f2[5] * (uint64_t)(uint32_t)g[1];
+  H[6] = H[6] + (uint64_t)(uint32_t)f[6] * (uint64_t)(uint32_t)g[0];
+  H[6] = H[6] + (uint64_t)(uint32_t)f2[7] * (uint64_t)(uint32_t)g19[9];
+  H[6] = H[6] + (uint64_t)(uint32_t)f[8] * (uint64_t)(uint32_t)g19[8];
+  H[6] = H[6] + (uint64_t)(uint32_t)f2[9] * (uint64_t)(uint32_t)g19[7];
+  t0 = H[6] >> 26;
+  H[7] += t0;
+  t1 = H[7] >> 25;
+  H[8] = t1 + (uint64_t)(uint32_t)f[0] * (uint64_t)(uint32_t)g[8];
+  H[8] = H[8] + (uint64_t)(uint32_t)f2[1] * (uint64_t)(uint32_t)g[7];
+  H[8] = H[8] + (uint64_t)(uint32_t)f[2] * (uint64_t)(uint32_t)g[6];
+  H[8] = H[8] + (uint64_t)(uint32_t)f2[3] * (uint64_t)(uint32_t)g[5];
+  H[8] = H[8] + (uint64_t)(uint32_t)f[4] * (uint64_t)(uint32_t)g[4];
+  H[8] = H[8] + (uint64_t)(uint32_t)f2[5] * (uint64_t)(uint32_t)g[3];
+  H[8] = H[8] + (uint64_t)(uint32_t)f[6] * (uint64_t)(uint32_t)g[2];
+  H[8] = H[8] + (uint64_t)(uint32_t)f2[7] * (uint64_t)(uint32_t)g[1];
+  H[8] = H[8] + (uint64_t)(uint32_t)f[8] * (uint64_t)(uint32_t)g[0];
+  H[8] = H[8] + (uint64_t)(uint32_t)f2[9] * (uint64_t)(uint32_t)g19[9];
+  t0 = H[8] >> 26;
+  H[9] = t0 + (uint64_t)(uint32_t)f[0] * (uint64_t)(uint32_t)g[9];
+  H[9] = H[9] + (uint64_t)(uint32_t)f[1] * (uint64_t)(uint32_t)g[8];
+  H[9] = H[9] + (uint64_t)(uint32_t)f[2] * (uint64_t)(uint32_t)g[7];
+  H[9] = H[9] + (uint64_t)(uint32_t)f[3] * (uint64_t)(uint32_t)g[6];
+  H[9] = H[9] + (uint64_t)(uint32_t)f[4] * (uint64_t)(uint32_t)g[5];
+  H[9] = H[9] + (uint64_t)(uint32_t)f[5] * (uint64_t)(uint32_t)g[4];
+  H[9] = H[9] + (uint64_t)(uint32_t)f[6] * (uint64_t)(uint32_t)g[3];
+  H[9] = H[9] + (uint64_t)(uint32_t)f[7] * (uint64_t)(uint32_t)g[2];
+  H[9] = H[9] + (uint64_t)(uint32_t)f[8] * (uint64_t)(uint32_t)g[1];
+  H[9] = H[9] + (uint64_t)(uint32_t)f[9] * (uint64_t)(uint32_t)g[0];
+#endif
+}
diff --git a/tendermint-fork_amd/csrc/ge25519.h b/tendermint-fork_amd/csrc/ge25519.h
--- a/tendermint-fork_amd/csrc/ge25519.h
+++ b/tendermint-fork_amd/csrc/ge25519.h
@@ -120,10 +120,8 @@
   fe uneg; fe_neg(uneg, u);
   const bool correct = fe_equal(chk, u);
   const bool flipped = fe_equal(chk, uneg);
-  fe_mul(t, uneg, sqrtm1);
-  const bool flipped_i = fe_equal(chk, t);
   fe_mul(t, r, sqrtm1);
-  fe_select(r, r, t, flipped || flipped_i);
+  fe_select(r, r, t, flipped);
   fe_neg(t, r);
   fe_select(r, r, t, fe_isnegative(r));
   const bool ok = correct || flipped;
diff --git a/tendermint-fork_amd/csrc/kernels.hip b/tendermint-fork_amd/csrc/kernels.hip
--- a/tendermint-fork_amd/csrc/kernels.hip
+++ b/tendermint-fork_amd/csrc/kernels.hip
@@ -393,10 +393,16 @@
     }
 #pragma unroll
     for (int j = 0; j < 8; j++) er[j] = (uint32_t)w[13 + j];
-    ge_p2 q;
-    hs_straus_joint(q, ds, er, W, tj, bl, bh);
-    if (zip215) p2_mul8(q);
-    id = p2_is_identity(q);
+    ge_p1p1 t;
+    hs_straus_joint_completed(t, ds, er, W, tj, bl, bh);
+    if (zip215) {
+      ge_p2 q;
+      ge_p1p1_to_p2(q, t);
+      p2_mul8(q);
+      id = p2_is_identity(q);
+    } else {
+      id = p1p1_is_identity(t);
+    }
   } else {
     SlabTabJ tj{slab, slot};
     id = verify_main_hsj(ds, (flags & 2) != 0, er, W, A, Rx, Ry, tj, bl, bh, zip215 != 0);
diff --git a/tendermint-fork_amd/csrc/verify_hs.h b/tendermint-fork_amd/csrc/verify_hs.h
--- a/tendermint-fork_amd/csrc/verify_hs.h
+++ b/tendermint-fork_amd/csrc/verify_hs.h
@@ -398,8 +398,9 @@
   h = (D - l) >> 2;
 }
 
-template <class DS, class TJ, class BL, class BH>
-TMED_HD void hs_straus_joint(ge_p2 &out, const DS &ds, const uint32_t er[8], int W, TJ &tj, BL &bl, BH &bh) {
+template <bool kCompleted, class DS, class TJ, class BL, class BH>
+TMED_HD void hs_straus_joint_sum(ge_p2 &out, ge_p1p1 &last, const DS &ds, const uint32_t er[8], int W, TJ &tj, BL &bl,
+                                 BH &bh) {
   constexpr bool b26 = BL::kBits == 26;
   static_assert(BL::kBits == 16 || BL::kBits == 26, "B windows of radix 2^16 or 2^26");
   uint32_t el[4] = {er[0], er[1], er[2], er[3]}, eh[4] = {er[4], er[5], er[6], er[7]};
@@ -490,12 +491,32 @@
       niels_apply_sign(nb, dh < 0);
       ge_madd_niels(t, r, nb, false);
     }
-    ge_p1p1_to_p2(q, t);
-  }
-  out = q;
+    if (!kCompleted || n > 0) ge_p1p1_to_p2(q, t);
+  }
+  if (kCompleted) last = t; else out = q;
+}
+
+template <class DS, class TJ, class BL, class BH>
+TMED_HD void hs_straus_joint(ge_p2 &out, const DS &ds, const uint32_t er[8], int W, TJ &tj, BL &bl, BH &bh) {
+  ge_p1p1 unused;
+  hs_straus_joint_sum<false>(out, unused, ds, er, W, tj, bl, bh);
+}
+
+template <class DS, class TJ, class BL, class BH>
+TMED_HD void hs_straus_joint_completed(ge_p1p1 &out, const DS &ds, const uint32_t er[8], int W, TJ &tj, BL &bl, BH &bh) {
+  ge_p2 unused;
+  hs_straus_joint_sum<true>(unused, out, ds, er, W, tj, bl, bh);
 }
 
 TMED_HD bool p2_is_identity(const ge_p2 &q) { return fe_iszero(q.X) && fe_equal(q.Y, q.Z) && !fe_iszero(q.Z); }
+
+TMED_HD bool p1p1_is_identity(const ge_p1p1 &t) {
+  fe e, g, f;
+  fe_carry(e, t.X);
+  fe_carry(g, t.Z);
+  fe_carry(f, t.T);
+  return fe_iszero(e) && fe_equal(t.Y, t.T) && !fe_iszero(g) && !fe_iszero(f);
+}
 
 TMED_HD void p2_mul8(ge_p2 &q) {
   ge_p1p1 t;
```

Result: no change. 113.7 million verifies/s (-0.0%).
